# PoTaTo-Mika/fish-speech

Measured on AMD Instinct MI355X. Metric: audio-sec/wall-sec (RTF) + p50 first-sample latency, S2-Pro 4B @1/2/4/8 GPU, higher is better.
Workload: dtype bf16; 1 GPU; BASELINE config 2 per GPU: one utterance = 64-token prompt + 216 Dual-AR frames (top_k 30, top_p 0.8, temp 0.8) + codec decode [1,10,216] -> 442368 samples; global_batch=1, frames=216, prompt_len=64, first_chunk_frames=1, vocoder_chunks=first_chunk_frames, then growing 4x, vocoder=serial, parallelism=dp1

## Files before the change

### fish-speech_amd/csrc/fm_attn.hip

```cpp
#include "fm_kernels.h"
#include "fm_runtime.h"
#include "fm_attn_dev.h"
#include "fm_frag.h"

template <typename T>
__device__ __forceinline__ void head_prep(const T* src, int hd, bool norm, const T* nw, float eps,
                                          const float* tab, bool do_rope, float (&x0)[2],
                                          float (&x1)[2], int& np, int lane) {
    const int half = hd >> 1;
    np = 0;
    for (int p = lane; p < half; p += 64, ++np) {
        x0[np] = ld(src, 2 * p);
        x1[np] = ld(src, 2 * p + 1);
    }
    if (norm) {
        float ss = 0.f;
        for (int i = 0; i < np; ++i) ss += x0[i] * x0[i] + x1[i] * x1[i];
        ss = wave_sum(ss);
        const float rs = 1.0f / sqrtf(ss / (float)hd + eps);
        for (int i = 0; i < np; ++i) {
            const int p = lane + 64 * i;
            x0[i] = rnd<T>((x0[i] * rs) * ld(nw, 2 * p));
            x1[i] = rnd<T>((x1[i] * rs) * ld(nw, 2 * p + 1));
        }
    }
    if (do_rope) {
        for (int i = 0; i < np; ++i) {
            const int p = lane + 64 * i;
            const float c = tab[2 * p], s = tab[2 * p + 1];
            const float y0 = x0[i] * c - x1[i] * s;
            const float y1 = x1[i] * c + x0[i] * s;
            x0[i] = rnd<T>(y0);
            x1[i] = rnd<T>(y1);
        }
    }
}

template <typename T>
__global__ __launch_bounds__(512) void attn_decode2_kernel(AttnDecArgs<T> a) {
    extern __shared__ __attribute__((aligned(16))) unsigned char smem[];
    unsigned long long tz[7] = {0, 0, 0, 0, 0, 0, 0};
    DBG_TS(tz, 0)
    const int lane = threadIdx.x & 63, wave = threadIdx.x >> 6;
    const int r = blockIdx.x, kvh = blockIdx.y, sp = blockIdx.z;
    const int hd = a.hd, g = a.nh / a.nkv, ks = hd + 8, cap = a.cap;
    const int half = hd >> 1;
    const T* raw = a.qkv + (size_t)r * a.ldqkv;
    const int slot = a.row_slot[r];
    const int pos = a.row_pos[r];
    float q0[2][2], q1[2][2];
    for (int i = 0; i < 2; ++i) {
        const int hh = wave + 8 * i;
        for (int u = 0; u < 2; ++u) {
            const int p = lane + 64 * u;
            const bool ok = hh < g && p < half;
            const T* src = raw + (size_t)(kvh * g + (ok ? hh : 0)) * hd;
// ... 385 lines not shown
        for (int e = 0; e < 8; ++e) {
            o[e] += __shfl_xor(o[e], 16);
            o[e] += __shfl_xor(o[e], 32);
        }
        if (lane < 16 && vd < hd)
#pragma unroll
            for (int e = 0; e < 8; ++e) ored[wave][h][vd + e] = o[e];
    }
    __syncthreads();
    const bool single = nsp == 1;
    float* part = a.part + (((size_t)r * a.nh + (size_t)kvh * g) * a.maxsplit + sp) * (hd + 2);
    for (int idx = threadIdx.x; idx < g * hd; idx += 256) {
        const int h = idx / hd, e = idx - h * hd;
        const float o = (ored[0][h][e] + ored[1][h][e]) + (ored[2][h][e] + ored[3][h][e]);
        if (single) {
            st(a.out + (size_t)r * a.nh * hd + (size_t)(kvh * g + h) * hd, e, o / mls[h][1]);
        } else {
            float* pp = part + (size_t)h * a.maxsplit * (hd + 2);
            __hip_atomic_store(pp + 2 + e, o, __ATOMIC_RELAXED, __HIP_MEMORY_SCOPE_AGENT);
            if (e == 0) {
                __hip_atomic_store(pp, mls[h][0], __ATOMIC_RELAXED, __HIP_MEMORY_SCOPE_AGENT);
                __hip_atomic_store(pp + 1, mls[h][1], __ATOMIC_RELAXED, __HIP_MEMORY_SCOPE_AGENT);
            }
        }
    }
    if (single) return;
    asm volatile("s_waitcnt vmcnt(0)" ::: "memory");
    __syncthreads();
    if (threadIdx.x == 0) {
        const int t = __hip_atomic_fetch_add(a.cnt + (size_t)r * a.nkv + kvh, 1, __ATOMIC_RELAXED,
                                             __HIP_MEMORY_SCOPE_AGENT);
        flag = t == nsp - 1;
        if (t == nsp - 1) __hip_atomic_store(a.cnt + (size_t)r * a.nkv + kvh, 0, __ATOMIC_RELAXED, __HIP_MEMORY_SCOPE_AGENT);
    }
    __syncthreads();
    if (!flag) return;
    const float* p0 = a.part + (((size_t)r * a.nh + (size_t)kvh * g) * a.maxsplit) * (hd + 2);
    auto ldp = [](const float* q) { return __hip_atomic_load(q, __ATOMIC_RELAXED, __HIP_MEMORY_SCOPE_AGENT); };
    for (int idx = threadIdx.x; idx < g * hd; idx += 256) {
        const int h = idx / hd, e = idx - h * hd;
        const float* pp = p0 + (size_t)h * a.maxsplit * (hd + 2);
        float M = -INFINITY;
        for (int q = 0; q < nsp; ++q) M = fmaxf(M, ldp(pp + (size_t)q * (hd + 2)));
        float L = 0.f, O = 0.f;
        for (int q = 0; q < nsp; ++q) {
            const float w = expf(ldp(pp + (size_t)q * (hd + 2)) - M);
            L += w * ldp(pp + (size_t)q * (hd + 2) + 1);
            O += w * ldp(pp + (size_t)q * (hd + 2) + 2 + e);
        }
        st(a.out + (size_t)r * a.nh * hd + (size_t)(kvh * g + h) * hd, e, O / L);
    }
}

template <typename T> __device__ __forceinline__ void cvt16(const u32x4_t v, float (&o)[16 / sizeof(T)]) {
    if constexpr (sizeof(T) == 2) {
#pragma unroll
        for (int i = 0; i < 4; ++i) {
            o[2 * i] = __uint_as_float(v[i] << 16);
            o[2 * i + 1] = __uint_as_float(v[i] & 0xffff0000u);
        }
    } else {
#pragma unroll
        for (int i = 0; i < 4; ++i) o[i] = __uint_as_float(v[i]);
    }
}

constexpr int FD_GM = 4;
__device__ __forceinline__ float sum_rows4(float v, int lane) {
    const unsigned u = __float_as_uint(v);
    const auto r32 = __builtin_amdgcn_permlane32_swap(u, u, false, false);
    v += __uint_as_float(lane < 32 ? r32[1] : r32[0]);
    const unsigned w = __float_as_uint(v);
    const auto r16 = __builtin_amdgcn_permlane16_swap(w, w, false, false);
    return v + __uint_as_float(((lane >> 4) & 1) ? r16[0] : r16[1]);
}
template <typename T> __device__ __forceinline__ typename Frag<T>::f frag_f32(const float* v) {
    typename Frag<T>::f f;
    if constexpr (sizeof(T) == 2) {
#pragma unroll
        for (int i = 0; i < 4; ++i) f[i] = hi_pair(v[2 * i], v[2 * i + 1]);
    } else {
#pragma unroll
        for (int i = 0; i < 4; ++i) {
            f.lo[i] = v[i];
            f.hi[i] = v[4 + i];
        }
    }
    return f;
}
template <typename T, int HD, int NW, int GM>
__global__ __launch_bounds__(NW * 64) void attn_fd_kernel(AttnDecArgs<T> a) {
    static_assert(GM == 1 || GM == 2 || GM == FD_GM, "1, 2 or every q head of the kv head");
    static_assert(HD % 32 == 0 && HD <= 128, "head_dim a multiple of 32 up to 128");
    constexpr int NT = NW * 64, FD_TILE = 16 * NW;
    constexpr int VL = 8 * (int)sizeof(T) / 16;
    constexpr int half = HD / 2;
    __shared__ __attribute__((aligned(16))) float q_s[GM][HD];
    __shared__ __attribute__((aligned(16))) float kv_new[2][HD];
    __shared__ __attribute__((aligned(16))) float wml[NW][GM][2];
    constexpr int OG = NW > 4 ? 1 : 4;
    __shared__ __attribute__((aligned(16))) float ored[NW][OG][GM][HD];
    __shared__ int flag;
    unsigned long long tz[7] = {0, 0, 0, 0, 0, 0, 0};
    DBG_TS(tz, 0)
    const int lane = threadIdx.x & 63, wave = threadIdx.x >> 6;
    const int l16 = lane & 15, qq = lane >> 4;
    const int r = blockIdx.x, kvh = blockIdx.y;
    const int hg = GM == FD_GM ? 0 : (int)blockIdx.z / a.maxsplit, sp = (int)blockIdx.z - hg * a.maxsplit;
    const int g = min(GM, a.nh / a.nkv - hg * GM), h0 = kvh * (a.nh / a.nkv) + hg * GM, nitem = g + 2;
    const int slot = a.row_slot[r];
    const int pos = a.row_pos[r];
    constexpr int NI = (2 + GM + NW - 1) / NW;
    float x0[NI], x1[NI];
#pragma unroll
    for (int i = 0; i < NI; ++i) {
        const int it = wave + NW * i;
        const int row = it < g ? h0 + it : (it == g ? a.nh + kvh : a.nh + a.nkv + kvh);
        const bool ok = it < nitem && lane < half;
        float v0, v1;
        raw_pair<T>(a.qkv, a.ldqkv, a.qslab, a.qslab_kp, gridDim.x, a.qbias, r,
                    (size_t)(it < nitem ? row : 0) * HD + 2 * (lane < half ? lane : 0), v0, v1);
        x0[i] = ok ? v0 : 0.f;
        x1[i] = ok ? v1 : 0.f;
    }
    const int npos = pos + 1;
    int nsp = min(a.maxsplit, (npos + a.cap - 1) / a.cap);
    const int chunk = ((npos + nsp - 1) / nsp + 15) & ~15;
    nsp = (npos + chunk - 1) / chunk;
    if (sp >= nsp) return;
    const int j0 = sp * chunk, jend = min(j0 + chunk, npos);
    const bool owner = jend == npos;
    const size_t base = (size_t)slot * a.slot_stride + a.layer_off + (size_t)kvh * a.S * HD;
    T* kc = a.kc + base;
    T* vc = a.vc + base;
    const int vd = 8 * l16 < HD ? 8 * l16 : HD - 8;
    using F = Frag<T>;
    constexpr int NKS = HD / 32;
    typename F::f kb[NKS];
    u32x4_t vb[4][VL];
    auto issue = [&](int jb) {
        const int jk = min(jb + 16 * wave + l16, jend - 1);
#pragma unroll
        for (int ks = 0; ks < NKS; ++ks) kb[ks] = F::load(kc + (size_t)jk * HD + 32 * ks + 8 * qq);
#pragma unroll
        for (int it = 0; it < 4; ++it) {
            const int jv = min(jb + 16 * wave + 4 * it + qq, jend - 1);
            const u32x4_t* pv = reinterpret_cast<const u32x4_t*>(vc + (size_t)jv * HD + vd);
#pragma unroll
            for (int c = 0; c < VL; ++c) vb[it][c] = pv[c];
        }
    };
    const float* tab = a.rope + (size_t)pos * HD;
    const float2 rcs = *reinterpret_cast<const float2*>(tab + 2 * (lane < half ? lane : 0));
    issue(j0);
#pragma unroll
    for (int i = 0; i < NI; ++i) {
        const int it = wave + NW * i;
        if (it >= nitem || (it >= g && !owner)) continue;
        const bool isq = it < g, isk = it == g;
        if (a.qk_norm && (isq || isk)) {
            const float ss = wave_sum(x0[i] * x0[i] + x1[i] * x1[i]);
            const float rs = 1.0f / sqrtf(ss / (float)HD + a.eps);
            const T* nw = isq ? a.qn : a.kn;
            if (lane < half) {
                x0[i] = rnd<T>((x0[i] * rs) * ld(nw, 2 * lane));
                x1[i] = rnd<T>((x1[i] * rs) * ld(nw, 2 * lane + 1));
            }
        }
        if (lane < half) {
            float y0 = x0[i], y1 = x1[i];
            if (isq || isk) {
                const float c = rcs.x, sn = rcs.y;
                y0 = rnd<T>(x0[i] * c - x1[i] * sn);
                y1 = rnd<T>(x1[i] * c + x0[i] * sn);
            }
            if (isq) {
                q_s[it][2 * lane] = y0;
                q_s[it][2 * lane + 1] = y1;
                if (a.qdbg && sp == 0) {
                    float* qdp = a.qdbg + ((size_t)r * a.nh + h0 + it) * HD;
                    qdp[2 * lane] = y0;
                    qdp[2 * lane + 1] = y1;
                }
            } else {
                kv_new[isk ? 0 : 1][2 * lane] = y0;
                kv_new[isk ? 0 : 1][2 * lane + 1] = y1;
                if (hg == 0) {
                    T* dst = (isk ? kc : vc) + (size_t)pos * HD;
                    st(dst, 2 * lane, y0);
                    st(dst, 2 * lane + 1, y1);
                }
            }
        }
    }
    lds_barrier();
    DBG_TS(tz, 1)
    const int qh = l16 >> 2;
    const bool qrow = (l16 & 3) == 0 && qh < g;
    typename F::f qa[NKS];
#pragma unroll
    for (int ks = 0; ks < NKS; ++ks) {
        float qv[8];
#pragma unroll
        for (int e = 0; e < 8; ++e) qv[e] = qrow ? q_s[qh < GM ? qh : 0][32 * ks + 8 * qq + e] : 0.f;
        qa[ks] = frag_f32<T>(qv);
    }
    __shared__ __attribute__((aligned(16))) float p_s[NW][16][GM];
    float m_run = -INFINITY, l_run = 0.f, o[GM][8];
#pragma unroll
    for (int h = 0; h < GM; ++h)
#pragma unroll
        for (int e = 0; e < 8; ++e) o[h][e] = 0.f;
    const int npass = (jend - j0 + FD_TILE - 1) / FD_TILE;
    for (int pa = 0; pa < npass; ++pa) {
        const int jb = j0 + pa * FD_TILE;
        const int jk = jb + 16 * wave + l16;
        if (owner && jk == pos) {
#pragma unroll
            for (int ks = 0; ks < NKS; ++ks) kb[ks] = frag_f32<T>(&kv_new[0][32 * ks + 8 * qq]);
        }
        f32x4_t sc = {0.f, 0.f, 0.f, 0.f};
#pragma unroll
        for (int ks = 0; ks < NKS; ++ks) sc = F::mma(qa[ks], kb[ks], sc);
        float vf[4][8];
#pragma unroll
        for (int it = 0; it < 4; ++it)
#pragma unroll
            for (int c = 0; c < VL; ++c) {
                float t[16 / sizeof(T)];
                cvt16<T>(vb[it][c], t);
#pragma unroll
                for (int u = 0; u < (int)(16 / sizeof(T)); ++u) vf[it][c * (16 / sizeof(T)) + u] = t[u];
            }
        if (pa + 1 < npass) issue(jb + FD_TILE);
        if (owner) {
#pragma unroll
            for (int it = 0; it < 4; ++it)
                if (min(jb + 16 * wave + 4 * it + qq, jend - 1) == pos)
#pragma unroll
                    for (int e = 0; e < 8; ++e) vf[it][e] = kv_new[1][vd + e];
        }
        const bool kval = jk < jend && qq < g;
        {
            const float sv = kval ? sc[0] * a.scale : -INFINITY;
            const float mnew = fmaxf(m_run, row_max16(sv));
            const float alpha = mnew == -INFINITY ? 1.f : expf(m_run - mnew);
            const float p = kval ? expf(sv - mnew) : 0.f;
            m_run = mnew;
            l_run = l_run * alpha + p;
            if (GM == FD_GM || qq < GM) p_s[wave][l16][qq] = p;
#pragma unroll
            for (int h = 0; h < GM; ++h) {
                if (h >= g) break;
                const float ah = __int_as_float(__builtin_amdgcn_readlane(__float_as_int(alpha), 16 * h));
#pragma unroll
                for (int e = 0; e < 8; ++e) o[h][e] *= ah;
            }
        }
        __builtin_amdgcn_wave_barrier();
#pragma unroll
        for (int it = 0; it < 4; ++it) {
            float pv[GM];
            if constexpr (GM == 4) {
                const f32x4_t t = *reinterpret_cast<const f32x4_t*>(&p_s[wave][4 * it + qq][0]);
                pv[0] = t[0], pv[1] = t[1], pv[2] = t[2], pv[3] = t[3];
            } else if constexpr (GM == 2) {
                const float2 t = *reinterpret_cast<const float2*>(&p_s[wave][4 * it + qq][0]);
                pv[0] = t.x, pv[1] = t.y;
            } else {
                pv[0] = p_s[wave][4 * it + qq][0];
            }
#pragma unroll
            for (int h = 0; h < GM; ++h) {
                if (h >= g) break;
#pragma unroll
                for (int e = 0; e < 8; ++e) o[h][e] += pv[h] * vf[it][e];
            }
        }
        __builtin_amdgcn_wave_barrier();
    }
    DBG_TS(tz, 2)
    __shared__ unsigned long long wend[NW];
    if (a.dbg && lane == 0) wend[wave] = __builtin_amdgcn_s_memrealtime();
    const float lrow = row_sum16(l_run);
    if (l16 == 0 && qq < g) {
        wml[wave][qq][0] = m_run;
        wml[wave][qq][1] = lrow;
    }
#pragma unroll
    for (int h = 0; h < GM; ++h) {
        if (h >= g) break;
        if constexpr (OG == 1) {
#pragma unroll
            for (int e = 0; e < 8; ++e) o[h][e] = sum_rows4(o[h][e], lane);
        }
        if (8 * l16 < HD && (OG == 4 || qq == 0)) {
            f32x4_t* dst = reinterpret_cast<f32x4_t*>(&ored[wave][OG == 4 ? qq : 0][h][8 * l16]);
            dst[0] = (f32x4_t){o[h][0], o[h][1], o[h][2], o[h][3]};
            dst[1] = (f32x4_t){o[h][4], o[h][5], o[h][6], o[h][7]};
        }
    }
    DBG_TS(tz, 5)
    lds_barrier();
    DBG_TS(tz, 3)
    const bool single = nsp == 1;
    for (int idx = threadIdx.x; idx < g * HD; idx += NT) {
        const int h = idx / HD, e = idx - h * HD;
        float M = wml[0][h][0];
#pragma unroll
        for (int w = 1; w < NW; ++w) M = fmaxf(M, wml[w][h][0]);
        float L = 0.f, O = 0.f;
#pragma unroll
        for (int w = 0; w < NW; ++w) {
            const float sc = expf(wml[w][h][0] - M);
            L += sc * wml[w][h][1];
            if constexpr (OG == 4)
                O += sc * ((ored[w][0][h][e] + ored[w][1][h][e]) + (ored[w][2][h][e] + ored[w][3][h][e]));
            else
                O += sc * ored[w][0][h][e];
        }
        if (single) {
            st(a.out + (size_t)r * a.nh * HD + (size_t)(h0 + h) * HD, e, O / L);
        } else {
            float* pp = a.part + (((size_t)r * a.nh + h0 + h) * a.maxsplit + sp) * (HD + 2);
            __hip_atomic_store(pp + 2 + e, O, __ATOMIC_RELAXED, __HIP_MEMORY_SCOPE_AGENT);
            if (e == 0) {
                __hip_atomic_store(pp, M, __ATOMIC_RELAXED, __HIP_MEMORY_SCOPE_AGENT);
                __hip_atomic_store(pp + 1, L, __ATOMIC_RELAXED, __HIP_MEMORY_SCOPE_AGENT);
            }
        }
    }
    if (a.dbg && threadIdx.x == 0) {
        tz[4] = __builtin_amdgcn_s_memrealtime();
        for (int w = 0; w < NW; ++w) tz[6] = wend[w] > tz[6] ? wend[w] : tz[6];
        dbg_record(a.dbg, 0xFFFC, (unsigned)(nsp << 16 | (jend - j0)), tz);
    }
    if (single) return;
    asm volatile("s_waitcnt vmcnt(0)" ::: "memory");
    __syncthreads();
    if (threadIdx.x == 0) {
        int* tk = a.cnt + (size_t)r * a.nh + kvh * (a.nh / a.nkv) + hg;
        const int t = __hip_atomic_fetch_add(tk, 1, __ATOMIC_RELAXED, __HIP_MEMORY_SCOPE_AGENT);
        flag = t == nsp - 1;
        if (t == nsp - 1) __hip_atomic_store(tk, 0, __ATOMIC_RELAXED, __HIP_MEMORY_SCOPE_AGENT);
    }
    __syncthreads();
    if (!flag) return;
    DBG_TS(tz, 5)
    constexpr int PP = GM * HD * 8 / NT > 0 ? GM * HD * 8 / NT : 1;
    const int q = l16, grp = threadIdx.x >> 4;
    const int k0 = grp * PP, h = k0 / half, e0 = 2 * (k0 - h * half);
    if (h >= g) return;
    const int qc = q < nsp ? q : nsp - 1;
    const unsigned long long* pp = reinterpret_cast<const unsigned long long*>(
        a.part + (((size_t)r * a.nh + h0 + h) * a.maxsplit + qc) * (HD + 2));
    const unsigned long long ml = __hip_atomic_load(pp, __ATOMIC_RELAXED, __HIP_MEMORY_SCOPE_AGENT);
    unsigned long long ov[PP];
#pragma unroll
    for (int j = 0; j < PP; ++j) ov[j] = __hip_atomic_load(pp + 1 + e0 / 2 + j, __ATOMIC_RELAXED, __HIP_MEMORY_SCOPE_AGENT);
    const float mq = q < nsp ? __uint_as_float((unsigned)ml) : -INFINITY;
    const float lq = __uint_as_float((unsigned)(ml >> 32));
    float M = mq;
#pragma unroll
    for (int m = 1; m < 16; m <<= 1) M = fmaxf(M, __shfl_xor(M, m));
    const float w = q < nsp ? expf(mq - M) : 0.f;
    float L = w * lq;
#pragma unroll
    for (int m = 1; m < 16; m <<= 1) L += __shfl_xor(L, m);
    T* out = a.out + (size_t)r * a.nh * HD + (size_t)(h0 + h) * HD + e0;
#pragma unroll
    for (int j = 0; j < PP; ++j) {
        float o0 = w * __uint_as_float((unsigned)ov[j]), o1 = w * __uint_as_float((unsigned)(ov[j] >> 32));
#pragma unroll
        for (int m = 1; m < 16; m <<= 1) {
            o0 += __shfl_xor(o0, m);
            o1 += __shfl_xor(o1, m);
        }
        if (q == (j & 15)) {
            st(out, 2 * j, o0 / L);
            st(out, 2 * j + 1, o1 / L);
        }
    }
    if (a.dbg && threadIdx.x == 0) {
        tz[6] = __builtin_amdgcn_s_memrealtime();
        dbg_record(a.dbg, 0xFFFB, (unsigned)nsp, tz);
    }
}

template <typename T>
__global__ __launch_bounds__(64) void fast_attn2_kernel(FastFusedArgs<T> a) {
    unsigned long long tz[7] = {0, 0, 0, 0, 0, 0, 0};
    DBG_TS(tz, 0)
    fast_attn_head<T>(a, blockIdx.x, blockIdx.y, threadIdx.x, tz);
    if (a.dbg && threadIdx.x == 0) {
        tz[4] = __builtin_amdgcn_s_memrealtime();
        dbg_record(a.dbg, 0xFFFE, (unsigned)a.cpos, tz);
    }
}

template <typename T>
__global__ __launch_bounds__(256) void fast_attn_fused_kernel(FastFusedArgs<T> a) {
    extern __shared__ __attribute__((aligned(16))) unsigned char smem[];
    const int lane = threadIdx.x & 63, wave = threadIdx.x >> 6;
    const int r = blockIdx.x, kvh = blockIdx.y;
    const int slot = a.row_slot[r];
    const int hd = a.hd, g = a.nh / a.nkv, C = a.S, cpos = a.cpos;
    float* Kt = reinterpret_cast<float*>(smem);
    float* Vt = Kt + (size_t)C * hd;
    float* qs = Vt + (size_t)C * hd;
    float* ps = qs + 4 * hd;
    const size_t base = (size_t)slot * a.slot_stride + a.layer_off + (size_t)kvh * C * hd;
    T* kc = a.kc + base;
    T* vc = a.vc + base;
    const T* raw = a.qkv + (size_t)r * a.ldqkv;
    const float* tab = a.rope + (size_t)cpos * hd;
    if (wave < 2) {
        float x0[2], x1[2];
        int np;
        const int hk = wave == 0 ? a.nh + kvh : a.nh + a.nkv + kvh;
        head_prep<T>(raw + (size_t)hk * hd, hd, wave == 0 && a.qk_norm, a.kn, a.eps, tab, wave == 0, x0,
                     x1, np, lane);
        T* dst = (wave == 0 ? kc : vc) + (size_t)cpos * hd;
        float* tile = (wave == 0 ? Kt : Vt) + (size_t)cpos * hd;
        for (int i = 0; i < np; ++i) {
            const int p = lane + 64 * i;
            st(dst, 2 * p, x0[i]);
            st(dst, 2 * p + 1, x1[i]);
            tile[2 * p] = x0[i];
            tile[2 * p + 1] = x1[i];
        }
    }
    for (int idx = threadIdx.x; idx < cpos * hd; idx += 256) {
        Kt[idx] = ld(kc, idx);
        Vt[idx] = ld(vc, idx);
    }
    for (int hb = 0; hb < g; hb += 4) {
        const int ql = hb + wave;
        if (ql < g) {
            float x0[2], x1[2];
// ... 785 lines not shown
```

### fish-speech_amd/csrc/fm_kernels.h

```cpp
#pragma once
#include <algorithm>
#include "fm_common.h"
#include "fm_tune_table.h"

enum { EPI_STORE = 0, EPI_RESID = 1, EPI_SWIGLU = 2, EPI_F32 = 3 };

template <typename T> void launch_swiglu_i8(hipStream_t s, const T* t, int ldt, T* act, int lda, int inter, int R);
template <typename T> void launch_pack(hipStream_t s, const T* src, int N, int K, T* dst);
template <typename T> void launch_quant_rows(hipStream_t s, T* w, int N, int K, int8_t* q, T* scale);
template <typename T> void launch_i8_to(hipStream_t s, const int8_t* q, int64_t n, T* dst);
void launch_pack_q8(hipStream_t s, const int8_t* src, int N, int K, int8_t* dst);
void launch_pack_q8s(hipStream_t s, const int8_t* src, int N, int K, int8_t* dst);
void launch_quant4(hipStream_t s, bf16_t* w, int N, int K, int gs, uint8_t* q, uint32_t* sz);
void launch_pack_q4(hipStream_t s, const uint8_t* q, int N, int K, uint8_t* dst);
void launch_pack_q4_rows(hipStream_t s, const uint8_t* q, int N, int K, uint32_t* dst);
void launch_pack_sz4(hipStream_t s, const uint32_t* sz, int N, int K, int gs, uint32_t* dst);
void launch_pack_q4s(hipStream_t s, const uint8_t* q, int N, int K, uint32_t* dst);

template <typename T> struct LinearArgs {
    const T* W;
    const T* W2;
    const T* bias;
    const T* X;
    int ldx, R, N, K;
// ... 341 lines not shown
    float* slab;
    bf16_t* act = nullptr;
    int lda = 0;
    const bf16_t* wscale = nullptr;
    const unsigned char* q8s = nullptr;
    const uint32_t* q4s = nullptr;
    const uint32_t* sz = nullptr;
};
void launch_prompt_skinny(hipStream_t s, const PromptSkinnyArgs& a, int ks);
int prompt_skinny_ks(int N, int K, int target);

template <typename T> struct AttnDecArgs {
    const T* qkv;
    int ldqkv;
    const int* row_slot;
    const int* row_pos;
    int nh, nkv, hd, qk_norm;
    float eps;
    const T* qn;
    const T* kn;
    const float* rope;
    T* kc;
    T* vc;
    size_t slot_stride, layer_off;
    int S, maxsplit;
    float scale;
    float* part;
    int cap;
    int* cnt;
    T* out;
    unsigned long long* dbg;
    float* qdbg = nullptr;
    int nwb = 4;
    int hpb = 4;
    const float* qslab = nullptr;
    int qslab_kp = 1;
    const T* qbias = nullptr;
};
template <typename T> void launch_attn_decode2(hipStream_t s, const AttnDecArgs<T>& a, int R);
inline size_t attn2_lds_bytes(int hd, int g, int cap, size_t esz) {
    return (size_t)cap * (hd + 8) * esz + (size_t)cap * hd * esz + (size_t)g * hd * 4 + (size_t)g * cap * 4 +
           16 + 8 * (size_t)g * 4;
}
inline int attn2_cap(int hd, int g, size_t esz) {
    long budget = 150L * 1024 - 16 - 8L * g * 4 - (long)g * hd * 4;
    long per = (long)(2 * hd + 8) * (long)esz + 4L * g;
    long c = budget / per;
    c = c > 256 ? 256 : c;
    return (int)(c & ~15L);
}
constexpr int FD_NSP = 16;
inline bool attn_fd_ok(int hd, int g) { return (hd == 32 || hd == 64 || hd == 128) && g >= 1 && g <= 4; }
template <typename T> void launch_attn_fd(hipStream_t s, const AttnDecArgs<T>& a, int R);
template <typename T> void launch_attn_decode3(hipStream_t s, const AttnDecArgs<T>& a, int R);
template <typename T> void launch_fast_attn_fused(hipStream_t s, const FastFusedArgs<T>& a, int R);
template <typename T> void launch_fast_attn2(hipStream_t s, const FastFusedArgs<T>& a, int R);
template <typename T> void launch_sample_radix(hipStream_t s, const SampleArgs& a, int R);
int sample_fast_max_row();
void sample_init();
template <typename T>
void launch_attn_combine(hipStream_t s, const float* part, const int* row_pos, int R, int nh, int hd,
                         int split, int maxsplit, T* out);
```

### fish-speech_amd/csrc/fm_llm.cpp

```cpp
#include <math.h>

#include <memory>

#include "fm_llm_model.h"

static thread_local std::string g_err;
void fm_set_error(const std::string& s) { g_err = s; }
extern "C" const char* fm_last_error(void) { return g_err.c_str(); }
extern "C" int fm_device_count(void) {
    int n = 0;
    if (hipGetDeviceCount(&n) != hipSuccess) return 0;
    return n;
}

static void check_tokens(fm_llm* m, const int32_t* tok, int T) {
    const fm_model_config& c = m->c;
    for (int t = 0; t < T; ++t) {
        const int t0 = tok[t];
        FMCHECK(t0 >= 0 && t0 < c.vocab_size, "token id out of range: " + std::to_string(t0));
        for (int q = 0; q < m->C; ++q) {
            const int v = tok[(size_t)(q + 1) * T + t];
            FMCHECK(v >= 0 && v < m->cb, "codebook token out of range: " + std::to_string(v));
        }
    }
}

static void reset_slot(fm_llm* m, int slot, const fm_sampling* sp) {
    HIPCHK(hipMemsetAsync((char*)m->ras + (size_t)slot * m->C1 * 10 * 4, 0, (size_t)m->C1 * 10 * 4, m->stream));
    SlotParams p{};
    if (sp) {
        FMCHECK(sp->top_k >= 1, "top_k must be >= 1: got " + std::to_string(sp->top_k));
        p.temperature = sp->temperature;
        p.top_p = sp->top_p;
        p.top_k = sp->top_k;
        p.mask_im_end = sp->mask_im_end;
        p.seed = sp->seed;
    } else {
        p.temperature = 0.7f;
        p.top_p = 0.9f;
        p.top_k = 1;
    }
    p.step = 0;
    p.force = m->host_force[slot];
    HIPCHK(hipMemcpyAsync(m->sp + slot, &p, sizeof p, hipMemcpyHostToDevice, m->stream));
    HIPCHK(hipStreamSynchronize(m->stream));
    m->host_step[slot] = 0;
}

static void upload_frame_rows(fm_llm* m, const int32_t* slots, int n) {
    std::vector<int> s(slots, slots + n), p(n);
    if (s == m->uploaded_slots) return;
    for (int i = 0; i < n; ++i) p[i] = m->host_pos[s[i]];
    HIPCHK(hipMemcpyAsync(m->frame_slot, s.data(), (size_t)n * 4, hipMemcpyHostToDevice, m->stream));
    HIPCHK(hipMemcpyAsync(m->frame_pos, p.data(), (size_t)n * 4, hipMemcpyHostToDevice, m->stream));
    HIPCHK(hipStreamSynchronize(m->stream));
    m->uploaded_slots = s;
}

static void chain_err_async(fm_llm* m) {
    if (fm_tuning().gemv_chain || fm_tuning().fin_split > 1 ||
        (m->fxt && fm_tuning().fattn_wo))
        HIPCHK(hipMemcpyAsync(m->h_chain_err, m->chain_err, sizeof(int), hipMemcpyDeviceToHost, m->stream));
}
static void chain_err_check(fm_llm* m) {
    if (!m->h_chain_err || !m->h_chain_err[0]) return;
    m->h_chain_err[0] = 0;
    HIPCHK(hipMemset(m->chain_cnt, 0, GEMV_CHAIN_WORDS * sizeof(unsigned)));
    HIPCHK(hipMemset(m->chain_err, 0, 16 * sizeof(int)));
    if (m->fin_cnt) HIPCHK(hipMemset(m->fin_cnt, 0, (size_t)std::max(m->max_slots, 64) * 2 * sizeof(int)));
    throw FmError{FM_ERR_STATE,
                  "in-launch hand-off wait timed out (gemv chain / split finalize / fused fast "
                  "attention + wo; counters reset)"};
}

extern "C" {

int fm_llm_open(const fm_model_config* cfg, int device, int precision, int max_slots, fm_llm** out) {
    return fm_guard([&] {
        FMCHECK(cfg && out, "null argument");
        FMCHECK(precision == FM_PREC_BF16 || precision == FM_PREC_FP32, "bad precision");
        FMCHECK(max_slots >= 1 && max_slots <= 4096, "bad max_slots");
        const fm_model_config& c = *cfg;
        FMCHECK(c.dim % 32 == 0 && c.fast_dim % 32 == 0, "dims must be multiples of 32");
        FMCHECK(c.intermediate_size % 32 == 0 && c.fast_intermediate_size % 32 == 0,
                "intermediate sizes must be multiples of 32");
        FMCHECK((c.n_head * c.head_dim) % 32 == 0 && (c.fast_n_head * c.fast_head_dim) % 32 == 0,
                "n_head*head_dim must be a multiple of 32");
        FMCHECK(c.head_dim % 8 == 0 && c.head_dim <= 256 && c.fast_head_dim <= 256, "bad head_dim");
        FMCHECK(c.n_head % c.n_local_heads == 0 && c.fast_n_head % c.fast_n_local_heads == 0, "bad GQA");
        FMCHECK(c.num_codebooks >= 1 && c.num_codebooks <= 63, "bad num_codebooks");
        FMCHECK(c.codebook_size <= 8192, "codebook_size > 8192 unsupported");
        FMCHECK(c.im_end_id >= 0 && c.im_end_id < c.vocab_size, "im_end_id must be set");
        FMCHECK(c.semantic_begin_id >= 0 && c.semantic_end_id < c.vocab_size &&
                    c.semantic_begin_id <= c.semantic_end_id,
                "bad semantic id range");
        int ndev = fm_device_count();
        FMCHECK(ndev > 0, "no HIP device visible");
        FMCHECK(device >= 0 && device < ndev, "bad device index");
        HIPCHK(hipSetDevice(device));
        std::unique_ptr<fm_llm> m(new fm_llm());
        m->c = c;
        m->device = device;
        m->prec = precision;
        m->esz = precision == FM_PREC_BF16 ? 2 : 4;
        m->max_slots = max_slots;
        m->S = (c.max_seq_len + 7) / 8 * 8;
        m->C = c.num_codebooks;
        m->C1 = c.num_codebooks + 1;
        m->cb = c.codebook_size;
        HIPCHK(hipStreamCreateWithFlags(&m->stream, hipStreamNonBlocking));
        const char* g = getenv("FISHMI_GRAPH");
        m->use_graph = !(g && g[0] == '0');
        build_inventory(m.get());
        *out = m.release();
    });
}

int fm_llm_set_quant_int4(fm_llm* m, int groupsize) {
    return fm_guard([&] {
        FMCHECK(m && (groupsize == 32 || groupsize == 64 || groupsize == 128 || groupsize == 256),
                "int4: groupsize must be 32, 64, 128 or 256 (WeightOnlyInt4QuantHandler, quantize.py:366)");
        FMCHECK(!m->finalized, "weights are frozen after finalize");
        for (auto& kv : m->w) FMCHECK(!kv.second.set, "set the quantization mode before any tensor");
        FMCHECK(m->quant == FM_QUANT_NONE, "quantization mode already set");
// ... 513 lines not shown
```

### fish-speech_amd/csrc/fm_llm_frame.cpp

```cpp
#include <math.h>

#include <algorithm>
#include <array>

#include "fm_codec.h"
#include "fm_llm_model.h"

template <typename T> struct Run {
    typedef T type_t;
    fm_llm* m;
    hipStream_t s;
    int64_t E;
    bool rows_distinct_slots = false, bs_frame = false, x_ss = false;
    struct BsPending {
        bool on = false;
        const float* slab = nullptr;
        int kparts = 0, d = 0, R = 0;
        void* res = nullptr;
        void* out = nullptr;
        const void* sc = nullptr;
    } pend;
    std::vector<std::array<int, 2>> segs;
    void set_pending(const float* slab, int kparts, int d, int R, void* res, void* out, const void* sc) {
        pend = BsPending{true, slab, kparts, d, R, res, out, sc};
// ... 692 lines not shown
        a.ldx = ldx_in;
        a.xidx = xidx;
        a.xidx_ld = m->C1;
        a.xidx_col = xcol;
        a.xidx_rows = xidx ? m->cb : 0;
        gemv(L.wqkv, a, PRO_NORM, EPI_STORE, 1, "linear", kv_rows ? d.nq() / 16 : 0);
    }
    GemvArgs<T> qkv_args(const StackDims& d, const LayerW& L, int n) {
        GemvArgs<T> a = ga();
        a.bias = (const T*)L.bqkv;
        a.nw = (const T*)L.an;
        a.R = n;
        a.N = d.nqkv();
        a.K = d.dim;
        a.Y = (T*)m->qkv;
        a.ldy = d.nqkv();
        return a;
    }
    static int dead_q_bits(const fm_llm* m) { return m->quant && !m->fdm.o_bias ? fm_tuning().fast_dead_q : 0; }
    bool qkv0_live() const {
        return sizeof(T) == 2 && (m->quant ? (dead_q_bits(m) & 1) : (row_bits() & 32)) && m->qkv0 && m->qkv0_built &&
               m->qkv0_epoch == fm_tuning().epoch;
    }

    struct Small {
        const StackDims& d;
        const LayerW& L;
        int n;
        bool first;
        const void* x_in;
        int ldx_in;
        const int32_t* xidx;
        int xcol;
        void *xb, *hb;
        bool is_fast;
        int cpos, layer;
        KsbPlan kp;
        void* xo;
        int pair = 0;
        const void* x_in1 = nullptr;
    };
    static const void* row1(const Small& c, const void* p, int w) {
        return (const char*)p + (c.pair == 2 ? (size_t)w * sizeof(T) : 0);
    }
    static void* row1(const Small& c, void* p, int w) { return (char*)p + (c.pair == 2 ? (size_t)w * sizeof(T) : 0); }
    struct SmallPath {
        bool rf;
        bool fw;
        bool att_wo;
        bool row_here;
        bool tab;
        bool kv0;
        bool kv_only;
    };
    SmallPath small_path(const Small& c, bool kv_only) const {
        const StackDims& d = c.d;
        SmallPath p{};
        p.kv_only = kv_only;
        p.rf = row_fin(c.n);
        const int fq = m->qmode();
        const bool fw_any = c.is_fast && p.rf && fm_tuning().fattn_wo && m->fxt && m->fdm.n_layer * m->C >= 2 &&
                            m->fdm.n_layer * m->C <= 40 && fattn_wo_ok(d.nh, d.nkv, d.hd, c.cpos, d.dim, d.nq(), fq);
        p.fw = fw_any && !kv_only;
        p.att_wo = c.is_fast && !kv_only && fm_tuning().attn_wo && !m->quant && c.n == 1 && c.cpos < 16 && d.hd % 16 == 0 &&
                   d.hd <= 128 && d.nh % d.nkv == 0 && (d.nq() / c.kp.wo) % d.hd == 0 && d.nqkv() % 8 == 0;
        p.row_here = row_qkv(c.n) && (!c.first || (row_bits() & 16));
        const bool bits56 = sizeof(T) == 2 && !m->quant && c.is_fast && c.n == 1;
        const int dq = sizeof(T) == 2 && c.is_fast && c.n == 1 && fw_any && fattn_wo_dead_ok(d.nq(), fq) ? dead_q_bits(m) : 0;
        p.tab = (bits56 || (dq & 1)) && c.first && c.xidx && p.fw && qkv0_live();
        p.kv0 = bits56 && c.cpos == 0 && (row_bits() & 64) && p.row_here && !p.att_wo && d.hd <= 256 &&
                (d.nqkv() - d.nq()) % fm_tuning().row_qkv_rp == 0;
        if ((dq & 2) && c.cpos == 0 && !p.att_wo && d.hd <= 256)
            p.kv0 = m->quant == FM_QUANT_INT4
                        ? p.row_here && (d.nqkv() - d.nq()) % fm_tuning().row_qkv_rp == 0 && (d.nqkv() - d.nq()) % 8 == 0
                        : !p.row_here && d.nq() % 16 == 0 && d.nqkv() % 16 == 0;
        return p;
    }
    FastFusedArgs<T> small_fast_args(const Small& c, const SmallPath& p) const {
        const StackDims& d = c.d;
        FastFusedArgs<T> fa{(const T*)m->qkv, d.nqkv(), m->frame_slot, d.nh, d.nkv, d.hd, d.qk_norm,
                            m->c.norm_eps, (const T*)c.L.qn, (const T*)c.L.kn, m->frope, (T*)m->fkc,
                            (T*)m->fvc, m->fslot_stride, (size_t)c.layer * m->flayer_stride, m->C, c.cpos,
                            1.0f / sqrtf((float)d.hd), (T*)m->att};
        fa.dbg = fm_tuning().dbg;
        fa.noq = p.kv0;
        return fa;
    }
    void small_qkv(const Small& c, const SmallPath& p) {
        if (p.tab && !c.pair) return;
        const StackDims& d = c.d;
        GemvArgs<T> a = qkv_args(d, c.L, c.n);
        if (!c.is_fast && c.n == 1 && fm_tuning().kv_prefetch)
            kv_prefetch(a, (const T*)m->kc, (const T*)m->vc, m->frame_slot, m->frame_pos, m->slot_stride,
                        (size_t)c.layer * m->layer_stride, m->S, d.nkv, d.hd);
        else if (c.is_fast && c.n == 1 && fm_tuning().fkv_prefetch && m->fiota && c.cpos < 16)
            kv_prefetch(a, (const T*)m->fkc, (const T*)m->fvc, m->frame_slot, m->fiota + c.cpos, m->fslot_stride,
                        (size_t)c.layer * m->flayer_stride, m->C, d.nkv, d.hd);
        if (c.first) {
            qkv_first(d, c.L, a, c.n, c.x_in, c.ldx_in, c.pair ? nullptr : c.xidx, c.pair ? 0 : c.xcol, m->qkv,
                      p.kv0 || c.pair);
        } else if (p.row_here) {
            qkv_row(d, c.L, a, false, c.xb, 0, nullptr, 0, m->qkv, p.kv0, c.pair != 0);
        } else {
            a.X = (const T*)c.xb;
            a.ldx = d.dim;
            a.ss_in = m->ssX;
            a.ss_gran = p.rf ? 1 : 0;
            gemv(c.L.wqkv, a, PRO_PRENORM, EPI_STORE, 1, "linear", p.kv0 ? d.nq() / 16 : 0);
        }
    }
    void small_attn(const Small& c, const SmallPath& p) {
        const StackDims& d = c.d;
        const int n = c.n;
        hipStream_t st = s;
        if (!c.is_fast) {
            AttnDecArgs<T> aa{(const T*)m->qkv, d.nqkv(), m->frame_slot, m->frame_pos, d.nh, d.nkv, d.hd,
                              d.qk_norm, m->c.norm_eps, (const T*)c.L.qn, (const T*)c.L.kn, m->rope, (T*)m->kc,
                              (T*)m->vc, m->slot_stride, (size_t)c.layer * m->layer_stride, m->S,
                              m->maxsplit, 1.0f / sqrtf((float)d.hd), m->part};
            aa.cap = attn2_frame_cap(d.hd, d.nh / d.nkv, E, false);
            aa.maxsplit = FM_CEIL(m->S, aa.cap);
            aa.cnt = m->attn_cnt;
            aa.dbg = fm_tuning().dbg;
            aa.out = (T*)m->att;
            auto go = [st, aa, n] { attn_slow_on(st, aa, n); };
            m->prof.record("attn_slow", 0, go);
            launch("attn", 0, 0, go);
        } else if (!p.att_wo && !p.fw) {
            const FastFusedArgs<T> fa = small_fast_args(c, p);
            const bool f2 = c.cpos < 16 && d.hd <= 256;
            launch("attn", 0, 0, [st, fa, n, f2] {
                if (f2)
                    launch_fast_attn2<T>(st, fa, n);
                else
                    launch_fast_attn_fused<T>(st, fa, n);
            });
        }
    }
    void small_wo(const Small& c, const SmallPath& p) {
        const StackDims& d = c.d;
        const LayerW& L = c.L;
        if (p.fw || p.rf) {
            FattnWoArgs A{};
            RowGemvArgs& r = A.wo;
            row_weight(r, L.wo);
            r.X = (const bf16_t*)m->att;
            r.bias = (const bf16_t*)L.bo;
            if (!c.pair) {
                row_residual(r, c.first, c.x_in, c.ldx_in, c.xidx, c.xcol, c.xb, d.dim);
                r.res_out = (bf16_t*)c.hb;
            } else {
                RowGemvArgs r1{};
                row_residual(r1, c.first, c.x_in1, c.ldx_in, c.xidx, c.xcol, (const bf16_t*)c.xb + d.dim, d.dim);
                r.ldr = r1.ldr;
                r.residx = r1.residx;
                r.res_col = r1.res_col;
                r.res_rows = r1.res_rows;
                if (c.pair == 2) {
                    r.res = r1.res;
                    r.res_out = (bf16_t*)c.hb + d.dim;
                } else {
                    r.xr = 2;
                    r.res = (const bf16_t*)(c.first ? c.x_in : c.xb);
                    r.res1 = r1.res;
                    r.res_out = (bf16_t*)c.hb;
                    r.res_out1 = (bf16_t*)c.hb + d.dim;
                }
            }
            r.N = d.dim;
            r.K = d.nq();
            if (!p.fw) {
                rowgemv(r, ROWGEMV_FIN);
                return;
            }
            const FastFusedArgs<T> fa = small_fast_args(c, p);
            A.at = *reinterpret_cast<const FastFusedArgs<bf16_t>*>(&fa);
            A.at.dbg = nullptr;
            A.at.row_pos = m->frame_pos;
            A.xt = m->fxt;
            A.gen = 1 + c.layer + m->fdm.n_layer * c.cpos;
            A.err = m->chain_err;
            A.delay = fm_tuning().fw_delay;
            A.cheap = fm_tuning().fw_cheap;
            A.prio = fm_tuning().fw_prio;
            A.ilp = fm_tuning().fattn_ilp;
            if (p.tab) {
                A.qtab = (const bf16_t*)m->qkv0;
                A.qidx = c.xidx;
                A.qcol = c.xcol;
                A.qrows = m->cb;
            }
            A.kv0 = p.kv0;
            A.pair = c.pair;
            hipStream_t st = s;
            auto go = [st, A] { launch_fattn_wo(st, A); };
            launch("attn", rowgemv_wbytes(r), 2.0 * r.N * r.K, go, "attn_wo");
            return;
        }
        GemvArgs<T> a = ga();
        a.bias = (const T*)L.bo;
        a.X = (const T*)m->att;
        a.ldx = d.nq();
        a.R = c.n;
        a.N = d.dim;
        a.K = d.nq();
        a.Yf = m->slabA;
        a.ldy = d.dim;
        if (c.first) {
            a.res = (const T*)c.x_in;
            a.ldr = c.ldx_in;
            a.residx = c.xidx;
            a.xidx_ld = m->C1;
            a.xidx_col = c.xcol;
            a.xidx_rows = c.xidx ? m->cb : 0;
        } else {
            a.res = (const T*)c.xb;
            a.ldr = d.dim;
        }
        a.res_out = (T*)c.hb;
        a.ldro = d.dim;
        a.ss_out = m->ssH;
        a.tickets = m->tickets;
        if (p.att_wo) a.att = small_fast_args(c, p);
// ... 556 lines not shown
```

### fish-speech_amd/csrc/fm_llm_model.h

```cpp
#pragma once
#include <hip/hip_runtime.h>

#include <algorithm>

#include "fm_kernels.h"
#include "fm_runtime.h"

static constexpr int PREFILL_CHUNK = 1024;
static constexpr int ATTN_PIECE = 256;
static constexpr int ATTN_SPLIT = 64;
static constexpr int GEMV_MAX_ROWS = 8;
static constexpr int KSB_MAX = 8;

inline int attn2_frame_cap(int hd, int g, size_t esz, bool batched) {
    const int cap = attn2_cap(hd, g, esz), knob = batched ? fm_tuning().attn_cap_batched : fm_tuning().attn_cap;
    return knob ? std::min(cap, knob) : cap;
}
struct AttnSlowPlan {
    int kernel, nwb, cap;
    int hpb = 4;
};
inline int fd_hpb_rows(int R) { return R <= GEMV_MAX_ROWS ? fm_tuning().fd_hpb : 4; }
inline AttnSlowPlan attn_slow_plan(int R, int hd, int g, int cap0) {
    const FmTuning& tu = fm_tuning();
// ... 82 lines not shown
    int S = 0, C = 0, C1 = 0, cb = 0, nsem = 0, Nhead = 0, maxsplit = 0, Rmax = 0;
    std::vector<LayerW> slow, fast;
    void *emb = nullptr, *cbemb = nullptr, *norm = nullptr, *fproj_b = nullptr, *femb = nullptr, *fnorm = nullptr;
    Linear head_c, fproj_w, fout;
    void *kc = nullptr, *vc = nullptr, *fkc = nullptr, *fvc = nullptr;
    size_t slot_stride = 0, layer_stride = 0, fslot_stride = 0, flayer_stride = 0;
    float *rope = nullptr, *frope = nullptr;
    void *x = nullptr, *h = nullptr, *xn = nullptr, *qkv = nullptr, *q = nullptr, *att = nullptr,
         *act = nullptr;
    void *xl = nullptr, *xnl = nullptr, *fx = nullptr, *fh = nullptr, *fxn = nullptr;
    void *x2 = nullptr, *fx2 = nullptr;
    unsigned* chain_cnt = nullptr;
    int* chain_err = nullptr;
    int* h_chain_err = nullptr;
    void* plast = nullptr;
    float *part = nullptr, *logits = nullptr, *flogits = nullptr;
    void* act2 = nullptr;
    int* attn_cnt = nullptr;
    float *ssX = nullptr, *ssH = nullptr;
    int* tickets = nullptr;
    float* skpart = nullptr;
    long long skpart_cap = 0;
    float *slabA = nullptr, *slabB = nullptr;
    float *bsA = nullptr, *bsB = nullptr;
    float* bsQ = nullptr;
    int *frame_slot = nullptr, *frame_pos = nullptr, *prow_slot = nullptr, *prow_pos = nullptr;
    int32_t *tok_in = nullptr, *cols = nullptr, *ptok = nullptr, *ras = nullptr;
    SlotParams* sp = nullptr;
    int32_t* force_cols = nullptr;
    float *tap_slow = nullptr, *tap_fast = nullptr;
    std::vector<int> host_force;
    int32_t* h_cols = nullptr;
    int32_t* h_hist = nullptr;
    size_t h_hist_n = 0;
    std::vector<int> host_pos, host_step;
    std::vector<int> uploaded_slots;
    bool use_graph = true;
    std::map<int, hipGraphExec_t> graphs;
    Profiler prof;
    std::vector<void*> allocs;
    int quant = FM_QUANT_NONE;
    int q4_gs = 0;
    int qmode() const { return quant == FM_QUANT_INT8 ? 1 : (quant == FM_QUANT_INT4 ? 2 : 0); }
    int* fin_cnt = nullptr;
    float* fin_ss = nullptr;
    bool compact = false;
    bool streams_codes() const { return quant != FM_QUANT_INT4 || fm_tuning().int4_stream || compact; }
    int64_t mem[7] = {0, 0, 0, 0, 0, 0, 0};
    int mem_cat = 6;
    bool row_ok = false;
    bool row_qkv_ok = false;
    bool row_w13_ok = false;
    uint32_t* fxt = nullptr;
    int32_t* fiota = nullptr;
    void* qkv0 = nullptr;
    int32_t* qkv0_iota = nullptr;
    unsigned qkv0_epoch = 0;
    bool qkv0_built = false;
    struct Prefix {
        void* buf = nullptr;
        int npos = 0;
        size_t bytes = 0;
    };
    std::map<int, Prefix> prefixes;
    int next_prefix_id = 1;
    int* pfx_slots = nullptr;

    ~fm_llm() {
        if (device >= 0) (void)hipSetDevice(device);
        for (auto& g : graphs) (void)hipGraphExecDestroy(g.second);
        for (auto& kv : w) {
            if (kv.second.p) (void)hipFree(kv.second.p);
            if (kv.second.q) (void)hipFree(kv.second.q);
        }
        for (void* p : allocs) (void)hipFree(p);
        for (auto& kv : prefixes) (void)hipFree(kv.second.buf);
        if (h_cols) (void)hipHostFree(h_cols);
        if (h_hist) (void)hipHostFree(h_hist);
        if (h_chain_err) (void)hipHostFree(h_chain_err);
        if (stream) (void)hipStreamDestroy(stream);
    }
    void* dalloc(size_t bytes, bool zero = true) {
        void* p = nullptr;
        if (bytes == 0) bytes = 16;
        hipError_t e = hipMalloc(&p, bytes);
        if (e != hipSuccess)
            throw FmError{FM_ERR_OOM, "hipMalloc(" + std::to_string(bytes) + ") failed: " + hipGetErrorString(e)};
        if (zero) HIPCHK(hipMemsetAsync(p, 0, bytes, stream));
        allocs.push_back(p);
        mem[mem_cat] += (int64_t)bytes;
        return p;
    }
};

void add_t(fm_llm* m, const std::string& n, int64_t rows, int64_t cols);
void build_inventory(fm_llm* m);
DTensor& tensor_for(fm_llm* m, const char* name, int64_t numel);
bool is_quant_linear(const std::string& n);
std::string base_of(const std::string& n);
void finalize(fm_llm* m);
void ensure_qkv0(fm_llm* m);
void launch_frame(fm_llm* m, int n);
void decode_frame_eager(fm_llm* m, int n);
void prefill_frame(fm_llm* m, int slot, const int32_t* tokens, int T, int pos0);
void prefill_batch_frame(fm_llm* m, int n, const int32_t* slots, const int32_t* const* toks, const int32_t* T,
                         const int32_t* pos0);
// ... 3 lines not shown
```

### fish-speech_amd/csrc/fm_llm_weights.cpp

```cpp
#include "fm_llm_model.h"

void add_t(fm_llm* m, const std::string& n, int64_t rows, int64_t cols) {
    DTensor t;
    t.rows = rows;
    t.cols = cols;
    t.numel = rows * cols;
    m->w[n] = t;
}
static void add_stack(fm_llm* m, const std::string& pre, const StackDims& s) {
    for (int i = 0; i < s.n_layer; ++i) {
        std::string p = pre + std::to_string(i) + ".";
        add_t(m, p + "attention.wqkv.weight", s.nqkv(), s.dim);
        if (s.qkv_bias) add_t(m, p + "attention.wqkv.bias", 1, s.nqkv());
        add_t(m, p + "attention.wo.weight", s.dim, s.nq());
        if (s.o_bias) add_t(m, p + "attention.wo.bias", 1, s.dim);
        if (s.qk_norm) {
            add_t(m, p + "attention.q_norm.weight", 1, s.hd);
            add_t(m, p + "attention.k_norm.weight", 1, s.hd);
        }
        add_t(m, p + "feed_forward.w1.weight", s.inter, s.dim);
        add_t(m, p + "feed_forward.w3.weight", s.inter, s.dim);
        add_t(m, p + "feed_forward.w2.weight", s.dim, s.inter);
        add_t(m, p + "ffn_norm.weight", 1, s.dim);
        add_t(m, p + "attention_norm.weight", 1, s.dim);
// ... 330 lines not shown
    if (m->finalized) return;
    const fm_model_config& c = m->c;
    bsacc_init();
    sample_init();
    for (auto& kv : m->w) FMCHECK(kv.second.set || kv.second.optional, "tensor not set: " + kv.first);
    if (m->compact) {
        FMCHECK(m->quant && m->prec == FM_PREC_BF16, "compact: a weight-only bf16 handle only");
        for (auto& kv : m->w) {
            if (!is_quant_linear(kv.first)) continue;
            const int64_t K = kv.second.cols;
            if (m->quant == FM_QUANT_INT4)
                FMCHECK(m->q4_gs % 128 == 0 && K % 128 == 0 && K % m->q4_gs == 0,
                        "compact int4 needs a group size and in_features that are multiples of 128: " + kv.first +
                            " (group size " + std::to_string(m->q4_gs) + ", in_features " + std::to_string(K) + ")");
            else
                FMCHECK(K % 64 == 0, "compact int8 needs in_features % 64 == 0: " + kv.first);
        }
    }
    if (m->quant) quantize_linears(m);
    std::map<std::string, Linear> plain;
    for (auto& kv : m->w)
        if (is_linear_weight(kv.first) && !is_ffn_w13(kv.first)) plain[kv.first] = plain_linear(m, kv.first);
    m->row_ok = m->row_qkv_ok = m->row_w13_ok = true;
    auto stack = [&](const std::string& pre, const StackDims& d, std::vector<LayerW>& out) {
        out.resize(d.n_layer);
        for (int i = 0; i < d.n_layer; ++i) {
            std::string p = pre + std::to_string(i) + ".";
            LayerW& L = out[i];
            L.wqkv = plain.at(p + "attention.wqkv.weight");
            L.wo = plain.at(p + "attention.wo.weight");
            L.w13 = w13_linear(m, p, d.inter, d.dim);
            L.w2 = plain.at(p + "feed_forward.w2.weight");
            L.bqkv = m->quant ? nullptr : Wopt(m, p + "attention.wqkv.bias");
            L.bo = m->quant ? nullptr : Wopt(m, p + "attention.wo.bias");
            L.qn = Wopt(m, p + "attention.q_norm.weight");
            L.kn = Wopt(m, p + "attention.k_norm.weight");
            L.an = W(m, p + "attention_norm.weight");
            L.fn = W(m, p + "ffn_norm.weight");
            m->row_ok = m->row_ok && L.wo.rm && L.w2.rm;
            m->row_qkv_ok = m->row_qkv_ok && L.wqkv.rm;
            m->row_w13_ok = m->row_w13_ok && L.w13.rm;
        }
    };
    stack("layers.", m->sd, m->slow);
    stack("fast_layers.", m->fdm, m->fast);
    {
        int32_t io[16];
        for (int c = 0; c < 16; ++c) io[c] = c - 1;
        m->fiota = (int32_t*)m->dalloc(sizeof(io), false);
        HIPCHK(hipMemcpy(m->fiota, io, sizeof(io), hipMemcpyHostToDevice));
    }
    if (m->prec == FM_PREC_BF16)
        m->fxt = (uint32_t*)m->dalloc(2 * (size_t)m->fdm.nh * m->fdm.hd * sizeof(uint32_t));
    m->emb = W(m, "embeddings.weight");
    m->cbemb = W(m, "codebook_embeddings.weight");
    m->norm = W(m, "norm.weight");
    if (plain.count("fast_project_in.weight")) m->fproj_w = plain.at("fast_project_in.weight");
    m->fproj_b = m->quant ? nullptr : Wopt(m, "fast_project_in.bias");
    m->femb = W(m, "fast_embeddings.weight");
    m->fnorm = W(m, "fast_norm.weight");
    m->fout = plain.at("fast_output.weight");
    m->head_c = head_linear(m);
    for (auto& kv : m->w) {
        const DTensor& t = kv.second;
        if (!t.p || is_linear_weight(kv.first)) continue;
        const int64_t rows = t.rows > 1 ? (t.rows + 15) / 16 * 16 : 1;
        const std::string& n = kv.first;
        const bool scales = n.size() > 7 && n.compare(n.size() - 7, 7, ".scales") == 0;
        m->mem[scales ? 1 : 4] += rows * t.cols * (int64_t)m->esz;
    }
    const StackDims& d = m->sd;
    m->layer_stride = (size_t)d.nkv * m->S * d.hd;
    m->slot_stride = m->layer_stride * d.n_layer;
    m->mem_cat = 5;
    m->kc = m->dalloc(m->slot_stride * m->max_slots * m->esz);
    m->vc = m->dalloc(m->slot_stride * m->max_slots * m->esz);
    const StackDims& f = m->fdm;
    m->flayer_stride = (size_t)f.nkv * m->C * f.hd;
    m->fslot_stride = m->flayer_stride * f.n_layer;
    m->fkc = m->dalloc(m->fslot_stride * m->max_slots * m->esz);
    m->fvc = m->dalloc(m->fslot_stride * m->max_slots * m->esz);
    m->mem_cat = 6;
    auto rt = rope_table_host(m->S, d.hd, c.rope_base);
    m->rope = (float*)m->dalloc(rt.size() * 4, false);
    HIPCHK(hipMemcpy(m->rope, rt.data(), rt.size() * 4, hipMemcpyHostToDevice));
    auto frt = rope_table_host(m->C, f.hd, c.rope_base);
    m->frope = (float*)m->dalloc(frt.size() * 4, false);
    HIPCHK(hipMemcpy(m->frope, frt.data(), frt.size() * 4, hipMemcpyHostToDevice));
    const int R = m->Rmax = std::max(m->max_slots, PREFILL_CHUNK);
    const int dmax = std::max(c.dim, c.fast_dim);
    const int qkvmax = std::max(d.nqkv(), f.nqkv()), qmax = std::max(d.nq(), f.nq());
    const int imax = std::max(d.inter, f.inter);
    const size_t E = m->esz;
    m->x = m->dalloc((size_t)R * dmax * E);
    m->h = m->dalloc((size_t)R * dmax * E);
    m->xn = m->dalloc((size_t)R * dmax * E);
    m->qkv = m->dalloc((size_t)R * qkvmax * E);
    m->q = m->dalloc((size_t)R * qmax * E);
    m->att = m->dalloc((size_t)R * qmax * E);
    m->act = m->dalloc((size_t)R * imax * E);
    m->act2 = m->dalloc((size_t)R * 2 * imax * E);
    const int n = m->max_slots;
    m->xl = m->dalloc((size_t)n * dmax * E);
    m->plast = m->dalloc((size_t)n * dmax * E);
    m->xnl = m->dalloc((size_t)n * dmax * E);
    m->fx = m->dalloc((size_t)std::max(n, 2) * dmax * E);
// ... 54 lines not shown
```

### fish-speech_amd/csrc/fm_ops.cpp

```cpp
#include <hip/hip_runtime.h>
#include <math.h>
#include <string.h>

#include <algorithm>
#include <vector>

#include "fm_codec.h"
#include "fm_kernels.h"
#include "fm_llm_model.h"
#include "fm_ops_util.h"
#include "fm_runtime.h"

using namespace fm_ops_util;

namespace {

struct TuneScope {
    int& knob;
    const int keep;
    TuneScope(int& k, int v) : knob(k), keep(k) { knob = v; }
    ~TuneScope() { knob = keep; }
};

template <typename T>
// ... 468 lines not shown
    r.K = K;
    InOut<bf16_t> y(b, o.y, (size_t)(o.pair == 1 ? 2 : 1) * N);
    r.res = res;
    r.res_out = y.d;
    if (o.pair == 1) {
        r.xr = 2;
        r.res = b.upload<bf16_t>(o.res0, (size_t)N);
        r.res1 = res;
        r.res_out1 = y.d + N;
    }
    int* err = (int*)b.alloc(16);
    if (o.fused) {
        FattnWoArgs A{};
        A.at = at;
        A.wo = r;
        A.wo.X = att;
        A.xt = (uint32_t*)b.alloc((size_t)2 * K * 4);
        if (o.xt_init) b.put(A.xt, o.xt_init, (size_t)2 * K * 4);
        A.gen = o.gen;
        A.err = err;
        A.delay = fm_tuning().fw_delay;
        A.cheap = fm_tuning().fw_cheap;
        A.prio = fm_tuning().fw_prio;
        A.ilp = o.ilp;
        if (qtab) {
            A.qtab = qtab;
            A.qidx = idx;
            A.qcol = o.idx_col;
            A.qrows = o.qrows;
        }
        A.kv0 = o.kv0;
        A.pair = o.pair;
        launch_fattn_wo(s, A);
    } else {
        FMCHECK(!o.pair, "the unfused composition runs one row");
        if (qtab) {
            const int iv = o.idx[o.idx_col], xi = iv < 0 ? 0 : (iv >= o.qrows ? o.qrows - 1 : iv);
            at.qkv = qtab + (size_t)xi * ld;
        }
        at.noq = o.kv0;
        launch_fast_attn2<bf16_t>(s, at, 1);
        HIPCHK(hipGetLastError());
        r.X = att;
        launch_rowgemv(s, r, ROWGEMV_FIN);
    }
    HIPCHK(hipGetLastError());
    y.get(s);
    kc.get(s);
    vc.get(s);
    HIPCHK(hipMemcpyAsync(&o.status[1], err, 4, hipMemcpyDeviceToHost, s));
    HIPCHK(hipStreamSynchronize(s));
}

template <typename T>
void embed_t(hipStream_t s, const int32_t* tok, int R, const float* emb, int V, const float* cbemb, int d, int C,
             int cb, int sb, int se, int scale, float* x) {
    DevBufs b(s);
    T* e = b.upload<T>(emb, (size_t)V * d);
    T* ce = b.upload<T>(cbemb, (size_t)C * cb * d);
    int32_t* td = (int32_t*)b.alloc((size_t)R * (C + 1) * 4);
    b.put(td, tok, (size_t)R * (C + 1) * 4);
    T* xd = (T*)b.alloc((size_t)R * d * sizeof(T));
    launch_embed<T>(s, td, R, e, ce, d, C, cb, sb, se, scale, xd, nullptr);
    HIPCHK(hipGetLastError());
    download<T>(xd, (size_t)R * d, x, s);
}

int count_nonzero(const int* d, size_t n, hipStream_t s) {
    std::vector<int> h(n);
    HIPCHK(hipMemcpyAsync(h.data(), d, n * 4, hipMemcpyDeviceToHost, s));
    HIPCHK(hipStreamSynchronize(s));
    return (int)std::count_if(h.begin(), h.end(), [](int v) { return v != 0; });
}

template <typename T> T* upload_packed(DevBufs& b, const float* w, int N, int K) {
    T* t = b.upload<T>(w, (size_t)N * K);
    T* pk = (T*)b.alloc((size_t)((N + 15) / 16 * 16) * K * sizeof(T));
    launch_pack<T>(b.s, t, N, K, pk);
    HIPCHK(hipGetLastError());
    return pk;
}

template <typename T>
void linear_op_t(hipStream_t s, int epi, const float* w, const float* w2, const float* bias, const float* x, int ldx,
                 const float* res, int ldr, int R, int N, int K, int split, float* y, int ldy, int y_rows, int reps,
                 int* ksb_out, int* dirty) {
    DevBufs b(s);
    const bool f32 = epi == EPI_F32;
    LinearArgs<T> a{};
    a.W = upload_packed<T>(b, w, N, K);
    if (epi == EPI_SWIGLU) a.W2 = upload_packed<T>(b, w2, N, K);
    if (bias) a.bias = b.upload<T>(bias, (size_t)N);
    a.X = b.upload<T>(x, (size_t)R * ldx);
    a.ldx = ldx;
    a.R = R;
    a.N = N;
    a.K = K;
    a.ldy = ldy;
    if (epi == EPI_RESID) {
        a.res = b.upload<T>(res, (size_t)R * ldr);
        a.ldr = ldr;
    }
    InOut<T> yt(b, y, f32 ? 1 : (size_t)y_rows * ldy);
    InOut<float> yf(b, y, f32 ? (size_t)y_rows * ldy : 1);
    a.Y = f32 ? nullptr : yt.d;
    a.Yf = f32 ? yf.d : nullptr;
// ... 563 lines not shown
        FMCHECK(qkv && kcache && vcache && out, "null argument");
        FMCHECK(!qk_norm || (qn && kn), "qk_norm needs both norm weights");
        FMCHECK(kernel >= 0 && kernel <= 3,
                "kernel must be 0 (fast_attn2), 1 (fast_attn2, noq), 2 (fast_attn_fused) or 3 (qk_rope_cache + fast_attn)");
        FMCHECK(R >= 1 && R <= 64 && nh >= 1 && nkv >= 1 && nh % nkv == 0, "bad rows / head counts");
        FMCHECK(hd >= 8 && hd <= 256 && hd % 8 == 0, "head_dim a multiple of 8 up to 256");
        FMCHECK(S >= 1 && S <= 63 && cpos >= 0 && cpos < S, "1 to 63 codebooks, cpos among them");
        FMCHECK(kernel > 1 || cpos < 16, "fast_attn2 positions are < 16");
        FMCHECK(kernel != 1 || cpos == 0, "noq is the codebook-0 form");
        FMCHECK(kernel != 2 || (size_t)2 * S * hd * 4 + (size_t)4 * hd * 4 + 1024 <= 64 * 1024, "fast_attn_fused: LDS tile too large");
        check_slot_rows(R, row_slot, nullptr, nslots, layers, layer, S);
        for (int r = 0; r < R; ++r)
            for (int q = 0; q < r; ++q) FMCHECK(row_slot[q] != row_slot[r], "two rows in one slot");
        StreamGuard g(device);
        const SlotRows sr{row_slot, nullptr, nslots, layers, layer};
        if (precision == FM_PREC_BF16)
            fast_attn_t<bf16_t>(g.s, kernel, qkv, R, nh, nkv, hd, qn, kn, qk_norm, eps, rope_base, sr, cpos, kcache, vcache, S, out);
        else
            fast_attn_t<float>(g.s, kernel, qkv, R, nh, nkv, hd, qn, kn, qk_norm, eps, rope_base, sr, cpos, kcache, vcache, S, out);
    });
}

int fm_op_fattn_wo(int device, int quant, int gs, int fused, const float* qkv, const float* qtab, int qrows,
                   const int32_t* idx, int idx_n, int idx_col, int nh, int nkv, int hd, const float* qn, const float* kn,
                   int qk_norm, float eps, float rope_base, int slot, int cpos, int nslots, int layers, int layer,
                   float* kcache, float* vcache, int S, const float* w, const float* bias, const float* res,
                   int res_rows, int ldr, const float* res0, int N, int kv0, int pair, int ilp, int gen, int pos0,
                   const uint32_t* xt_init, float* y, int* status) {
    return fm_guard([&] {
        FMCHECK(qkv && kcache && vcache && w && res && y && status, "null argument");
        FMCHECK(quant == FM_QUANT_NONE || quant == FM_QUANT_INT8 || quant == FM_QUANT_INT4, "bad quant");
        FMCHECK(!qk_norm || (qn && kn), "qk_norm needs both norm weights");
        FMCHECK(nh >= 1 && nkv >= 1 && nh % nkv == 0 && hd >= 8 && hd <= 128 && hd % 8 == 0, "bad heads / head_dim");
        FMCHECK(S >= 1 && S <= 63 && cpos >= 0 && cpos < S && N >= 16 && N % 16 == 0, "bad S / cpos / N");
        FMCHECK(quant == FM_QUANT_NONE || !bias, "the int8 / int4 row forms take no bias");
        FMCHECK(quant != FM_QUANT_INT4 || (gs >= 8 && gs % 8 == 0 && (nh * hd) % gs == 0), "bad int4 group size");
        FMCHECK(!idx || (idx_n >= 1 && idx_col >= 0 && idx_col < idx_n), "bad index column");
        FMCHECK(res_rows >= 1 && ldr >= N && gen >= 1 && gen <= 40 && pos0 >= 0, "bad residual table / gen / position");
        FMCHECK(!qtab || (idx && !kv0 && qrows >= 1 && qrows == res_rows), "the table form is gathered by the residual's index");
        FMCHECK(!kv0 || (!idx && cpos == 0), "the K / V-only form runs at codebook 0, no gather");
        FMCHECK(pair >= 0 && pair <= 2, "pair must be 0, 1 or 2");
        FMCHECK(!pair || (fused && quant == FM_QUANT_NONE && !kv0 && cpos == 1 && (qtab != nullptr) == (idx != nullptr) &&
                          (pair == 1 ? res0 != nullptr : !qtab)),
                "pair form: fused, bf16, positions 0 and 1, row 0's residual (pair 1), no table in the last layer (pair 2)");
        check_slot_rows(1, &slot, nullptr, nslots, layers, layer, S);
        StreamGuard g(device);
        const FattnWoOp o{quant, gs, fused, qkv, qtab, qrows, idx, idx_n, idx_col, nh, nkv, hd, qn, kn, qk_norm, eps,
                          rope_base, slot, cpos, nslots, layers, layer, kcache, vcache, S, w, bias, res, res_rows, ldr,
                          res0, N, kv0, pair, ilp, gen, pos0, xt_init, y, status};
        fattn_wo_op(g.s, o);
    });
}

int fm_op_qk_rope(int device, int precision, int kernel, const float* qkv, int nh, int nkv, int hd, const float* qn,
                  const float* kn, int qk_norm, float eps, float rope_base, int pos, float* q_out, float* k_out) {
    return fm_guard([&] {
        FMCHECK(qkv && q_out && k_out, "null argument");
        FMCHECK(!qk_norm || (qn && kn), "qk_norm needs both norm weights");
        FMCHECK(kernel >= 0 && kernel <= 3,
                "kernel must be 0 (slow attn_decode2), 1 (fast attn2), 2 (slow attn_dec3) or 3 (slow attn_fd)");
        FMCHECK(nh >= 1 && nkv >= 1 && nh % nkv == 0 && nh / nkv <= 16, "bad head counts");
        FMCHECK(hd >= 8 && hd <= 256 && hd % 8 == 0, "bad head_dim");
        FMCHECK(pos >= 0 && pos < 65536, "bad position");
        StreamGuard g(device);
        if (precision == FM_PREC_BF16)
            qk_rope_t<bf16_t>(g.s, kernel, qkv, nh, nkv, hd, qn, kn, qk_norm, eps, rope_base, pos, q_out, k_out);
        else
            qk_rope_t<float>(g.s, kernel, qkv, nh, nkv, hd, qn, kn, qk_norm, eps, rope_base, pos, q_out, k_out);
    });
}

int fm_op_embed(int device, int precision, const int32_t* tok, int R, const float* emb, int vocab,
                const float* cbemb, int dim, int num_codebooks, int codebook_size, int semantic_begin_id,
                int semantic_end_id, int scale_codebook_embeddings, float* x) {
    return fm_guard([&] {
        FMCHECK(tok && emb && cbemb && x && R >= 1 && dim % 8 == 0, "bad arguments");
        for (int r = 0; r < R; ++r) {
            FMCHECK(tok[(size_t)r * (num_codebooks + 1)] >= 0 && tok[(size_t)r * (num_codebooks + 1)] < vocab,
                    "token id out of range");
            for (int q = 1; q <= num_codebooks; ++q) {
                const int v = tok[(size_t)r * (num_codebooks + 1) + q];
                FMCHECK(v >= 0 && v < codebook_size, "codebook token out of range");
            }
        }
        StreamGuard g(device);
        if (precision == FM_PREC_BF16)
            embed_t<bf16_t>(g.s, tok, R, emb, vocab, cbemb, dim, num_codebooks, codebook_size, semantic_begin_id,
                            semantic_end_id, scale_codebook_embeddings, x);
        else
            embed_t<float>(g.s, tok, R, emb, vocab, cbemb, dim, num_codebooks, codebook_size, semantic_begin_id,
                           semantic_end_id, scale_codebook_embeddings, x);
    });
}

int fm_op_quant4(int device, const float* w, int N, int K, int gs, uint8_t* q, float* scale, float* zero,
                 float* w_deq, const float* x, int R, float* y_q4, float* y_bf16) {
    return fm_guard([&] {
        FMCHECK(w && q && scale && zero && w_deq && N >= 1 && gs >= 2 && K % gs == 0, "bad arguments");
        FMCHECK(!x || (R >= 1 && R <= 8 && K % 32 == 0 && y_bf16), "bad GEMV arguments");
        StreamGuard g(device);
        DevBufs b(g.s);
        const int Np = (N + 15) / 16 * 16;
        bf16_t* dw = (bf16_t*)b.alloc((size_t)Np * K * 2);
        {
            bf16_t* t = b.upload<bf16_t>(w, (size_t)N * K);
            HIPCHK(hipMemcpyAsync(dw, t, (size_t)N * K * 2, hipMemcpyDeviceToDevice, g.s));
// ... 703 lines not shown
```

### fish-speech_amd/csrc/fm_rowgemv.hip

```cpp
#include "fm_common.h"
#include "fm_kernels.h"
#include "fm_runtime.h"
#include <type_traits>

typedef __attribute__((ext_vector_type(2))) uint32_t u32x2_t;
typedef __attribute__((ext_vector_type(4))) __bf16 bf16x4_t;

__device__ __forceinline__ float dot4(u32x2_t w, u32x2_t x, float acc) {
    const bf16x4_t wb = __builtin_bit_cast(bf16x4_t, w), xb = __builtin_bit_cast(bf16x4_t, x);
    acc = __builtin_amdgcn_fdot2_f32_bf16(__builtin_shufflevector(wb, wb, 0, 1), __builtin_shufflevector(xb, xb, 0, 1),
                                          acc, false);
    acc = __builtin_amdgcn_fdot2_f32_bf16(__builtin_shufflevector(wb, wb, 2, 3), __builtin_shufflevector(xb, xb, 2, 3),
                                          acc, false);
    return acc;
}
__device__ __forceinline__ float lo16(uint32_t w) { return __uint_as_float(w << 16); }
__device__ __forceinline__ float hi16(uint32_t w) { return __uint_as_float(w & 0xffff0000u); }
__device__ __forceinline__ float dot8r(u32x4_t w, u32x4_t x, float acc) {
    const bf16x8_t wb = __builtin_bit_cast(bf16x8_t, w), xb = __builtin_bit_cast(bf16x8_t, x);
    acc = __builtin_amdgcn_fdot2_f32_bf16(__builtin_shufflevector(wb, wb, 0, 1), __builtin_shufflevector(xb, xb, 0, 1),
                                          acc, false);
    acc = __builtin_amdgcn_fdot2_f32_bf16(__builtin_shufflevector(wb, wb, 2, 3), __builtin_shufflevector(xb, xb, 2, 3),
                                          acc, false);
    acc = __builtin_amdgcn_fdot2_f32_bf16(__builtin_shufflevector(wb, wb, 4, 5), __builtin_shufflevector(xb, xb, 4, 5),
                                          acc, false);
    acc = __builtin_amdgcn_fdot2_f32_bf16(__builtin_shufflevector(wb, wb, 6, 7), __builtin_shufflevector(xb, xb, 6, 7),
                                          acc, false);
    return acc;
}
__device__ __forceinline__ void ld_pair_bf(const bf16_t* p, float& x0, float& x1) {
    const uint32_t w = *reinterpret_cast<const uint32_t*>(p);
    x0 = lo16(w);
    x1 = hi16(w);
}

template <int QM> struct RowT {
    static constexpr int EPL = QM ? 8 : 4;
    static constexpr int CE = 64 * EPL;
    using XV = typename std::conditional<QM != 0, u32x4_t, u32x2_t>::type;
    static constexpr int WPL = QM == 2 ? 1 : 2;
};

template <int U, int RP, bool PRENORM, int EPI, bool G, int QM, bool TX, int XR = 1>
__device__ __forceinline__ void rowgemv_body(const RowGemvArgs& a, const int blk, const uint32_t* xt, const uint32_t gen,
                                             int* err) {
    static_assert(!TX || (!PRENORM && EPI == 1), "tagged x: the residual form only");
    static_assert(XR == 1 || (XR == 2 && QM == 0 && EPI <= 1 && (!G || EPI == 1)), "two x rows: bf16 STORE / FIN");
    constexpr bool FIN = EPI == 1;
    using R = RowT<QM>;
    using XV = typename R::XV;
    constexpr int EPL = R::EPL, NW = EPL / 2;
    constexpr int SB = XR * 4 * RP;
    constexpr bool LATE = XR == 2 && !TX && !PRENORM && U >= 10;
    __shared__ float red[XR * (4 * RP + 8)];
    const int lane = threadIdx.x & 63, wave = threadIdx.x >> 6;
    const int n0 = blk * RP;
    const int nch = a.K / R::CE;
    const int wa = (wave * nch) >> 2, nmy = (((wave + 1) * nch) >> 2) - wa;
    const int last = nmy > 0 ? nmy - 1 : 0;
    const unsigned long long ts0 = a.dbg ? __builtin_amdgcn_s_memrealtime() : 0;
    const int er = n0 + (int)(threadIdx.x % RP);
    const int ex = XR == 2 ? (int)((threadIdx.x / RP) & 1) : 0;
    int ri = 0, xi = 0;
    if constexpr (G && FIN) {
        const int32_t iv = a.residx[a.res_col];
        ri = iv < 0 ? 0 : (iv >= a.res_rows ? a.res_rows - 1 : iv);
    } else if constexpr (G) {
        const int32_t iv = a.xidx[a.xcol];
        xi = iv < 0 ? 0 : (iv >= a.xrows ? a.xrows - 1 : iv);
    }
    bf16_t rv = 0;
    if constexpr (FIN && XR == 2) rv = ex ? a.res1[(size_t)ri * a.ldr + er] : a.res[er];
    else if constexpr (FIN) rv = a.res[(size_t)ri * a.ldr + er];
    const bf16_t bv = *(a.bias ? a.bias + er : a.X);
    bf16_t sv = 0;
    if constexpr (QM == 1) sv = a.wscale[er];
    const XV* xp = reinterpret_cast<const XV*>(a.X + (size_t)xi * a.ldx) + (size_t)wa * 64 + lane;
    const XV* gp = reinterpret_cast<const XV*>(PRENORM ? a.nw : a.X) + (size_t)wa * 64 + lane;
    XV xv[XR][U], gv[PRENORM ? U : 1];
    if constexpr (!TX) {
#pragma unroll
        for (int u = 0; u < U; ++u) {
            const int j = (u < last ? u : last) * 64;
            xv[0][u] = xp[j];
            if constexpr (XR == 2 && !LATE) xv[1][u] = (reinterpret_cast<const XV*>(a.X1) + (size_t)wa * 64 + lane)[j];
            if constexpr (PRENORM) gv[u] = gp[j];
        }
    }
    constexpr int PF = 2;
    const bool pf_on = EPI == 0 && a.pf_kc != nullptr;
    int pf_s = 0, pf_p = 0;
    if constexpr (EPI == 0) {
        pf_s = *(pf_on ? a.pf_slot : reinterpret_cast<const int32_t*>(a.X));
        pf_p = *(pf_on ? a.pf_pos : reinterpret_cast<const int32_t*>(a.X));
    }
    asm volatile("" ::: "memory");
    constexpr int WU = QM == 2 ? 1 : U, WR = QM == 2 ? 1 : RP;
    constexpr int QU = QM == 2 ? U : 1, QR = QM == 2 ? RP : 1;
    u32x2_t wv[WU][WR];
    uint32_t w4[QU][QR], szv[QU][QR];
    if constexpr (QM == 2) {
        const size_t rw = (size_t)(a.K >> 3);
        const int ng = a.K / a.gs;
        const uint32_t* wp = a.Wq4 + (size_t)n0 * rw + (size_t)wa * 64 + lane;
#pragma unroll
        for (int u = 0; u < U; ++u) {
            const int jc = u < last ? u : last;
#pragma unroll
            for (int r = 0; r < RP; ++r) {
                w4[u][r] = __builtin_nontemporal_load(wp + r * rw + jc * 64);
                szv[u][r] = a.wsz[(size_t)(n0 + r) * ng + ((wa + jc) * 512 + lane * 8) / a.gs];
            }
        }
    } else {
        const unsigned char* wb = QM ? reinterpret_cast<const unsigned char*>(a.Wq) : reinterpret_cast<const unsigned char*>(a.W);
        const size_t rowb = (size_t)a.K * (QM ? 1 : 2);
        const u32x2_t* wp = reinterpret_cast<const u32x2_t*>(wb + (size_t)n0 * rowb) + (size_t)wa * 64 + lane;
        const size_t rs8 = rowb / 8;
#pragma unroll
        for (int u = 0; u < U; ++u) {
            const int j = (u < last ? u : last) * 64;
#pragma unroll
            for (int r = 0; r < RP; ++r) wv[u][r] = __builtin_nontemporal_load(wp + r * rs8 + j);
        }
    }
    asm volatile("" ::: "memory");
    unsigned long long tsw = 0, tsx = 0;
    unsigned polls = 0;
    if constexpr (TX) {
        if (a.dbg) tsw = __builtin_amdgcn_s_memrealtime();
        const __amdgpu_buffer_rsrc_t xr = __builtin_amdgcn_make_buffer_rsrc((void*)xt, (short)0, XR * a.K * 4, 0x00020000);
        u32x4_t xw[XR][U][EPL / 4];
        for (unsigned it = 0;; ++it) {
            polls = it + 1;
#pragma unroll
            for (int x = 0; x < XR; ++x)
#pragma unroll
                for (int u = 0; u < U; ++u) {
                    const int jc = u < last ? u : last;
#pragma unroll
                    for (int q = 0; q < EPL / 4; ++q)
                        xw[x][u][q] = __builtin_amdgcn_raw_buffer_load_b128(
                            xr, (x * a.K + (wa + jc) * R::CE + EPL * lane + 4 * q) * 4, 0, 16);
                }
            bool ok = true;
#pragma unroll
            for (int x = 0; x < XR; ++x)
#pragma unroll
                for (int u = 0; u < U; ++u)
#pragma unroll
                    for (int q = 0; q < EPL / 4; ++q)
#pragma unroll
                        for (int e = 0; e < 4; ++e) ok = ok && ((xw[x][u][q][e] & 0xffffu) == gen);
            if (__all(ok)) break;
            if (it >= (1u << 14)) {
                if (lane == 0) __hip_atomic_store(err, 1, __ATOMIC_RELAXED, __HIP_MEMORY_SCOPE_AGENT);
                break;
            }
            __builtin_amdgcn_s_sleep(1);
        }
        if (a.dbg) tsx = __builtin_amdgcn_s_memrealtime();
#pragma unroll
        for (int x = 0; x < XR; ++x)
#pragma unroll
            for (int u = 0; u < U; ++u)
#pragma unroll
                for (int h = 0; h < NW; ++h) {
                    const uint32_t w0 = xw[x][u][(2 * h) >> 2][(2 * h) & 3], w1 = xw[x][u][(2 * h + 1) >> 2][(2 * h + 1) & 3];
                    xv[x][u][h] = (w0 >> 16) | (w1 & 0xffff0000u);
                }
    }
    float pfw[PF];
    if constexpr (EPI == 0) {
        const char* kcb = reinterpret_cast<const char*>(pf_on ? a.pf_kc : a.X);
        const long long dv = pf_on ? reinterpret_cast<const char*>(a.pf_vc) - kcb : 0;
        const int nkv = pf_on ? a.pf_nkv : 1;
        const int b = blockIdx.x, h = b % nkv, jb = b / nkv, nb = ((int)gridDim.x - 1 - h) / nkv + 1;
        const int spr = pf_on ? a.pf_hd * 2 / 64 : 1;
        const int np = pf_on ? pf_p + 1 : 0, total = 2 * np * spr;
        const long long base = pf_on ? (long long)pf_s * (long long)a.pf_slot_stride + (long long)a.pf_layer_off +
                                           (long long)h * a.pf_S * a.pf_hd
                                     : 0;
#pragma unroll
        for (int q = 0; q < PF; ++q) {
            const int i = (jb + nb * q) * 256 + (int)threadIdx.x;
            const bool ok = i < total;
            const int ii = ok ? i : 0, row = ii / spr, sec = ii - row * spr;
            const bool isv = row >= np;
            const long long off = (isv ? dv : 0) + 2 * (base + (long long)(isv ? row - np : row) * a.pf_hd) + sec * 64;
            pfw[q] = *reinterpret_cast<const float*>(kcb + (ok ? off : 0));
        }
    }
    if constexpr (PRENORM && XR == 1) {
        float sl = 0.f;
#pragma unroll
        for (int u = 0; u < U; ++u) {
            if (u < nmy) {
#pragma unroll
                for (int h = 0; h < NW; ++h) {
                    const float e0 = lo16(xv[0][u][h]), e1 = hi16(xv[0][u][h]);
                    sl += e0 * e0 + e1 * e1;
                }
            }
        }
        sl = wave_sum(sl);
        if (lane == 0) red[4 * RP + wave] = sl;
        lds_barrier();
        const float tot = ((red[4 * RP] + red[4 * RP + 1]) + red[4 * RP + 2]) + red[4 * RP + 3];
        const float rs = 1.0f / sqrtf(tot / (float)a.K + a.eps);
#pragma unroll
        for (int u = 0; u < U; ++u) {
            XV o;
// ... 71 lines not shown
                }
            } else {
                float xf[8];
#pragma unroll
                for (int h = 0; h < 4; ++h) {
                    xf[2 * h] = lo16(xv[0][u][h]);
                    xf[2 * h + 1] = hi16(xv[0][u][h]);
                }
                xs += ((xf[0] + xf[1]) + (xf[2] + xf[3])) + ((xf[4] + xf[5]) + (xf[6] + xf[7]));
#pragma unroll
                for (int r = 0; r < RP; ++r) {
                    const uint32_t c0 = wv[u][r][0] ^ 0x80808080u, c1 = wv[u][r][1] ^ 0x80808080u;
                    float t = acc[0][r];
#pragma unroll
                    for (int e = 0; e < 4; ++e) t = fmaf((float)((c0 >> (8 * e)) & 0xffu), xf[e], t);
#pragma unroll
                    for (int e = 0; e < 4; ++e) t = fmaf((float)((c1 >> (8 * e)) & 0xffu), xf[4 + e], t);
                    acc[0][r] = t;
                }
            }
        }
    }
    if constexpr (LATE) {
#pragma unroll
        for (int r = 0; r < RP; ++r) asm volatile("" : "+v"(acc[0][r])::"memory");
        const XV* xp1 = reinterpret_cast<const XV*>(a.X1) + (size_t)wa * 64 + lane;
#pragma unroll
        for (int u = 0; u < U; ++u) xv[1][u] = xp1[(u < last ? u : last) * 64];
#pragma unroll
        for (int u = 0; u < U; ++u) {
            if (u < nmy) {
#pragma unroll
                for (int r = 0; r < RP; ++r) acc[1][r] = dot4(wv[u][r], xv[1][u], acc[1][r]);
            }
        }
    }
    if constexpr (EPI == 0) {
#pragma unroll
        for (int q = 0; q < PF; ++q) asm volatile("" ::"v"(pfw[q]));
    }
    const unsigned long long ts1 = a.dbg ? __builtin_amdgcn_s_memrealtime() : 0;
#pragma unroll
    for (int x = 0; x < XR; ++x)
#pragma unroll
        for (int r = 0; r < RP; ++r) {
            const float v = wave_sum(acc[x][r]);
            if (lane == 0) red[(4 * x + wave) * RP + r] = v;
        }
    if constexpr (QM == 1) {
        const float v = wave_sum(xs);
        if (lane == 0) red[4 * RP + 4 + wave] = v;
    }
    __syncthreads();
    if ((int)threadIdx.x < XR * RP) {
        const int t = XR == 2 ? (int)(threadIdx.x % RP) : (int)threadIdx.x;
        const float* rd = red + 4 * RP * ex;
        float v = ((rd[t] + rd[RP + t]) + rd[2 * RP + t]) + rd[3 * RP + t];
        if constexpr (QM == 1) {
            const float xt = ((red[4 * RP + 4] + red[4 * RP + 5]) + red[4 * RP + 6]) + red[4 * RP + 7];
            v = bfround(bfround(v - 128.f * xt) * bf2f(sv));
        }
        if (a.bias) v += bf2f(bv);
        if constexpr (FIN) {
            (ex ? a.res_out1 : a.res_out)[er] = f2bf(bfround(bf2f(rv) + bfround(v)));
        } else if constexpr (EPI == 3) {
            a.Yf[er] = bfround(v);
        } else if constexpr (EPI == 2) {
            const float up = __shfl_down(v, RP / 2, 64);
            if (t < RP / 2) {
                const float g = bfround(v);
                a.Y[blockIdx.x * (RP / 2) + t] = f2bf(bfround(g / (1.0f + expf(-g))) * bfround(up));
            }
        } else if constexpr (XR == 2) {
            if (ex || er >= a.skip0) (ex ? a.Y1 : a.Y)[er] = f2bf(v);
        } else {
            a.Y[er] = f2bf(v);
        }
    }
    if (a.dbg && threadIdx.x == 0) {
#pragma unroll
        for (int x = 0; x < XR; ++x) {
            if constexpr (TX) {
                const unsigned long long t[7] = {ts0, tsw, tsx, ts1, __builtin_amdgcn_s_memrealtime(), 0, 0};
                dbg_record(a.dbg, 0xFFF8u, polls, t);
            } else {
                const unsigned long long t[7] = {ts0, ts1, __builtin_amdgcn_s_memrealtime(), 0, 0, 0, 0};
                dbg_record(a.dbg, 0xFFFAu, (unsigned)blk, t);
            }
        }
    }
}

template <int U, int RP, bool PRENORM, int EPI, bool G, int QM>
__global__ __launch_bounds__(256) __attribute__((amdgpu_waves_per_eu(RP == 2 ? 5 : 3)))
void rowgemv_kernel(RowGemvArgs a) {
    rowgemv_body<U, RP, PRENORM, EPI, G, QM, false>(a, blockIdx.x, nullptr, 0u, nullptr);
}

template <int U, int RP, bool PRENORM, int EPI, bool G>
__global__ __launch_bounds__(256) __attribute__((amdgpu_waves_per_eu(RP == 2 ? 5 : 3)))
void rowgemv2_kernel(RowGemvArgs a) {
    if constexpr (EPI == 0) {
        if (((int)blockIdx.x + 1) * RP <= a.skip0) {
            RowGemvArgs b = a;
            b.X = a.X1;
            b.Y = a.Y1;
            rowgemv_body<U, RP, PRENORM, EPI, false, 0, false>(b, blockIdx.x, nullptr, 0u, nullptr);
            return;
        }
    }
    rowgemv_body<U, RP, PRENORM, EPI, G, 0, false, 2>(a, blockIdx.x, nullptr, 0u, nullptr);
}

int rowgemv_u(int K, int qm) {
    const int ce = qm ? 512 : 256;
    if (K <= 0 || K % ce) return 0;
    const int need = (K / ce + 3) / 4;
    for (int u : {2, 3, 4, 5, 6, 8, 10, 12})
        if (need <= u) return u;
    return 0;
}

template <int RP, bool PRENORM, int EPI, int QM>
static void rowgemv_go(hipStream_t s, const RowGemvArgs& a, int U) {
    const dim3 grid(a.N / RP), block(256);
    auto go = [&](void (*plain)(RowGemvArgs), void (*gathered)(RowGemvArgs)) {
        ((EPI == 1 ? a.residx != nullptr : a.xidx != nullptr) ? gathered : plain)<<<grid, block, 0, s>>>(a);
    };
#define RG(u) go(rowgemv_kernel<u, RP, PRENORM, EPI, false, QM>, rowgemv_kernel<u, RP, PRENORM, EPI, true, QM>)
    switch (U) {
        case 2: RG(2); break;
        case 3: RG(3); break;
        case 4: RG(4); break;
        case 5: RG(5); break;
        case 6: RG(6); break;
        case 8: RG(8); break;
        case 10: RG(10); break;
// ... 497 lines not shown
        const bool two = A.pair != 2;
        FMCHECK(two || !A.qtab, "fused fast attention + wo, pair form: the first layer is not the last");
        switch (rowgemv_u(A.wo.K, 0)) {
#define FW(u)                                                                                                            \
    case u:                                                                                                              \
        (A.qtab ? fattn_wo_pair_kernel<u, true, 2>                                                                       \
                : (two ? fattn_wo_pair_kernel<u, false, 2> : fattn_wo_pair_kernel<u, false, 1>))<<<grid, block, 0, s>>>(A); \
        break;
            FW(2) FW(3) FW(4)
            default: FW(5)
#undef FW
        }
        return;
    }
    if ((A.qtab || A.kv0) && qm) {
        auto dead = [&](auto q) {
            constexpr int Q = decltype(q)::value;
            switch (rowgemv_u(A.wo.K, Q)) {
#define FW(u) \
    case u: (A.qtab ? fattn_wo_kernel<u, true, Q, 1> : fattn_wo_kernel<u, false, Q, 2>)<<<grid, block, 0, s>>>(A); break;
                FW(2) FW(3) FW(4)
                default: FW(5)
#undef FW
            }
        };
        if (qm == 2) dead(std::integral_constant<int, 2>{});
        else dead(std::integral_constant<int, 1>{});
        return;
    }
    if (A.qtab || A.kv0) {
        switch (rowgemv_u(A.wo.K, 0)) {
#define FW(u) \
    case u: (A.qtab ? fattn_wo_kernel<u, true, 0, 1> : fattn_wo_kernel<u, false, 0, 2>)<<<grid, block, 0, s>>>(A); break;
            FW(2) FW(3) FW(4) FW(5) FW(6)
            default: (A.qtab ? fattn_wo_kernel<8, true, 0, 1> : fattn_wo_kernel<8, false, 0, 2>)<<<grid, block, 0, s>>>(A); break;
#undef FW
        }
        return;
    }
    auto go = [&](auto q) {
        constexpr int Q = decltype(q)::value;
        switch (rowgemv_u(A.wo.K, Q)) {
#define FW(u) \
    case u: (G ? fattn_wo_kernel<u, true, Q, 0> : fattn_wo_kernel<u, false, Q, 0>)<<<grid, block, 0, s>>>(A); break;
            FW(2) FW(3) FW(4) FW(5) FW(6)
            default: (G ? fattn_wo_kernel<8, true, Q, 0> : fattn_wo_kernel<8, false, Q, 0>)<<<grid, block, 0, s>>>(A); break;
#undef FW
        }
    };
    if (qm == 2) go(std::integral_constant<int, 2>{});
    else if (qm == 1) go(std::integral_constant<int, 1>{});
    else go(std::integral_constant<int, 0>{});
}
```

### fish-speech_amd/csrc/fm_tune_table.h

```cpp
#ifndef FM_TUNE_RULES
#define FM_TUNE_RULES
enum { FM_RULE_BOOL, FM_RULE_ANY, FM_RULE_SET, FM_RULE_RANGE, FM_RULE_MULT16 };
template <typename... V> constexpr int fm_knob_set(V... v) { return (0 | ... | (1 << v)); }
#define FM_BOOL FM_RULE_BOOL, 0, 0
#define FM_ANY FM_RULE_ANY, 0, 0
#define FM_SET(...) FM_RULE_SET, fm_knob_set(__VA_ARGS__), 0
#define FM_RANGE(lo, hi) FM_RULE_RANGE, lo, hi
#define FM_MIN(lo) FM_RULE_RANGE, lo, 0x7fffffff
#define FM_MULT16 FM_RULE_MULT16, 0, 0
#define FM_ZERO_OR_MULT16 FM_RULE_MULT16, 1, 0
#endif

#ifdef FM_KNOB
FM_KNOB(gemv_nt, 1, FM_BOOL)
FM_KNOB(gemv_u, 8, FM_SET(2, 4, 8))
FM_KNOB(gemv_wpb, 4, FM_SET(4, 8))
FM_KNOB(sampler_kth, 1, FM_BOOL)
FM_KNOB(sampler_fast, 1, FM_BOOL)
FM_KNOB(attn_cap, 32, FM_ZERO_OR_MULT16)
FM_KNOB(attn_wo, 0, FM_BOOL)
FM_KNOB(ksb_blocks, 512, FM_MIN(1))
FM_KNOB(batched_fused_attn, 1, FM_BOOL)
FM_KNOB(attn_cap_batched, 128, FM_ZERO_OR_MULT16)
FM_KNOB(linear_u32, 4, FM_SET(4, 8))
// ... 15 lines not shown
FM_KNOB(prompt_qkv_slab, 1, FM_BOOL)
FM_KNOB(prompt_fin, 1, FM_BOOL)
FM_KNOB(prompt_swiglu, 1, FM_BOOL)
FM_KNOB(prompt_skinny_q, 1, FM_RANGE(0, 2))
FM_KNOB(prompt_gemm_q, 1, FM_RANGE(0, 2))
FM_KNOB(prompt_ks_tiles, 384, FM_MIN(1))
FM_KNOB(prompt_ks_max, 8, FM_SET(1, 2, 4, 8))
FM_KNOB(conv2, 1, FM_BOOL)
FM_KNOB(conv_splitk, 1, FM_BOOL)
FM_KNOB(resunit_cfg, 1, FM_RANGE(0, 2))
FM_KNOB(resunit_enc, 1, FM_BOOL)
FM_KNOB(resunit_384, 1, FM_BOOL)
FM_KNOB(codec_norm, 1, FM_BOOL)
FM_KNOB(codec_rope, 1, FM_BOOL)
FM_KNOB(codec_swiglu, 1, FM_BOOL)
FM_KNOB(codec_fuse, 1, FM_BOOL)
FM_KNOB(bstream, 1, FM_BOOL)
FM_KNOB(bstream_kparts, 0, FM_SET(0, 1, 2, 4, 8))
FM_KNOB(bstream_nw, 0, FM_RANGE(0, 16))
FM_KNOB(bs_dummy, 2, FM_RANGE(0, 2))
FM_KNOB(gemv_dummy, 2, FM_RANGE(0, 2))
FM_KNOB(bs_qkv_slab, 1, FM_BOOL)
FM_KNOB(fast_tail, 1, FM_BOOL)
FM_KNOB(fkv_prefetch, 0, FM_BOOL)
FM_KNOB(kv_prefetch, 1, FM_BOOL)
FM_KNOB(bstream_chain, 0, FM_ANY)
FM_KNOB(bstream_acc, 1, FM_ANY)
FM_KNOB(rmsnorm_block, 0, FM_BOOL)
FM_KNOB(ksb_balance, 0, FM_BOOL)
FM_KNOB(chain_max, 4, FM_RANGE(2, 4))
FM_KNOB(chain_sleep, 4, FM_SET(1, 4, 16))
FM_KNOB(gemv_chain, 0, FM_BOOL)
FM_KNOB(bs_xfirst, 1, FM_BOOL)
FM_KNOB(bs_vec_epi, 1, FM_BOOL)
FM_KNOB(bsacc_kparts, 0, FM_SET(0, 1, 2, 4, 8))
FM_KNOB(q_u, 4, FM_SET(2, 4, 8, 16))
FM_KNOB(fin8, 1, FM_BOOL)
FM_KNOB(fin_split, 0, FM_RANGE(0, 16))
FM_KNOB(bstream_q8, 1, FM_BOOL)
FM_KNOB(bstream_q4, 1, FM_BOOL)
FM_KNOB(int4_stream, 1, FM_BOOL)
FM_KNOB(fw_delay, 0, FM_RANGE(0, 1000))
FM_KNOB(fw_cheap, 0, FM_BOOL)
FM_KNOB(fw_prio, 0, FM_BOOL)
FM_KNOB(fattn_wo, 1, FM_BOOL)
FM_KNOB(fattn_ilp, 1, FM_BOOL)
FM_KNOB(row_qkv_rp, 8, FM_SET(4, 8, 16))
FM_KNOB(rowgemv_q4, 31, FM_RANGE(0, 31))
FM_KNOB(rowgemv, 123, FM_RANGE(0, 127))
FM_KNOB(row_copies, 1, FM_BOOL)
FM_KNOB(prefix_vec, 1, FM_BOOL)
FM_KNOB(fast_pair, 1, FM_BOOL)
FM_KNOB(fast_dead_q, 1, FM_RANGE(0, 3))
#endif
```

### fish-speech_amd/fishmi/native.py

```python
from __future__ import annotations

import ctypes
import os

import numpy as np

HERE = os.path.dirname(os.path.abspath(__file__))
LIB_PATH = os.path.join(HERE, "libfishmi.so")

FM_PREC_BF16, FM_PREC_FP32 = 0, 1
FM_DT_F32, FM_DT_BF16, FM_DT_I8 = 0, 1, 2
FM_QUANT_NONE, FM_QUANT_INT8, FM_QUANT_INT4 = 0, 1, 2

_lib = None

ABI_SYMBOLS = [
    "fm_device_count", "fm_last_error", "fm_stream_peak", "fm_llm_open", "fm_llm_set_quant", "fm_llm_set_quant_int4", "fm_llm_set_tensor", "fm_llm_synth_tensor",
    "fm_llm_finalize", "fm_llm_prefill", "fm_llm_prefill_batch", "fm_llm_decode", "fm_llm_decode_frames", "fm_llm_generate", "fm_llm_generate_at", "fm_llm_prefill_at", "fm_llm_slot_pos", "fm_llm_teacher_step",
    "fm_llm_frame_bytes", "fm_llm_profile", "fm_llm_profile_read", "fm_llm_kernel_bench", "fm_llm_use_graph", "fm_llm_debug_vec", "fm_tune", "fm_tune_get", "fm_debug_ts_read",
    "fm_llm_close", "fm_source_hash", "fm_codec_open", "fm_codec_set_tensor", "fm_codec_synth_tensor",
    "fm_codec_finalize", "fm_codec_decode", "fm_codec_stream_reset", "fm_codec_decode_chunk",
    "fm_codec_stream_open", "fm_codec_stream_decode", "fm_codec_stream_rewind", "fm_codec_stream_close",
    "fm_codec_profile_read", "fm_codec_debug_read", "fm_codec_enable_encoder", "fm_codec_encode",
    "fm_codec_close", "fm_llm_force", "fm_llm_read_logits", "fm_op_rmsnorm", "fm_op_qk_rope", "fm_op_decode_attn", "fm_op_prompt_attn",
    "fm_op_embed", "fm_op_quant4", "fm_op_batched_linear_q8", "fm_op_batched_linear_q4", "fm_rope_table",
    "fm_op_linear", "fm_op_gemv", "fm_op_rowgemv", "fm_op_rowgemv_pair", "fm_op_bstream", "fm_op_finalize_norm", "fm_op_prompt_skinny", "fm_op_sample",
    "fm_llm_prefix_save", "fm_llm_prefix_load", "fm_llm_prefix_drop", "fm_llm_prefix_info", "fm_llm_prefill_batch_at",
    "fm_llm_set_quant_compact", "fm_llm_memory_info", "fm_op_linear_q", "fm_op_prompt_skinny_q", "fm_op_prompt_gemm_q",
    "fm_op_codec_conv", "fm_op_codec_resunit", "fm_op_codec_window_attn", "fm_op_codec_rope_qk", "fm_op_codec_dwconv_ln",
    "fm_op_codec_rvq_decode", "fm_op_codec_snake", "fm_op_codec_silu_mul", "fm_op_codec_wn_fold", "fm_op_codec_vq_encode",
    "fm_op_decode_attn_ex", "fm_op_prompt_attn_ex", "fm_op_qk_rope_cache", "fm_op_fast_attn", "fm_op_fattn_wo",
]


FM_ERR_OOM = -4


class FishMIError(RuntimeError):
    code = None


def tree_source_hash() -> str:
    import hashlib
    import re

    pkg = os.path.dirname(HERE)
    mk = open(os.path.join(pkg, "Makefile")).read()
    srcs = re.search(r"^SRCS\s*=\s*(.+)$", mk, re.M).group(1).split()
    heads = sorted(f for f in os.listdir(os.path.join(pkg, "csrc")) if f.endswith(".h"))
    files = srcs + [os.path.join("csrc", h) for h in heads] + [os.path.join("..", "include", "fishmi.h")]
    h = hashlib.sha256()
    for f in files:
        with open(os.path.join(pkg, f), "rb") as fh:
            h.update(fh.read())
    return h.hexdigest()[:16]


class SamplingC(ctypes.Structure):
    _fields_ = [("temperature", ctypes.c_float), ("top_p", ctypes.c_float),
                ("top_k", ctypes.c_int), ("seed", ctypes.c_uint64), ("mask_im_end", ctypes.c_int)]


class CodecConvDesc(ctypes.Structure):
    _fields_ = [(n, ctypes.c_int) for n in
                "precision kind Ci Co k stride dil strided npre Lx ldx Lq flags ksplit slab_rows rope_pos0 rope_nqk "
                "rope_hd".split()] + \
               [("rope_base", ctypes.c_float), ("norm_eps", ctypes.c_float)] + \
               [(n, ctypes.c_int) for n in "ldo out_rows ldr res_rows ldo2 out2_rows reps".split()]


def lib():
    global _lib
    if _lib is not None:
        return _lib
    if not os.path.exists(LIB_PATH):
        raise FishMIError(f"{LIB_PATH} is missing: build it with `make -C fish-speech_amd` "
                          "(or __graft_entry__.build()); there is no CPU fallback")
    if not os.environ.get("FISHMI_NO_TORCH_FIRST"):
        try:
            import torch
        except ImportError:
            pass
    L = ctypes.CDLL(LIB_PATH)
    L.fm_source_hash.restype = ctypes.c_char_p
# ... 24 lines not shown
    L.fm_llm_set_quant_int4.argtypes = [vp, i32]
    L.fm_llm_set_quant_compact.argtypes = [vp, i32]
    L.fm_llm_memory_info.argtypes = [vp, ctypes.POINTER(ctypes.c_int64)]
    L.fm_llm_set_tensor.argtypes = [vp, ctypes.c_char_p, vp, i32, i64]
    L.fm_llm_synth_tensor.argtypes = [vp, ctypes.c_char_p, i64, u64, f32, i32]
    L.fm_llm_finalize.argtypes = [vp]
    L.fm_llm_prefill.argtypes = [vp, i32, pi32, i32, ctypes.POINTER(SamplingC), pi32]
    L.fm_llm_prefill_batch.argtypes = [vp, i32, pi32, pi32, pi32, ctypes.POINTER(SamplingC), pi32]
    L.fm_llm_decode.argtypes = [vp, pi32, i32, pi32]
    L.fm_llm_decode_frames.argtypes = [vp, pi32, i32, i32, pi32]
    L.fm_llm_generate.argtypes = [vp, i32, pi32, i32, i32, ctypes.POINTER(SamplingC), pi32,
                                  ctypes.POINTER(ctypes.c_int)]
    L.fm_llm_generate_at.argtypes = [vp, i32, pi32, i32, i32, i32, ctypes.POINTER(SamplingC), pi32,
                                     ctypes.POINTER(ctypes.c_int)]
    L.fm_llm_prefill_at.argtypes = [vp, i32, pi32, i32, i32, ctypes.POINTER(SamplingC), pi32]
    L.fm_llm_slot_pos.argtypes = [vp, i32, ctypes.POINTER(ctypes.c_int)]
    L.fm_llm_prefix_save.argtypes = [vp, i32, i32, ctypes.POINTER(ctypes.c_int)]
    L.fm_llm_prefix_load.argtypes = [vp, i32, pi32, i32]
    L.fm_llm_prefix_drop.argtypes = [vp, i32]
    L.fm_llm_prefix_info.argtypes = [vp, i32, ctypes.POINTER(ctypes.c_int), ctypes.POINTER(ctypes.c_int64)]
    L.fm_llm_prefill_batch_at.argtypes = [vp, i32, pi32, pi32, pi32, pi32, ctypes.POINTER(SamplingC), pi32]
    L.fm_llm_teacher_step.argtypes = [vp, i32, pi32, i32, i32, pi32, pf32, pf32, pf32]
    L.fm_llm_frame_bytes.argtypes = [vp, i32, i32]
    L.fm_llm_frame_bytes.restype = i64
    L.fm_llm_profile.argtypes = [vp, i32]
    L.fm_llm_profile_read.argtypes = [vp, ctypes.c_char_p, ctypes.POINTER(ctypes.c_double),
                                      ctypes.POINTER(ctypes.c_int64), ctypes.POINTER(ctypes.c_int64)]
    L.fm_llm_kernel_bench.argtypes = [vp, ctypes.c_char_p, i32, ctypes.POINTER(ctypes.c_double),
                                      ctypes.POINTER(ctypes.c_int64), ctypes.POINTER(ctypes.c_int64)]
    L.fm_llm_use_graph.argtypes = [vp, i32]
    L.fm_llm_debug_vec.argtypes = [vp, ctypes.c_char_p, i32, pf32, i64]
    L.fm_tune.argtypes = [ctypes.c_char_p, i32]
    L.fm_tune_get.argtypes = [ctypes.c_char_p, ctypes.POINTER(ctypes.c_int)]
    L.fm_debug_ts_read.argtypes = [ctypes.POINTER(ctypes.c_uint64), i64, ctypes.POINTER(ctypes.c_int64)]
    L.fm_llm_close.argtypes = [vp]
    L.fm_llm_force.argtypes = [vp, i32, pi32]
    L.fm_llm_read_logits.argtypes = [vp, i32, pf32, pf32]
    L.fm_op_rmsnorm.argtypes = [i32, i32, i32, pf32, pf32, i32, i32, f32, pf32]
    L.fm_op_qk_rope.argtypes = [i32, i32, i32, pf32, i32, i32, i32, pf32, pf32, i32, f32, f32, i32, pf32, pf32]
    L.fm_op_prompt_attn.argtypes = [i32, i32, i32, pf32, i32, i32, i32, i32, i32, pf32, pf32, i32, pf32]
    L.fm_op_decode_attn.argtypes = [i32, i32, i32, pf32, i32, i32, i32, i32, pf32, pf32, i32, f32, f32, pi32, pf32,
                                    pf32, i32, i32, pf32, pf32, pf32]
    L.fm_op_decode_attn_ex.argtypes = [i32, i32, i32, pf32, pf32, i32, pf32, i32, i32, i32, i32, pf32, pf32, i32, f32, f32,
                                       pi32, pi32, i32, i32, i32, pf32, pf32, i32, i32, i32, i32, i32, pf32, pi32]
    L.fm_op_prompt_attn_ex.argtypes = [i32, i32, i32, pf32, i32, i32, i32, i32, pi32, pi32, i32, i32, i32, i32, pf32, pf32,
                                       i32, pf32]
    L.fm_op_qk_rope_cache.argtypes = [i32, i32, pf32, pf32, i32, pf32, i32, i32, i32, i32, pf32, pf32, i32, f32, f32, pi32,
                                      pi32, i32, i32, i32, i32, pf32, pf32, i32, pf32]
    L.fm_op_fast_attn.argtypes = [i32, i32, i32, pf32, i32, i32, i32, i32, pf32, pf32, i32, f32, f32, pi32, i32, i32, i32,
                                  i32, pf32, pf32, i32, pf32]
    L.fm_op_fattn_wo.argtypes = [i32, i32, i32, i32, pf32, pf32, i32, pi32, i32, i32, i32, i32, i32, pf32, pf32, i32, f32, f32,
                                 i32, i32, i32, i32, i32, pf32, pf32, i32, pf32, pf32, pf32, i32, i32, pf32, i32, i32, i32,
                                 i32, i32, i32, ctypes.POINTER(ctypes.c_uint32), pf32, pi32]
    L.fm_op_embed.argtypes = [i32, i32, pi32, i32, pf32, i32, pf32, i32, i32, i32, i32, i32, i32, pf32]
    L.fm_op_quant4.argtypes = [i32, pf32, i32, i32, i32, ctypes.POINTER(ctypes.c_uint8), pf32, pf32, pf32, pf32, i32,
                               pf32, pf32]
    L.fm_op_batched_linear_q8.argtypes = [i32, pf32, i32, i32, pf32, i32, i32, pf32, pf32, pi32,
                                          ctypes.POINTER(ctypes.c_int8), pf32]
    L.fm_op_batched_linear_q4.argtypes = [i32, pf32, i32, i32, i32, pf32, i32, i32, pf32, pf32, pi32,
                                          ctypes.POINTER(ctypes.c_uint8), pf32, pf32, pf32]
    L.fm_rope_table.argtypes = [i32, i32, f32, pf32]
    L.fm_op_linear.argtypes = [i32, i32, i32, pf32, pf32, pf32, pf32, i32, pf32, i32, i32, i32, i32, i32, pf32, i32,
                               i32, i32, pi32, pi32]
    L.fm_op_linear_q.argtypes = [i32, i32, i32, pf32, i32, i32, pf32, pf32, i32, pf32, i32, i32, i32, i32, pf32, pf32, i32,
                                 i32, i32, pi32, pi32, ctypes.POINTER(ctypes.c_int8), pf32, pf32]
    L.fm_op_gemv.argtypes = [i32, i32, i32, i32, i32, pf32, pf32, pf32, pf32, f32, pf32, i32, pi32, i32, i32, i32,
                             pf32, i32, i32, i32, i32, i32, pf32, i32, i32, pf32, i32, pi32]
    L.fm_op_rowgemv.argtypes = [i32, i32, i32, pf32, pf32, pf32, f32, pf32, i32, i32, pf32, i32, i32, pi32, i32, i32,
                                i32, i32, pf32, i32, i32, ctypes.POINTER(ctypes.c_int8), pf32]
    L.fm_op_rowgemv_pair.argtypes = [i32, i32, pf32, pf32, pf32, f32, pf32, pf32, pf32, i32, i32, pi32, i32, i32, i32, i32,
                                     i32, pf32, i32]
    L.fm_op_bstream.argtypes = [i32, i32, i32, i32, pf32, pf32, pf32, f32, pf32, i32, pf32, i32, i32, i32, i32, pf32,
                                i32, i32, pf32, i32, pi32, pi32]
    L.fm_op_finalize_norm.argtypes = [i32, i32, pf32, i32, i32, pf32, pf32, i32, pf32, pf32, f32, i32, i32, pf32, i32,
                                      i32, pf32, i32, i32, i32, pi32, pi32, pi32]
    L.fm_op_prompt_skinny.argtypes = [i32, pf32, pf32, i32, i32, i32, i32, i32, i32, pf32, i32, i32, i32, pi32]
    L.fm_op_prompt_skinny_q.argtypes = [i32, i32, i32, pf32, pf32, i32, i32, i32, i32, i32, i32, pf32, pf32, i32, i32, i32,
                                        pi32, ctypes.POINTER(ctypes.c_int8), pf32, pf32]
    L.fm_op_prompt_gemm_q.argtypes = [i32, i32, i32, pf32, pf32, pf32, i32, i32, i32, i32, pf32, i32, i32, pf32, pf32, i32,
                                      i32, i32, pi32, ctypes.POINTER(ctypes.c_int8), pf32, pf32]
    L.fm_op_sample.argtypes = [i32, i32, i32, pf32, i32, i32, i32, pi32, i32, pf32, pf32, pi32, pi32,
                               ctypes.POINTER(ctypes.c_uint64), pi32, pi32, i32, i32, i32, i32, i32, i32, pi32, i32,
                               pi32, pi32, i32, pf32, i32, pi32]
    L.fm_op_codec_conv.argtypes = [i32, ctypes.POINTER(CodecConvDesc), pf32, pf32, pf32, pf32, pf32, pf32, pf32, pf32, pf32,
                                   pi32, pi32]
    L.fm_op_codec_resunit.argtypes = [i32, i32, i32, i32, i32, pf32, pf32, pf32, pf32, pf32, pf32, pf32, pf32, i32, i32,
                                      pf32, i32, i32, pi32, pi32]
    L.fm_op_codec_window_attn.argtypes = [i32, i32, pf32, i32, i32, i32, i32, i32, pf32, i32, i32, pi32]
    L.fm_op_codec_rope_qk.argtypes = [i32, i32, pf32, i32, i32, i32, i32, f32, i32, i32, pi32]
    L.fm_op_codec_dwconv_ln.argtypes = [i32, i32, pf32, i32, i32, i32, pf32, pf32, pf32, pf32, pf32, i32, i32, pi32]
    L.fm_op_codec_rvq_decode.argtypes = [i32, i32, pi32, i32, i32, i32, i32, i32, pf32, pf32, pf32, pf32, i32, pf32, i32,
                                         i32, pi32]
    L.fm_op_codec_snake.argtypes = [i32, i32, pf32, i32, i64, pf32, pf32, i64, pf32, i32, pi32]
    L.fm_op_codec_silu_mul.argtypes = [i32, i32, pf32, pf32, i64, i64, i32, pi32]
    L.fm_op_codec_wn_fold.argtypes = [i32, pf32, pf32, i32, i32, pf32, i64, i32, pi32]
    L.fm_op_codec_vq_encode.argtypes = [i32, pf32, i32, i32, i32, i32, pf32, pf32, pf32, pi32, pf32, pf32, pi32, i32, pi32]
    if hasattr(L, "fm_codec_open"):
        L.fm_codec_open.argtypes = [vp, i32, i32, i32, ctypes.POINTER(vp)]
        L.fm_codec_set_tensor.argtypes = [vp, ctypes.c_char_p, vp, i32, i64]
        L.fm_codec_synth_tensor.argtypes = [vp, ctypes.c_char_p, i64, u64, f32, i32]
        L.fm_codec_finalize.argtypes = [vp]
        L.fm_codec_decode.argtypes = [vp, pi32, i32, pf32]
        L.fm_codec_stream_reset.argtypes = [vp]
        L.fm_codec_decode_chunk.argtypes = [vp, pi32, i32, pf32]
        L.fm_codec_stream_open.argtypes = [vp, ctypes.POINTER(ctypes.c_int)]
        L.fm_codec_stream_decode.argtypes = [vp, i32, pi32, i32, pf32]
# ... 56 lines not shown
```

### fish-speech_amd/fishmi/ops.py

```python
from __future__ import annotations

import ctypes

import numpy as np

from . import native

MODES = {"prologue_norm": 0, "prologue_prenorm": 1, "row_kernel": 2}


def _prec(precision: str) -> int:
    return native.FM_PREC_BF16 if precision == "bf16" else native.FM_PREC_FP32


def rmsnorm(x, w, eps, precision="bf16", mode="prologue_prenorm", device=0):
    x = np.ascontiguousarray(x, np.float32)
    R, d = x.reshape(-1, x.shape[-1]).shape
    w = np.ascontiguousarray(w, np.float32)
    y = np.zeros((R, d), np.float32)
    native.check(native.lib().fm_op_rmsnorm(device, _prec(precision), MODES[mode], native.f32p(x),
                                            native.f32p(w), R, d, float(eps), native.f32p(y)))
    return y.reshape(x.shape)


# ... 143 lines not shown


FAST_ATTN_KERNELS = {"attn2": 0, "attn2_noq": 1, "fused": 2, "unfused": 3}


def fast_attn(qkv, nh, nkv, hd, row_slot, cpos, kcache, vcache, rope_base, qn=None, kn=None, eps=1e-6, layer=0,
              precision="bf16", kernel="attn2", device=0):
    raw = np.ascontiguousarray(qkv, np.float32)
    R = raw.shape[0]
    assert raw.shape == (R, (nh + 2 * nkv) * hd)
    kc, vc = _caches(kcache, vcache, nkv, hd)
    nslots, layers, _, S, _ = kc.shape
    rs = np.ascontiguousarray(row_slot, np.int32)
    assert rs.shape == (R,)
    qk, qn_, kn_ = _norm_w(qn, kn, hd)
    out = np.zeros((R, nh, hd), np.float32)
    native.check(native.lib().fm_op_fast_attn(
        device, _prec(precision), FAST_ATTN_KERNELS[kernel], native.f32p(raw), R, nh, nkv, hd, native.f32p(qn_),
        native.f32p(kn_), qk, float(eps), float(rope_base), native.i32p(rs), int(cpos), nslots, layers, int(layer),
        native.f32p(kc), native.f32p(vc), S, native.f32p(out)))
    return out, kc, vc


def fattn_wo(qkv, nh, nkv, hd, slot, cpos, kcache, vcache, rope_base, w, res, bias=None, qn=None, kn=None, eps=1e-6,
             layer=0, quant=0, gs=128, fused=True, qtab=None, idx=None, idx_col=0, res0=None, kv0=False, pair=0, ilp=1,
             gen=1, pos0=0, xt_init=None, device=0):
    raw = np.ascontiguousarray(qkv, np.float32).reshape(-1, (nh + 2 * nkv) * hd)
    assert raw.shape[0] == (2 if pair else 1)
    kc, vc = _caches(kcache, vcache, nkv, hd)
    nslots, layers, _, S, _ = kc.shape
    ww = np.ascontiguousarray(w, np.float32)
    N = ww.shape[0]
    assert ww.shape == (N, nh * hd)
    rr = np.ascontiguousarray(res, np.float32).reshape(-1, np.shape(res)[-1])
    qt = None if qtab is None else np.ascontiguousarray(qtab, np.float32)
    ix = None if idx is None else np.ascontiguousarray(idx, np.int32)
    bi = None if bias is None else np.ascontiguousarray(bias, np.float32)
    r0 = None if res0 is None else np.ascontiguousarray(res0, np.float32)
    xt = None if xt_init is None else np.ascontiguousarray(xt_init, np.uint32)
    assert xt is None or xt.shape == (2 * nh * hd,)
    qk, qn_, kn_ = _norm_w(qn, kn, hd)
    y = np.zeros((2, N) if pair == 1 else (N,), np.float32)
    status = np.zeros(2, np.int32)
    native.check(native.lib().fm_op_fattn_wo(
        device, int(quant), int(gs), int(fused), native.f32p(raw), _opt(qt), 0 if qt is None else qt.shape[0],
        None if ix is None else native.i32p(ix), 0 if ix is None else ix.size, int(idx_col), nh, nkv, hd,
        native.f32p(qn_), native.f32p(kn_), qk, float(eps), float(rope_base), int(slot), int(cpos), nslots, layers,
        int(layer), native.f32p(kc), native.f32p(vc), S, native.f32p(ww), _opt(bi), native.f32p(rr), rr.shape[0],
        rr.shape[1], _opt(r0), N, int(kv0), int(pair), int(ilp), int(gen), int(pos0),
        None if xt is None else xt.ctypes.data_as(ctypes.POINTER(ctypes.c_uint32)), native.f32p(y), native.i32p(status)))
    return y, kc, vc, bool(status[0]), int(status[1])


def embed(tok, emb, cbemb, num_codebooks, codebook_size, semantic_begin_id, semantic_end_id, scale,
          precision="bf16", device=0):
    t = np.ascontiguousarray(tok, np.int32)
    emb = np.ascontiguousarray(emb, np.float32)
    cbemb = np.ascontiguousarray(cbemb, np.float32)
    R, d = t.shape[0], emb.shape[1]
    x = np.zeros((R, d), np.float32)
    native.check(native.lib().fm_op_embed(device, _prec(precision), native.i32p(t), R, native.f32p(emb),
                                          emb.shape[0], native.f32p(cbemb), d, num_codebooks, codebook_size,
                                          semantic_begin_id, semantic_end_id, int(scale), native.f32p(x)))
    return x


def rope_table(seq_len, head_dim, base):
    out = np.zeros((seq_len, head_dim // 2, 2), np.float32)
    native.check(native.lib().fm_rope_table(seq_len, head_dim, float(base), native.f32p(out)))
    return out


def quant4(w, gs, x=None, device=0):
    w = np.ascontiguousarray(w, np.float32)
    N, K = w.shape
    q = np.zeros((N, K), np.uint8)
    sc = np.zeros((N, K // gs), np.float32)
    zr = np.zeros((N, K // gs), np.float32)
    wd = np.zeros((N, K), np.float32)
    if x is None:
        native.check(native.lib().fm_op_quant4(device, native.f32p(w), N, K, gs,
                                               q.ctypes.data_as(ctypes.POINTER(ctypes.c_uint8)),
                                               native.f32p(sc), native.f32p(zr), native.f32p(wd), None, 0, None, None))
        return q, sc, zr, wd
    x = np.ascontiguousarray(x, np.float32).reshape(-1, K)
    R = x.shape[0]
    yb = np.zeros((R, N), np.float32)
    y4 = np.zeros((R, N), np.float32) if (gs % 128 == 0 and K % 128 == 0) else None
    native.check(native.lib().fm_op_quant4(device, native.f32p(w), N, K, gs,
                                           q.ctypes.data_as(ctypes.POINTER(ctypes.c_uint8)), native.f32p(sc),
                                           native.f32p(zr), native.f32p(wd), native.f32p(x), R,
                                           native.f32p(y4) if y4 is not None else None, native.f32p(yb)))
    return q, sc, zr, wd, yb, y4


EPI_STORE, EPI_F32, EPI_SLAB, EPI_SWIGLU8 = 0, 3, 4, 7


def batched_linear_q8(w, x, epi, device=0):
    w = np.ascontiguousarray(w, np.float32)
    N, K = w.shape
    x = np.ascontiguousarray(x, np.float32).reshape(-1, K)
    R = x.shape[0]
    No = N // 2 if epi == EPI_SWIGLU8 else N
    cap = 8 if epi == EPI_SLAB else 1
    yq = np.zeros((cap, R, No), np.float32)
# ... 392 lines not shown
```

### include/fishmi.h

```cpp
#ifndef FISHMI_H
#define FISHMI_H

#include <stdint.h>

#ifdef __cplusplus
extern "C" {
#endif

#define FM_OK 0
#define FM_ERR_ARG -1
#define FM_ERR_HIP -2
#define FM_ERR_STATE -3
#define FM_ERR_OOM -4

#define FM_PREC_BF16 0
#define FM_PREC_FP32 1

#define FM_DT_F32 0
#define FM_DT_BF16 1
#define FM_DT_I8 2

#define FM_QUANT_NONE 0
#define FM_QUANT_INT8 1
#define FM_QUANT_INT4 2
// ... 56 lines not shown
int fm_llm_prefill_batch_at(fm_llm* h, int n, const int32_t* slots, const int32_t* tokens,
                            const int32_t* T, const int32_t* pos0, const fm_sampling* sp,
                            int32_t* first_cols);
int fm_llm_teacher_step(fm_llm* h, int slot, const int32_t* x, int S, int pos0,
                        const int32_t* next_col, float* slow_logits, float* hidden,
                        float* fast_logits);
int64_t fm_llm_frame_bytes(fm_llm* h, int n, int pos);
int fm_llm_profile(fm_llm* h, int enable);
int fm_llm_profile_read(fm_llm* h, const char* kernel_class, double* total_ms, int64_t* launches,
                        int64_t* bytes);
int fm_llm_kernel_bench(fm_llm* h, const char* kernel_class, int reps, double* avg_us,
                        int64_t* launches, int64_t* bytes);
int fm_llm_use_graph(fm_llm* h, int enable);
int fm_llm_debug_vec(fm_llm* h, const char* name, int index, float* out, int64_t n);
int fm_llm_force(fm_llm* h, int slot, const int32_t* col);
int fm_llm_read_logits(fm_llm* h, int slot, float* slow_logits, float* fast_logits);
int fm_tune(const char* key, int value);
int fm_tune_get(const char* key, int* value);
int fm_debug_ts_read(unsigned long long* out, int64_t max_records, int64_t* n_records);
int fm_llm_close(fm_llm* h);

int fm_op_rmsnorm(int device, int precision, int mode, const float* x, const float* w, int R, int d,
                  float eps, float* y);
int fm_op_qk_rope(int device, int precision, int kernel, const float* qkv, int nh, int nkv, int hd,
                  const float* qn, const float* kn, int qk_norm, float eps, float rope_base, int pos,
                  float* q_out, float* k_out);
int fm_op_decode_attn(int device, int precision, int kernel, const float* qkv, int R, int nh, int nkv, int hd,
                      const float* qn, const float* kn, int qk_norm, float eps, float rope_base, const int* pos,
                      const float* kcache, const float* vcache, int S, int min_split, float* out, float* kc_out,
                      float* vc_out);
int fm_op_prompt_attn(int device, int precision, int kernel, const float* q, int R, int nh, int nkv, int hd, int pos0,
                      const float* kcache, const float* vcache, int S, float* out);
int fm_op_decode_attn_ex(int device, int precision, int kernel, const float* qkv, const float* slab, int kp,
                         const float* bias, int R, int nh, int nkv, int hd, const float* qn, const float* kn,
                         int qk_norm, float eps, float rope_base, const int* row_slot, const int* pos, int nslots,
                         int layers, int layer, float* kcache, float* vcache, int S, int cap, int nwb, int frame,
                         int reps, float* out, int* info);
int fm_op_prompt_attn_ex(int device, int precision, int kernel, const float* q, int R, int nh, int nkv, int hd,
                         const int* row_slot, const int* row_pos, int one_slot, int nslots, int layers, int layer,
                         const float* kcache, const float* vcache, int S, float* out);
int fm_op_qk_rope_cache(int device, int precision, const float* qkv, const float* slab, int kp, const float* bias, int R,
                        int nh, int nkv, int hd, const float* qn, const float* kn, int qk_norm, float eps,
                        float rope_base, const int* row_slot, const int* row_pos, int fixed_pos, int nslots, int layers,
                        int layer, float* kcache, float* vcache, int S, float* q_out);
int fm_op_fast_attn(int device, int precision, int kernel, const float* qkv, int R, int nh, int nkv, int hd,
                    const float* qn, const float* kn, int qk_norm, float eps, float rope_base, const int* row_slot,
                    int cpos, int nslots, int layers, int layer, float* kcache, float* vcache, int S, float* out);
int fm_op_fattn_wo(int device, int quant, int gs, int fused, const float* qkv, const float* qtab, int qrows,
                   const int32_t* idx, int idx_n, int idx_col, int nh, int nkv, int hd, const float* qn, const float* kn,
                   int qk_norm, float eps, float rope_base, int slot, int cpos, int nslots, int layers, int layer,
                   float* kcache, float* vcache, int S, const float* w, const float* bias, const float* res,
                   int res_rows, int ldr, const float* res0, int N, int kv0, int pair, int ilp, int gen, int pos0,
                   const uint32_t* xt_init, float* y, int* status);
int fm_op_embed(int device, int precision, const int32_t* tok, int R, const float* emb, int vocab,
                const float* cbemb, int dim, int num_codebooks, int codebook_size, int semantic_begin_id,
                int semantic_end_id, int scale_codebook_embeddings, float* x);
int fm_op_quant4(int device, const float* w, int N, int K, int gs, uint8_t* q, float* scale, float* zero,
                 float* w_deq, const float* x, int R, float* y_q4, float* y_bf16);
int fm_op_batched_linear_q8(int device, const float* w, int N, int K, const float* x, int R, int epi,
                            float* y_q8, float* y_bf16, int* kparts, int8_t* q_out, float* scale_out);
int fm_op_linear(int device, int precision, int epi, const float* w, const float* w2, const float* bias,
                 const float* x, int ldx, const float* res, int ldr, int R, int N, int K, int split, float* y, int ldy,
                 int y_rows, int reps, int* ksb, int* dirty);
int fm_op_linear_q(int device, int quant, int gs, const float* w, int N, int K, const float* bias, const float* x,
                   int ldx, const float* res, int ldr, int R, int epi, int split, float* y_q, float* y_bf16, int ldy,
                   int y_rows, int reps, int* ksb, int* dirty, int8_t* q_out, float* scale_out, float* zero_out);
int fm_op_gemv(int device, int precision, int pro, int epi, int ksb, const float* w, const float* w2, const float* bias,
               const float* nw, float eps, const float* x, int ldx, const int32_t* idx, int idx_ld, int idx_col,
               int idx_rows, const float* res, int ldr, int ss_gran, int R, int N, int K, float* y, int ldy, int y_rows,
               float* ss_out, int reps, int* dirty);
int fm_op_rowgemv(int device, int kind, int q8, const float* w, const float* bias, const float* nw, float eps,
                  const float* x, int x_rows, int ldx, const float* res, int res_rows, int ldr, const int32_t* idx,
                  int idx_n, int idx_col, int N, int K, float* y, int y_len, int reps, int8_t* q_out, float* scale_out);
int fm_op_rowgemv_pair(int device, int kind, const float* w, const float* bias, const float* nw, float eps, const float* x,
                       const float* res0, const float* res1, int res_rows, int ldr, const int32_t* idx, int idx_n,
                       int idx_col, int skip0, int N, int K, float* y, int y_ld);
int fm_op_bstream(int device, int precision, int pro, int epi, const float* w, const float* bias, const float* nw,
                  float eps, const float* x, int ldx, const float* res, int ldr, int R, int N, int K, float* y, int ldy,
                  int y_rows, float* ss_out, int reps, int* plan, int* dirty);
int fm_op_finalize_norm(int device, int precision, const float* slab, int kparts, int lds, const float* bias,
                        const float* res, int ldr, const float* nw, const float* wscale, float eps, int d, int R,
                        float* x_out, int ldx, int x_rows, float* xn_out, int ldxn, int xn_rows, int reps, int* split,
                        int* err, int* dirty);
int fm_op_prompt_skinny(int device, const float* w, const float* x, int ldx, int R, int N, int K, int target, int act,
                        float* out, int out_rows, int ldo, int reps, int* ks);
int fm_op_prompt_skinny_q(int device, int quant, int gs, const float* w, const float* x, int ldx, int R, int N, int K,
                          int target, int act, float* y_q, float* y_bf16, int out_rows, int ldo, int reps, int* ks,
                          int8_t* q_out, float* scale_out, float* zero_out);
int fm_op_prompt_gemm_q(int device, int quant, int gs, const float* w, const float* bias, const float* x, int ldx, int R,
                        int N, int K, const float* res, int ldr, int ksplit, float* y_q, float* y_bf16, int out_rows,
                        int ldo, int reps, int* plan, int8_t* q_out, float* scale_out, float* zero_out);
int fm_op_sample(int device, int precision, int slow, const float* logits, int R, int ldl, int Nl,
                 const int32_t* row_slot, int slots, const float* temperature, const float* top_p, const int32_t* top_k,
                 const int32_t* mask_im_end, const uint64_t* seed, const int32_t* step, const int32_t* force, int sb,
                 int se, int im_end, int cb, int draw, int col_idx, const int32_t* ras, int ras_enable,
                 const int32_t* force_cols, int32_t* cols, int ldc, float* tap, int tap_ld, int* kernel);
int fm_op_batched_linear_q4(int device, const float* w, int N, int K, int gs, const float* x, int R, int epi,
                            float* y_q4, float* y_bf16, int* kparts, uint8_t* q_out, float* scale_out,
                            float* zero_out, float* w_deq);
int fm_rope_table(int seq_len, int head_dim, float base, float* out);

#define FM_CE_GELU 2
#define FM_CE_RES 4
#define FM_CE_GAMMA 8
#define FM_CE_STORE 16
#define FM_CE_TANH 64
// ... 74 lines not shown
```

Before: 12.47 audio-sec/wall-sec.

## Fuse slow-transformer decode attention with the output projection in one kernel

```diff
diff --git a/fish-speech_amd/csrc/fm_attn.hip b/fish-speech_amd/csrc/fm_attn.hip
--- a/fish-speech_amd/csrc/fm_attn.hip
+++ b/fish-speech_amd/csrc/fm_attn.hip
@@ -2,6 +2,7 @@
 #include "fm_runtime.h"
 #include "fm_attn_dev.h"
 #include "fm_frag.h"
+#include "fm_attn_fd_dev.h"
 
 template <typename T>
 __device__ __forceinline__ void head_prep(const T* src, int hd, bool norm, const T* nw, float eps,
@@ -493,339 +494,9 @@
     }
 }
 
-template <typename T> __device__ __forceinline__ void cvt16(const u32x4_t v, float (&o)[16 / sizeof(T)]) {
-    if constexpr (sizeof(T) == 2) {
-#pragma unroll
-        for (int i = 0; i < 4; ++i) {
-            o[2 * i] = __uint_as_float(v[i] << 16);
-            o[2 * i + 1] = __uint_as_float(v[i] & 0xffff0000u);
-        }
-    } else {
-#pragma unroll
-        for (int i = 0; i < 4; ++i) o[i] = __uint_as_float(v[i]);
-    }
-}
-
-constexpr int FD_GM = 4;
-__device__ __forceinline__ float sum_rows4(float v, int lane) {
-    const unsigned u = __float_as_uint(v);
-    const auto r32 = __builtin_amdgcn_permlane32_swap(u, u, false, false);
-    v += __uint_as_float(lane < 32 ? r32[1] : r32[0]);
-    const unsigned w = __float_as_uint(v);
-    const auto r16 = __builtin_amdgcn_permlane16_swap(w, w, false, false);
-    return v + __uint_as_float(((lane >> 4) & 1) ? r16[0] : r16[1]);
-}
-template <typename T> __device__ __forceinline__ typename Frag<T>::f frag_f32(const float* v) {
-    typename Frag<T>::f f;
-    if constexpr (sizeof(T) == 2) {
-#pragma unroll
-        for (int i = 0; i < 4; ++i) f[i] = hi_pair(v[2 * i], v[2 * i + 1]);
-    } else {
-#pragma unroll
-        for (int i = 0; i < 4; ++i) {
-            f.lo[i] = v[i];
-            f.hi[i] = v[4 + i];
-        }
-    }
-    return f;
-}
 template <typename T, int HD, int NW, int GM>
 __global__ __launch_bounds__(NW * 64) void attn_fd_kernel(AttnDecArgs<T> a) {
-    static_assert(GM == 1 || GM == 2 || GM == FD_GM, "1, 2 or every q head of the kv head");
-    static_assert(HD % 32 == 0 && HD <= 128, "head_dim a multiple of 32 up to 128");
-    constexpr int NT = NW * 64, FD_TILE = 16 * NW;
-    constexpr int VL = 8 * (int)sizeof(T) / 16;
-    constexpr int half = HD / 2;
-    __shared__ __attribute__((aligned(16))) float q_s[GM][HD];
-    __shared__ __attribute__((aligned(16))) float kv_new[2][HD];
-    __shared__ __attribute__((aligned(16))) float wml[NW][GM][2];
-    constexpr int OG = NW > 4 ? 1 : 4;
-    __shared__ __attribute__((aligned(16))) float ored[NW][OG][GM][HD];
-    __shared__ int flag;
-    unsigned long long tz[7] = {0, 0, 0, 0, 0, 0, 0};
-    DBG_TS(tz, 0)
-    const int lane = threadIdx.x & 63, wave = threadIdx.x >> 6;
-    const int l16 = lane & 15, qq = lane >> 4;
-    const int r = blockIdx.x, kvh = blockIdx.y;
-    const int hg = GM == FD_GM ? 0 : (int)blockIdx.z / a.maxsplit, sp = (int)blockIdx.z - hg * a.maxsplit;
-    const int g = min(GM, a.nh / a.nkv - hg * GM), h0 = kvh * (a.nh / a.nkv) + hg * GM, nitem = g + 2;
-    const int slot = a.row_slot[r];
-    const int pos = a.row_pos[r];
-    constexpr int NI = (2 + GM + NW - 1) / NW;
-    float x0[NI], x1[NI];
-#pragma unroll
-    for (int i = 0; i < NI; ++i) {
-        const int it = wave + NW * i;
-        const int row = it < g ? h0 + it : (it == g ? a.nh + kvh : a.nh + a.nkv + kvh);
-        const bool ok = it < nitem && lane < half;
-        float v0, v1;
-        raw_pair<T>(a.qkv, a.ldqkv, a.qslab, a.qslab_kp, gridDim.x, a.qbias, r,
-                    (size_t)(it < nitem ? row : 0) * HD + 2 * (lane < half ? lane : 0), v0, v1);
-        x0[i] = ok ? v0 : 0.f;
-        x1[i] = ok ? v1 : 0.f;
-    }
-    const int npos = pos + 1;
-    int nsp = min(a.maxsplit, (npos + a.cap - 1) / a.cap);
-    const int chunk = ((npos + nsp - 1) / nsp + 15) & ~15;
-    nsp = (npos + chunk - 1) / chunk;
-    if (sp >= nsp) return;
-    const int j0 = sp * chunk, jend = min(j0 + chunk, npos);
-    const bool owner = jend == npos;
-    const size_t base = (size_t)slot * a.slot_stride + a.layer_off + (size_t)kvh * a.S * HD;
-    T* kc = a.kc + base;
-    T* vc = a.vc + base;
-    const int vd = 8 * l16 < HD ? 8 * l16 : HD - 8;
-    using F = Frag<T>;
-    constexpr int NKS = HD / 32;
-    typename F::f kb[NKS];
-    u32x4_t vb[4][VL];
-    auto issue = [&](int jb) {
-        const int jk = min(jb + 16 * wave + l16, jend - 1);
-#pragma unroll
-        for (int ks = 0; ks < NKS; ++ks) kb[ks] = F::load(kc + (size_t)jk * HD + 32 * ks + 8 * qq);
-#pragma unroll
-        for (int it = 0; it < 4; ++it) {
-            const int jv = min(jb + 16 * wave + 4 * it + qq, jend - 1);
-            const u32x4_t* pv = reinterpret_cast<const u32x4_t*>(vc + (size_t)jv * HD + vd);
-#pragma unroll
-            for (int c = 0; c < VL; ++c) vb[it][c] = pv[c];
-        }
-    };
-    const float* tab = a.rope + (size_t)pos * HD;
-    const float2 rcs = *reinterpret_cast<const float2*>(tab + 2 * (lane < half ? lane : 0));
-    issue(j0);
-#pragma unroll
-    for (int i = 0; i < NI; ++i) {
-        const int it = wave + NW * i;
-        if (it >= nitem || (it >= g && !owner)) continue;
-        const bool isq = it < g, isk = it == g;
-        if (a.qk_norm && (isq || isk)) {
-            const float ss = wave_sum(x0[i] * x0[i] + x1[i] * x1[i]);
-            const float rs = 1.0f / sqrtf(ss / (float)HD + a.eps);
-            const T* nw = isq ? a.qn : a.kn;
-            if (lane < half) {
-                x0[i] = rnd<T>((x0[i] * rs) * ld(nw, 2 * lane));
-                x1[i] = rnd<T>((x1[i] * rs) * ld(nw, 2 * lane + 1));
-            }
-        }
-        if (lane < half) {
-            float y0 = x0[i], y1 = x1[i];
-            if (isq || isk) {
-                const float c = rcs.x, sn = rcs.y;
-                y0 = rnd<T>(x0[i] * c - x1[i] * sn);
-                y1 = rnd<T>(x1[i] * c + x0[i] * sn);
-            }
-            if (isq) {
-                q_s[it][2 * lane] = y0;
-                q_s[it][2 * lane + 1] = y1;
-                if (a.qdbg && sp == 0) {
-                    float* qdp = a.qdbg + ((size_t)r * a.nh + h0 + it) * HD;
-                    qdp[2 * lane] = y0;
-                    qdp[2 * lane + 1] = y1;
-                }
-            } else {
-                kv_new[isk ? 0 : 1][2 * lane] = y0;
-                kv_new[isk ? 0 : 1][2 * lane + 1] = y1;
-                if (hg == 0) {
-                    T* dst = (isk ? kc : vc) + (size_t)pos * HD;
-                    st(dst, 2 * lane, y0);
-                    st(dst, 2 * lane + 1, y1);
-                }
-            }
-        }
-    }
-    lds_barrier();
-    DBG_TS(tz, 1)
-    const int qh = l16 >> 2;
-    const bool qrow = (l16 & 3) == 0 && qh < g;
-    typename F::f qa[NKS];
-#pragma unroll
-    for (int ks = 0; ks < NKS; ++ks) {
-        float qv[8];
-#pragma unroll
-        for (int e = 0; e < 8; ++e) qv[e] = qrow ? q_s[qh < GM ? qh : 0][32 * ks + 8 * qq + e] : 0.f;
-        qa[ks] = frag_f32<T>(qv);
-    }
-    __shared__ __attribute__((aligned(16))) float p_s[NW][16][GM];
-    float m_run = -INFINITY, l_run = 0.f, o[GM][8];
-#pragma unroll
-    for (int h = 0; h < GM; ++h)
-#pragma unroll
-        for (int e = 0; e < 8; ++e) o[h][e] = 0.f;
-    const int npass = (jend - j0 + FD_TILE - 1) / FD_TILE;
-    for (int pa = 0; pa < npass; ++pa) {
-        const int jb = j0 + pa * FD_TILE;
-        const int jk = jb + 16 * wave + l16;
-        if (owner && jk == pos) {
-#pragma unroll
-            for (int ks = 0; ks < NKS; ++ks) kb[ks] = frag_f32<T>(&kv_new[0][32 * ks + 8 * qq]);
-        }
-        f32x4_t sc = {0.f, 0.f, 0.f, 0.f};
-#pragma unroll
-        for (int ks = 0; ks < NKS; ++ks) sc = F::mma(qa[ks], kb[ks], sc);
-        float vf[4][8];
-#pragma unroll
-        for (int it = 0; it < 4; ++it)
-#pragma unroll
-            for (int c = 0; c < VL; ++c) {
-                float t[16 / sizeof(T)];
-                cvt16<T>(vb[it][c], t);
-#pragma unroll
-                for (int u = 0; u < (int)(16 / sizeof(T)); ++u) vf[it][c * (16 / sizeof(T)) + u] = t[u];
-            }
-        if (pa + 1 < npass) issue(jb + FD_TILE);
-        if (owner) {
-#pragma unroll
-            for (int it = 0; it < 4; ++it)
-                if (min(jb + 16 * wave + 4 * it + qq, jend - 1) == pos)
-#pragma unroll
-                    for (int e = 0; e < 8; ++e) vf[it][e] = kv_new[1][vd + e];
-        }
-        const bool kval = jk < jend && qq < g;
-        {
-            const float sv = kval ? sc[0] * a.scale : -INFINITY;
-            const float mnew = fmaxf(m_run, row_max16(sv));
-            const float alpha = mnew == -INFINITY ? 1.f : expf(m_run - mnew);
-            const float p = kval ? expf(sv - mnew) : 0.f;
-            m_run = mnew;
-            l_run = l_run * alpha + p;
-            if (GM == FD_GM || qq < GM) p_s[wave][l16][qq] = p;
-#pragma unroll
-            for (int h = 0; h < GM; ++h) {
-                if (h >= g) break;
-                const float ah = __int_as_float(__builtin_amdgcn_readlane(__float_as_int(alpha), 16 * h));
-#pragma unroll
-                for (int e = 0; e < 8; ++e) o[h][e] *= ah;
-            }
-        }
-        __builtin_amdgcn_wave_barrier();
-#pragma unroll
-        for (int it = 0; it < 4; ++it) {
-            float pv[GM];
-            if constexpr (GM == 4) {
-                const f32x4_t t = *reinterpret_cast<const f32x4_t*>(&p_s[wave][4 * it + qq][0]);
-                pv[0] = t[0], pv[1] = t[1], pv[2] = t[2], pv[3] = t[3];
-            } else if constexpr (GM == 2) {
-                const float2 t = *reinterpret_cast<const float2*>(&p_s[wave][4 * it + qq][0]);
-                pv[0] = t.x, pv[1] = t.y;
-            } else {
-                pv[0] = p_s[wave][4 * it + qq][0];
-            }
-#pragma unroll
-            for (int h = 0; h < GM; ++h) {
-                if (h >= g) break;
-#pragma unroll
-                for (int e = 0; e < 8; ++e) o[h][e] += pv[h] * vf[it][e];
-            }
-        }
-        __builtin_amdgcn_wave_barrier();
-    }
-    DBG_TS(tz, 2)
-    __shared__ unsigned long long wend[NW];
-    if (a.dbg && lane == 0) wend[wave] = __builtin_amdgcn_s_memrealtime();
-    const float lrow = row_sum16(l_run);
-    if (l16 == 0 && qq < g) {
-        wml[wave][qq][0] = m_run;
-        wml[wave][qq][1] = lrow;
-    }
-#pragma unroll
-    for (int h = 0; h < GM; ++h) {
-        if (h >= g) break;
-        if constexpr (OG == 1) {
-#pragma unroll
-            for (int e = 0; e < 8; ++e) o[h][e] = sum_rows4(o[h][e], lane);
-        }
-        if (8 * l16 < HD && (OG == 4 || qq == 0)) {
-            f32x4_t* dst = reinterpret_cast<f32x4_t*>(&ored[wave][OG == 4 ? qq : 0][h][8 * l16]);
-            dst[0] = (f32x4_t){o[h][0], o[h][1], o[h][2], o[h][3]};
-            dst[1] = (f32x4_t){o[h][4], o[h][5], o[h][6], o[h][7]};
-        }
-    }
-    DBG_TS(tz, 5)
-    lds_barrier();
-    DBG_TS(tz, 3)
-    const bool single = nsp == 1;
-    for (int idx = threadIdx.x; idx < g * HD; idx += NT) {
-        const int h = idx / HD, e = idx - h * HD;
-        float M = wml[0][h][0];
-#pragma unroll
-        for (int w = 1; w < NW; ++w) M = fmaxf(M, wml[w][h][0]);
-        float L = 0.f, O = 0.f;
-#pragma unroll
-        for (int w = 0; w < NW; ++w) {
-            const float sc = expf(wml[w][h][0] - M);
-            L += sc * wml[w][h][1];
-            if constexpr (OG == 4)
-                O += sc * ((ored[w][0][h][e] + ored[w][1][h][e]) + (ored[w][2][h][e] + ored[w][3][h][e]));
-            else
-                O += sc * ored[w][0][h][e];
-        }
-        if (single) {
-            st(a.out + (size_t)r * a.nh * HD + (size_t)(h0 + h) * HD, e, O / L);
-        } else {
-            float* pp = a.part + (((size_t)r * a.nh + h0 + h) * a.maxsplit + sp) * (HD + 2);
-            __hip_atomic_store(pp + 2 + e, O, __ATOMIC_RELAXED, __HIP_MEMORY_SCOPE_AGENT);
-            if (e == 0) {
-                __hip_atomic_store(pp, M, __ATOMIC_RELAXED, __HIP_MEMORY_SCOPE_AGENT);
-                __hip_atomic_store(pp + 1, L, __ATOMIC_RELAXED, __HIP_MEMORY_SCOPE_AGENT);
-            }
-        }
-    }
-    if (a.dbg && threadIdx.x == 0) {
-        tz[4] = __builtin_amdgcn_s_memrealtime();
-        for (int w = 0; w < NW; ++w) tz[6] = wend[w] > tz[6] ? wend[w] : tz[6];
-        dbg_record(a.dbg, 0xFFFC, (unsigned)(nsp << 16 | (jend - j0)), tz);
-    }
-    if (single) return;
-    asm volatile("s_waitcnt vmcnt(0)" ::: "memory");
-    __syncthreads();
-    if (threadIdx.x == 0) {
-        int* tk = a.cnt + (size_t)r * a.nh + kvh * (a.nh / a.nkv) + hg;
-        const int t = __hip_atomic_fetch_add(tk, 1, __ATOMIC_RELAXED, __HIP_MEMORY_SCOPE_AGENT);
-        flag = t == nsp - 1;
-        if (t == nsp - 1) __hip_atomic_store(tk, 0, __ATOMIC_RELAXED, __HIP_MEMORY_SCOPE_AGENT);
-    }
-    __syncthreads();
-    if (!flag) return;
-    DBG_TS(tz, 5)
-    constexpr int PP = GM * HD * 8 / NT > 0 ? GM * HD * 8 / NT : 1;
-    const int q = l16, grp = threadIdx.x >> 4;
-    const int k0 = grp * PP, h = k0 / half, e0 = 2 * (k0 - h * half);
-    if (h >= g) return;
-    const int qc = q < nsp ? q : nsp - 1;
-    const unsigned long long* pp = reinterpret_cast<const unsigned long long*>(
-        a.part + (((size_t)r * a.nh + h0 + h) * a.maxsplit + qc) * (HD + 2));
-    const unsigned long long ml = __hip_atomic_load(pp, __ATOMIC_RELAXED, __HIP_MEMORY_SCOPE_AGENT);
-    unsigned long long ov[PP];
-#pragma unroll
-    for (int j = 0; j < PP; ++j) ov[j] = __hip_atomic_load(pp + 1 + e0 / 2 + j, __ATOMIC_RELAXED, __HIP_MEMORY_SCOPE_AGENT);
-    const float mq = q < nsp ? __uint_as_float((unsigned)ml) : -INFINITY;
-    const float lq = __uint_as_float((unsigned)(ml >> 32));
-    float M = mq;
-#pragma unroll
-    for (int m = 1; m < 16; m <<= 1) M = fmaxf(M, __shfl_xor(M, m));
-    const float w = q < nsp ? expf(mq - M) : 0.f;
-    float L = w * lq;
-#pragma unroll
-    for (int m = 1; m < 16; m <<= 1) L += __shfl_xor(L, m);
-    T* out = a.out + (size_t)r * a.nh * HD + (size_t)(h0 + h) * HD + e0;
-#pragma unroll
-    for (int j = 0; j < PP; ++j) {
-        float o0 = w * __uint_as_float((unsigned)ov[j]), o1 = w * __uint_as_float((unsigned)(ov[j] >> 32));
-#pragma unroll
-        for (int m = 1; m < 16; m <<= 1) {
-            o0 += __shfl_xor(o0, m);
-            o1 += __shfl_xor(o1, m);
-        }
-        if (q == (j & 15)) {
-            st(out, 2 * j, o0 / L);
-            st(out, 2 * j + 1, o1 / L);
-        }
-    }
-    if (a.dbg && threadIdx.x == 0) {
-        tz[6] = __builtin_amdgcn_s_memrealtime();
-        dbg_record(a.dbg, 0xFFFB, (unsigned)nsp, tz);
-    }
+    attn_fd_body<T, HD, NW, GM, false>(a, blockIdx.x, blockIdx.y, blockIdx.z, gridDim.x, nullptr, 0u);
 }
 
 template <typename T>
diff --git a/fish-speech_amd/csrc/fm_attn_fd_dev.h b/fish-speech_amd/csrc/fm_attn_fd_dev.h
--- /dev/null
+++ b/fish-speech_amd/csrc/fm_attn_fd_dev.h
@@ -0,0 +1,352 @@
+#pragma once
+#include "fm_kernels.h"
+#include "fm_attn_dev.h"
+#include "fm_frag.h"
+
+template <typename T> __device__ __forceinline__ void cvt16(const u32x4_t v, float (&o)[16 / sizeof(T)]) {
+    if constexpr (sizeof(T) == 2) {
+#pragma unroll
+        for (int i = 0; i < 4; ++i) {
+            o[2 * i] = __uint_as_float(v[i] << 16);
+            o[2 * i + 1] = __uint_as_float(v[i] & 0xffff0000u);
+        }
+    } else {
+#pragma unroll
+        for (int i = 0; i < 4; ++i) o[i] = __uint_as_float(v[i]);
+    }
+}
+
+constexpr int FD_GM = 4;
+__device__ __forceinline__ float sum_rows4(float v, int lane) {
+    const unsigned u = __float_as_uint(v);
+    const auto r32 = __builtin_amdgcn_permlane32_swap(u, u, false, false);
+    v += __uint_as_float(lane < 32 ? r32[1] : r32[0]);
+    const unsigned w = __float_as_uint(v);
+    const auto r16 = __builtin_amdgcn_permlane16_swap(w, w, false, false);
+    return v + __uint_as_float(((lane >> 4) & 1) ? r16[0] : r16[1]);
+}
+template <typename T> __device__ __forceinline__ typename Frag<T>::f frag_f32(const float* v) {
+    typename Frag<T>::f f;
+    if constexpr (sizeof(T) == 2) {
+#pragma unroll
+        for (int i = 0; i < 4; ++i) f[i] = hi_pair(v[2 * i], v[2 * i + 1]);
+    } else {
+#pragma unroll
+        for (int i = 0; i < 4; ++i) {
+            f.lo[i] = v[i];
+            f.hi[i] = v[4 + i];
+        }
+    }
+    return f;
+}
+template <typename T, int HD, int NW, int GM, bool TAG>
+__device__ __forceinline__ void attn_fd_body(const AttnDecArgs<T>& a, const int bx, const int by, const int bz, const int R,
+                                             uint32_t* xt, const uint32_t gen) {
+    static_assert(!TAG || sizeof(T) == 2, "tagged output words: bf16");
+    static_assert(GM == 1 || GM == 2 || GM == FD_GM, "1, 2 or every q head of the kv head");
+    static_assert(HD % 32 == 0 && HD <= 128, "head_dim a multiple of 32 up to 128");
+    constexpr int NT = NW * 64, FD_TILE = 16 * NW;
+    constexpr int VL = 8 * (int)sizeof(T) / 16;
+    constexpr int half = HD / 2;
+    __shared__ __attribute__((aligned(16))) float q_s[GM][HD];
+    __shared__ __attribute__((aligned(16))) float kv_new[2][HD];
+    __shared__ __attribute__((aligned(16))) float wml[NW][GM][2];
+    constexpr int OG = NW > 4 ? 1 : 4;
+    __shared__ __attribute__((aligned(16))) float ored[NW][OG][GM][HD];
+    __shared__ int flag;
+    unsigned long long tz[7] = {0, 0, 0, 0, 0, 0, 0};
+    DBG_TS(tz, 0)
+    const int lane = threadIdx.x & 63, wave = threadIdx.x >> 6;
+    const int l16 = lane & 15, qq = lane >> 4;
+    const int r = bx, kvh = by;
+    const int hg = GM == FD_GM ? 0 : bz / a.maxsplit, sp = bz - hg * a.maxsplit;
+    const int g = min(GM, a.nh / a.nkv - hg * GM), h0 = kvh * (a.nh / a.nkv) + hg * GM, nitem = g + 2;
+    const int slot = a.row_slot[r];
+    const int pos = a.row_pos[r];
+    constexpr int NI = (2 + GM + NW - 1) / NW;
+    float x0[NI], x1[NI];
+#pragma unroll
+    for (int i = 0; i < NI; ++i) {
+        const int it = wave + NW * i;
+        const int row = it < g ? h0 + it : (it == g ? a.nh + kvh : a.nh + a.nkv + kvh);
+        const bool ok = it < nitem && lane < half;
+        float v0, v1;
+        raw_pair<T>(a.qkv, a.ldqkv, a.qslab, a.qslab_kp, R, a.qbias, r,
+                    (size_t)(it < nitem ? row : 0) * HD + 2 * (lane < half ? lane : 0), v0, v1);
+        x0[i] = ok ? v0 : 0.f;
+        x1[i] = ok ? v1 : 0.f;
+    }
+    const int npos = pos + 1;
+    int nsp = min(a.maxsplit, (npos + a.cap - 1) / a.cap);
+    const int chunk = ((npos + nsp - 1) / nsp + 15) & ~15;
+    nsp = (npos + chunk - 1) / chunk;
+    if (sp >= nsp) return;
+    const int j0 = sp * chunk, jend = min(j0 + chunk, npos);
+    const bool owner = jend == npos;
+    const size_t base = (size_t)slot * a.slot_stride + a.layer_off + (size_t)kvh * a.S * HD;
+    T* kc = a.kc + base;
+    T* vc = a.vc + base;
+    const int vd = 8 * l16 < HD ? 8 * l16 : HD - 8;
+    using F = Frag<T>;
+    constexpr int NKS = HD / 32;
+    typename F::f kb[NKS];
+    u32x4_t vb[4][VL];
+    auto issue = [&](int jb) {
+        const int jk = min(jb + 16 * wave + l16, jend - 1);
+#pragma unroll
+        for (int ks = 0; ks < NKS; ++ks) kb[ks] = F::load(kc + (size_t)jk * HD + 32 * ks + 8 * qq);
+#pragma unroll
+        for (int it = 0; it < 4; ++it) {
+            const int jv = min(jb + 16 * wave + 4 * it + qq, jend - 1);
+            const u32x4_t* pv = reinterpret_cast<const u32x4_t*>(vc + (size_t)jv * HD + vd);
+#pragma unroll
+            for (int c = 0; c < VL; ++c) vb[it][c] = pv[c];
+        }
+    };
+    const float* tab = a.rope + (size_t)pos * HD;
+    const float2 rcs = *reinterpret_cast<const float2*>(tab + 2 * (lane < half ? lane : 0));
+    issue(j0);
+#pragma unroll
+    for (int i = 0; i < NI; ++i) {
+        const int it = wave + NW * i;
+        if (it >= nitem || (it >= g && !owner)) continue;
+        const bool isq = it < g, isk = it == g;
+        if (a.qk_norm && (isq || isk)) {
+            const float ss = wave_sum(x0[i] * x0[i] + x1[i] * x1[i]);
+            const float rs = 1.0f / sqrtf(ss / (float)HD + a.eps);
+            const T* nw = isq ? a.qn : a.kn;
+            if (lane < half) {
+                x0[i] = rnd<T>((x0[i] * rs) * ld(nw, 2 * lane));
+                x1[i] = rnd<T>((x1[i] * rs) * ld(nw, 2 * lane + 1));
+            }
+        }
+        if (lane < half) {
+            float y0 = x0[i], y1 = x1[i];
+            if (isq || isk) {
+                const float c = rcs.x, sn = rcs.y;
+                y0 = rnd<T>(x0[i] * c - x1[i] * sn);
+                y1 = rnd<T>(x1[i] * c + x0[i] * sn);
+            }
+            if (isq) {
+                q_s[it][2 * lane] = y0;
+                q_s[it][2 * lane + 1] = y1;
+                if (a.qdbg && sp == 0) {
+                    float* qdp = a.qdbg + ((size_t)r * a.nh + h0 + it) * HD;
+                    qdp[2 * lane] = y0;
+                    qdp[2 * lane + 1] = y1;
+                }
+            } else {
+                kv_new[isk ? 0 : 1][2 * lane] = y0;
+                kv_new[isk ? 0 : 1][2 * lane + 1] = y1;
+                if (hg == 0) {
+                    T* dst = (isk ? kc : vc) + (size_t)pos * HD;
+                    st(dst, 2 * lane, y0);
+                    st(dst, 2 * lane + 1, y1);
+                }
+            }
+        }
+    }
+    lds_barrier();
+    DBG_TS(tz, 1)
+    const int qh = l16 >> 2;
+    const bool qrow = (l16 & 3) == 0 && qh < g;
+    typename F::f qa[NKS];
+#pragma unroll
+    for (int ks = 0; ks < NKS; ++ks) {
+        float qv[8];
+#pragma unroll
+        for (int e = 0; e < 8; ++e) qv[e] = qrow ? q_s[qh < GM ? qh : 0][32 * ks + 8 * qq + e] : 0.f;
+        qa[ks] = frag_f32<T>(qv);
+    }
+    __shared__ __attribute__((aligned(16))) float p_s[NW][16][GM];
+    float m_run = -INFINITY, l_run = 0.f, o[GM][8];
+#pragma unroll
+    for (int h = 0; h < GM; ++h)
+#pragma unroll
+        for (int e = 0; e < 8; ++e) o[h][e] = 0.f;
+    const int npass = (jend - j0 + FD_TILE - 1) / FD_TILE;
+    for (int pa = 0; pa < npass; ++pa) {
+        const int jb = j0 + pa * FD_TILE;
+        const int jk = jb + 16 * wave + l16;
+        if (owner && jk == pos) {
+#pragma unroll
+            for (int ks = 0; ks < NKS; ++ks) kb[ks] = frag_f32<T>(&kv_new[0][32 * ks + 8 * qq]);
+        }
+        f32x4_t sc = {0.f, 0.f, 0.f, 0.f};
+#pragma unroll
+        for (int ks = 0; ks < NKS; ++ks) sc = F::mma(qa[ks], kb[ks], sc);
+        float vf[4][8];
+#pragma unroll
+        for (int it = 0; it < 4; ++it)
+#pragma unroll
+            for (int c = 0; c < VL; ++c) {
+                float t[16 / sizeof(T)];
+                cvt16<T>(vb[it][c], t);
+#pragma unroll
+                for (int u = 0; u < (int)(16 / sizeof(T)); ++u) vf[it][c * (16 / sizeof(T)) + u] = t[u];
+            }
+        if (pa + 1 < npass) issue(jb + FD_TILE);
+        if (owner) {
+#pragma unroll
+            for (int it = 0; it < 4; ++it)
+                if (min(jb + 16 * wave + 4 * it + qq, jend - 1) == pos)
+#pragma unroll
+                    for (int e = 0; e < 8; ++e) vf[it][e] = kv_new[1][vd + e];
+        }
+        const bool kval = jk < jend && qq < g;
+        {
+            const float sv = kval ? sc[0] * a.scale : -INFINITY;
+            const float mnew = fmaxf(m_run, row_max16(sv));
+            const float alpha = mnew == -INFINITY ? 1.f : expf(m_run - mnew);
+            const float p = kval ? expf(sv - mnew) : 0.f;
+            m_run = mnew;
+            l_run = l_run * alpha + p;
+            if (GM == FD_GM || qq < GM) p_s[wave][l16][qq] = p;
+#pragma unroll
+            for (int h = 0; h < GM; ++h) {
+                if (h >= g) break;
+                const float ah = __int_as_float(__builtin_amdgcn_readlane(__float_as_int(alpha), 16 * h));
+#pragma unroll
+                for (int e = 0; e < 8; ++e) o[h][e] *= ah;
+            }
+        }
+        __builtin_amdgcn_wave_barrier();
+#pragma unroll
+        for (int it = 0; it < 4; ++it) {
+            float pv[GM];
+            if constexpr (GM == 4) {
+                const f32x4_t t = *reinterpret_cast<const f32x4_t*>(&p_s[wave][4 * it + qq][0]);
+                pv[0] = t[0], pv[1] = t[1], pv[2] = t[2], pv[3] = t[3];
+            } else if constexpr (GM == 2) {
+                const float2 t = *reinterpret_cast<const float2*>(&p_s[wave][4 * it + qq][0]);
+                pv[0] = t.x, pv[1] = t.y;
+            } else {
+                pv[0] = p_s[wave][4 * it + qq][0];
+            }
+#pragma unroll
+            for (int h = 0; h < GM; ++h) {
+                if (h >= g) break;
+#pragma unroll
+                for (int e = 0; e < 8; ++e) o[h][e] += pv[h] * vf[it][e];
+            }
+        }
+        __builtin_amdgcn_wave_barrier();
+    }
+    DBG_TS(tz, 2)
+    __shared__ unsigned long long wend[NW];
+    if (a.dbg && lane == 0) wend[wave] = __builtin_amdgcn_s_memrealtime();
+    const float lrow = row_sum16(l_run);
+    if (l16 == 0 && qq < g) {
+        wml[wave][qq][0] = m_run;
+        wml[wave][qq][1] = lrow;
+    }
+#pragma unroll
+    for (int h = 0; h < GM; ++h) {
+        if (h >= g) break;
+        if constexpr (OG == 1) {
+#pragma unroll
+            for (int e = 0; e < 8; ++e) o[h][e] = sum_rows4(o[h][e], lane);
+        }
+        if (8 * l16 < HD && (OG == 4 || qq == 0)) {
+            f32x4_t* dst = reinterpret_cast<f32x4_t*>(&ored[wave][OG == 4 ? qq : 0][h][8 * l16]);
+            dst[0] = (f32x4_t){o[h][0], o[h][1], o[h][2], o[h][3]};
+            dst[1] = (f32x4_t){o[h][4], o[h][5], o[h][6], o[h][7]};
+        }
+    }
+    DBG_TS(tz, 5)
+    lds_barrier();
+    DBG_TS(tz, 3)
+    const bool single = nsp == 1;
+    for (int idx = threadIdx.x; idx < g * HD; idx += NT) {
+        const int h = idx / HD, e = idx - h * HD;
+        float M = wml[0][h][0];
+#pragma unroll
+        for (int w = 1; w < NW; ++w) M = fmaxf(M, wml[w][h][0]);
+        float L = 0.f, O = 0.f;
+#pragma unroll
+        for (int w = 0; w < NW; ++w) {
+            const float sc = expf(wml[w][h][0] - M);
+            L += sc * wml[w][h][1];
+            if constexpr (OG == 4)
+                O += sc * ((ored[w][0][h][e] + ored[w][1][h][e]) + (ored[w][2][h][e] + ored[w][3][h][e]));
+            else
+                O += sc * ored[w][0][h][e];
+        }
+        if (single) {
+            if constexpr (TAG)
+                __hip_atomic_store(xt + (size_t)(h0 + h) * HD + e, ((uint32_t)f2bf(O / L) << 16) | gen, __ATOMIC_RELAXED,
+                                   __HIP_MEMORY_SCOPE_AGENT);
+            else
+                st(a.out + (size_t)r * a.nh * HD + (size_t)(h0 + h) * HD, e, O / L);
+        } else {
+            float* pp = a.part + (((size_t)r * a.nh + h0 + h) * a.maxsplit + sp) * (HD + 2);
+            __hip_atomic_store(pp + 2 + e, O, __ATOMIC_RELAXED, __HIP_MEMORY_SCOPE_AGENT);
+            if (e == 0) {
+                __hip_atomic_store(pp, M, __ATOMIC_RELAXED, __HIP_MEMORY_SCOPE_AGENT);
+                __hip_atomic_store(pp + 1, L, __ATOMIC_RELAXED, __HIP_MEMORY_SCOPE_AGENT);
+            }
+        }
+    }
+    if (a.dbg && threadIdx.x == 0) {
+        tz[4] = __builtin_amdgcn_s_memrealtime();
+        for (int w = 0; w < NW; ++w) tz[6] = wend[w] > tz[6] ? wend[w] : tz[6];
+        dbg_record(a.dbg, 0xFFFC, (unsigned)(nsp << 16 | (jend - j0)), tz);
+    }
+    if (single) return;
+    asm volatile("s_waitcnt vmcnt(0)" ::: "memory");
+    __syncthreads();
+    if (threadIdx.x == 0) {
+        int* tk = a.cnt + (size_t)r * a.nh + kvh * (a.nh / a.nkv) + hg;
+        const int t = __hip_atomic_fetch_add(tk, 1, __ATOMIC_RELAXED, __HIP_MEMORY_SCOPE_AGENT);
+        flag = t == nsp - 1;
+        if (t == nsp - 1) __hip_atomic_store(tk, 0, __ATOMIC_RELAXED, __HIP_MEMORY_SCOPE_AGENT);
+    }
+    __syncthreads();
+    if (!flag) return;
+    DBG_TS(tz, 5)
+    constexpr int PP = GM * HD * 8 / NT > 0 ? GM * HD * 8 / NT : 1;
+    const int q = l16, grp = threadIdx.x >> 4;
+    const int k0 = grp * PP, h = k0 / half, e0 = 2 * (k0 - h * half);
+    if (h >= g) return;
+    const int qc = q < nsp ? q : nsp - 1;
+    const unsigned long long* pp = reinterpret_cast<const unsigned long long*>(
+        a.part + (((size_t)r * a.nh + h0 + h) * a.maxsplit + qc) * (HD + 2));
+    const unsigned long long ml = __hip_atomic_load(pp, __ATOMIC_RELAXED, __HIP_MEMORY_SCOPE_AGENT);
+    unsigned long long ov[PP];
+#pragma unroll
+    for (int j = 0; j < PP; ++j) ov[j] = __hip_atomic_load(pp + 1 + e0 / 2 + j, __ATOMIC_RELAXED, __HIP_MEMORY_SCOPE_AGENT);
+    const float mq = q < nsp ? __uint_as_float((unsigned)ml) : -INFINITY;
+    const float lq = __uint_as_float((unsigned)(ml >> 32));
+    float M = mq;
+#pragma unroll
+    for (int m = 1; m < 16; m <<= 1) M = fmaxf(M, __shfl_xor(M, m));
+    const float w = q < nsp ? expf(mq - M) : 0.f;
+    float L = w * lq;
+#pragma unroll
+    for (int m = 1; m < 16; m <<= 1) L += __shfl_xor(L, m);
+    T* out = a.out + (size_t)r * a.nh * HD + (size_t)(h0 + h) * HD + e0;
+#pragma unroll
+    for (int j = 0; j < PP; ++j) {
+        float o0 = w * __uint_as_float((unsigned)ov[j]), o1 = w * __uint_as_float((unsigned)(ov[j] >> 32));
+#pragma unroll
+        for (int m = 1; m < 16; m <<= 1) {
+            o0 += __shfl_xor(o0, m);
+            o1 += __shfl_xor(o1, m);
+        }
+        if (q == (j & 15)) {
+            if constexpr (TAG) {
+                const uint64_t w = (uint64_t)(((uint32_t)f2bf(o0 / L) << 16) | gen) |
+                                   ((uint64_t)(((uint32_t)f2bf(o1 / L) << 16) | gen) << 32);
+                __hip_atomic_store(reinterpret_cast<uint64_t*>(xt + (size_t)(h0 + h) * HD + e0 + 2 * j), w, __ATOMIC_RELAXED,
+                                   __HIP_MEMORY_SCOPE_AGENT);
+            } else {
+                st(out, 2 * j, o0 / L);
+                st(out, 2 * j + 1, o1 / L);
+            }
+        }
+    }
+    if (a.dbg && threadIdx.x == 0) {
+        tz[6] = __builtin_amdgcn_s_memrealtime();
+        dbg_record(a.dbg, 0xFFFB, (unsigned)nsp, tz);
+    }
+}
diff --git a/fish-speech_amd/csrc/fm_kernels.h b/fish-speech_amd/csrc/fm_kernels.h
--- a/fish-speech_amd/csrc/fm_kernels.h
+++ b/fish-speech_amd/csrc/fm_kernels.h
@@ -417,6 +417,17 @@
 constexpr int FD_NSP = 16;
 inline bool attn_fd_ok(int hd, int g) { return (hd == 32 || hd == 64 || hd == 128) && g >= 1 && g <= 4; }
 template <typename T> void launch_attn_fd(hipStream_t s, const AttnDecArgs<T>& a, int R);
+struct SlowAttnWoArgs {
+    AttnDecArgs<bf16_t> at;
+    RowGemvArgs wo;
+    uint32_t* xt;
+    int gen;
+    int* err;
+    int rp;
+    int delay_pct, sleep, cheap;
+};
+bool slow_attn_wo_ok(int nh, int nkv, int hd, int N, int K);
+void launch_slow_attn_wo(hipStream_t s, const SlowAttnWoArgs& a);
 template <typename T> void launch_attn_decode3(hipStream_t s, const AttnDecArgs<T>& a, int R);
 template <typename T> void launch_fast_attn_fused(hipStream_t s, const FastFusedArgs<T>& a, int R);
 template <typename T> void launch_fast_attn2(hipStream_t s, const FastFusedArgs<T>& a, int R);
diff --git a/fish-speech_amd/csrc/fm_llm.cpp b/fish-speech_amd/csrc/fm_llm.cpp
--- a/fish-speech_amd/csrc/fm_llm.cpp
+++ b/fish-speech_amd/csrc/fm_llm.cpp
@@ -59,7 +59,7 @@
 
 static void chain_err_async(fm_llm* m) {
     if (fm_tuning().gemv_chain || fm_tuning().fin_split > 1 ||
-        (m->fxt && fm_tuning().fattn_wo))
+        (m->fxt && fm_tuning().fattn_wo) || (m->sxt && fm_tuning().slow_attn_wo))
         HIPCHK(hipMemcpyAsync(m->h_chain_err, m->chain_err, sizeof(int), hipMemcpyDeviceToHost, m->stream));
 }
 static void chain_err_check(fm_llm* m) {
@@ -69,7 +69,7 @@
     HIPCHK(hipMemset(m->chain_err, 0, 16 * sizeof(int)));
     if (m->fin_cnt) HIPCHK(hipMemset(m->fin_cnt, 0, (size_t)std::max(m->max_slots, 64) * 2 * sizeof(int)));
     throw FmError{FM_ERR_STATE,
-                  "in-launch hand-off wait timed out (gemv chain / split finalize / fused fast "
+                  "in-launch hand-off wait timed out (gemv chain / split finalize / fused fast or slow "
                   "attention + wo; counters reset)"};
 }
 
diff --git a/fish-speech_amd/csrc/fm_llm_frame.cpp b/fish-speech_amd/csrc/fm_llm_frame.cpp
--- a/fish-speech_amd/csrc/fm_llm_frame.cpp
+++ b/fish-speech_amd/csrc/fm_llm_frame.cpp
@@ -768,12 +768,22 @@
         bool tab;
         bool kv0;
         bool kv_only;
+        bool sw;
     };
+    bool slow_attn_wo_live(const Small& c, bool rf) const {
+        const StackDims& d = c.d;
+        if (!(sizeof(T) == 2 && !c.is_fast && c.n == 1 && rf && !m->quant && fm_tuning().slow_attn_wo && m->sxt &&
+              !fm_tuning().gemv_chain && d.n_layer >= 2 && d.n_layer <= 40 && !c.L.wo.rm_scale && !c.L.wo.rm_sz))
+            return false;
+        const AttnSlowPlan ap = attn_slow_plan(1, d.hd, d.nh / d.nkv, attn2_frame_cap(d.hd, d.nh / d.nkv, E, false));
+        return ap.kernel == 3 && ap.nwb == 8 && ap.hpb == 1 && slow_attn_wo_ok(d.nh, d.nkv, d.hd, d.dim, d.nq());
+    }
     SmallPath small_path(const Small& c, bool kv_only) const {
         const StackDims& d = c.d;
         SmallPath p{};
         p.kv_only = kv_only;
         p.rf = row_fin(c.n);
+        p.sw = !kv_only && slow_attn_wo_live(c, p.rf);
         const int fq = m->qmode();
         const bool fw_any = c.is_fast && p.rf && fm_tuning().fattn_wo && m->fxt && m->fdm.n_layer * m->C >= 2 &&
                             m->fdm.n_layer * m->C <= 40 && fattn_wo_ok(d.nh, d.nkv, d.hd, c.cpos, d.dim, d.nq(), fq);
@@ -825,20 +835,26 @@
             gemv(c.L.wqkv, a, PRO_PRENORM, EPI_STORE, 1, "linear", p.kv0 ? d.nq() / 16 : 0);
         }
     }
+    AttnDecArgs<T> small_slow_args(const Small& c) const {
+        const StackDims& d = c.d;
+        AttnDecArgs<T> aa{(const T*)m->qkv, d.nqkv(), m->frame_slot, m->frame_pos, d.nh, d.nkv, d.hd,
+                          d.qk_norm, m->c.norm_eps, (const T*)c.L.qn, (const T*)c.L.kn, m->rope, (T*)m->kc,
+                          (T*)m->vc, m->slot_stride, (size_t)c.layer * m->layer_stride, m->S,
+                          m->maxsplit, 1.0f / sqrtf((float)d.hd), m->part};
+        aa.cap = attn2_frame_cap(d.hd, d.nh / d.nkv, E, false);
+        aa.maxsplit = FM_CEIL(m->S, aa.cap);
+        aa.cnt = m->attn_cnt;
+        aa.dbg = fm_tuning().dbg;
+        aa.out = (T*)m->att;
+        return aa;
+    }
     void small_attn(const Small& c, const SmallPath& p) {
         const StackDims& d = c.d;
         const int n = c.n;
         hipStream_t st = s;
+        if (p.sw) return;
         if (!c.is_fast) {
-            AttnDecArgs<T> aa{(const T*)m->qkv, d.nqkv(), m->frame_slot, m->frame_pos, d.nh, d.nkv, d.hd,
-                              d.qk_norm, m->c.norm_eps, (const T*)c.L.qn, (const T*)c.L.kn, m->rope, (T*)m->kc,
-                              (T*)m->vc, m->slot_stride, (size_t)c.layer * m->layer_stride, m->S,
-                              m->maxsplit, 1.0f / sqrtf((float)d.hd), m->part};
-            aa.cap = attn2_frame_cap(d.hd, d.nh / d.nkv, E, false);
-            aa.maxsplit = FM_CEIL(m->S, aa.cap);
-            aa.cnt = m->attn_cnt;
-            aa.dbg = fm_tuning().dbg;
-            aa.out = (T*)m->att;
+            const AttnDecArgs<T> aa = small_slow_args(c);
             auto go = [st, aa, n] { attn_slow_on(st, aa, n); };
             m->prof.record("attn_slow", 0, go);
             launch("attn", 0, 0, go);
@@ -885,6 +901,25 @@
             }
             r.N = d.dim;
             r.K = d.nq();
+            if (p.sw) {
+                SlowAttnWoArgs W{};
+                if constexpr (sizeof(T) == 2) {
+                    W.at = small_slow_args(c);
+                    W.at.cap = attn_slow_plan(1, d.hd, d.nh / d.nkv, W.at.cap).cap;
+                }
+                W.wo = r;
+                W.xt = m->sxt;
+                W.gen = 1 + c.layer;
+                W.err = m->chain_err;
+                W.rp = fm_tuning().slow_attn_wo == 2 ? 4 : 2;
+                W.delay_pct = fm_tuning().slow_aw_delay;
+                W.sleep = fm_tuning().slow_aw_sleep;
+                W.cheap = fm_tuning().slow_aw_cheap;
+                hipStream_t st = s;
+                auto go = [st, W] { launch_slow_attn_wo(st, W); };
+                launch("slow_attn_wo", rowgemv_wbytes(r), 2.0 * r.N * r.K, go);
+                return;
+            }
             if (!p.fw) {
                 rowgemv(r, ROWGEMV_FIN);
                 return;
diff --git a/fish-speech_amd/csrc/fm_llm_model.h b/fish-speech_amd/csrc/fm_llm_model.h
--- a/fish-speech_amd/csrc/fm_llm_model.h
+++ b/fish-speech_amd/csrc/fm_llm_model.h
@@ -158,6 +158,7 @@
     bool row_qkv_ok = false;
     bool row_w13_ok = false;
     uint32_t* fxt = nullptr;
+    uint32_t* sxt = nullptr;
     int32_t* fiota = nullptr;
     void* qkv0 = nullptr;
     int32_t* qkv0_iota = nullptr;
diff --git a/fish-speech_amd/csrc/fm_llm_weights.cpp b/fish-speech_amd/csrc/fm_llm_weights.cpp
--- a/fish-speech_amd/csrc/fm_llm_weights.cpp
+++ b/fish-speech_amd/csrc/fm_llm_weights.cpp
@@ -406,6 +406,9 @@
     }
     if (m->prec == FM_PREC_BF16)
         m->fxt = (uint32_t*)m->dalloc(2 * (size_t)m->fdm.nh * m->fdm.hd * sizeof(uint32_t));
+    if (m->prec == FM_PREC_BF16 && !m->quant && m->sd.n_layer >= 2 && m->sd.n_layer <= 40 &&
+        slow_attn_wo_ok(m->sd.nh, m->sd.nkv, m->sd.hd, m->sd.dim, m->sd.nq()))
+        m->sxt = (uint32_t*)m->dalloc((size_t)m->sd.nq() * sizeof(uint32_t));
     m->emb = W(m, "embeddings.weight");
     m->cbemb = W(m, "codebook_embeddings.weight");
     m->norm = W(m, "norm.weight");
diff --git a/fish-speech_amd/csrc/fm_ops.cpp b/fish-speech_amd/csrc/fm_ops.cpp
--- a/fish-speech_amd/csrc/fm_ops.cpp
+++ b/fish-speech_amd/csrc/fm_ops.cpp
@@ -544,6 +544,105 @@
     HIPCHK(hipStreamSynchronize(s));
 }
 
+struct SlowAttnWoOp {
+    int fused, rp;
+    const float* qkv;
+    int nh, nkv, hd;
+    const float *qn, *kn;
+    int qk_norm;
+    float eps, base;
+    const int32_t *slots, *pos, *gens;
+    int nrun, restore, nslots, layers, layer;
+    const float *kc, *vc;
+    int S;
+    const float *w, *bias, *res;
+    int N;
+    const uint32_t* xt_init;
+    float *y, *krows, *vrows;
+    int* status;
+};
+void slow_attn_wo_op(hipStream_t s, const SlowAttnWoOp& o) {
+    DevBufs b(s);
+    const int nh = o.nh, nkv = o.nkv, hd = o.hd, S = o.S, N = o.N, K = nh * hd, ld = (nh + 2 * nkv) * hd, g = nh / nkv;
+    const AttnSlowPlan ap = attn_slow_plan(1, hd, g, attn2_frame_cap(hd, g, 2, false));
+    o.status[0] = ap.kernel == 3 && ap.nwb == 8 && ap.hpb == 1 && slow_attn_wo_ok(nh, nkv, hd, N, K) && !fm_tuning().gemv_chain;
+    o.status[1] = 0;
+    if (o.fused && !o.status[0]) return;
+    FMCHECK(ap.kernel == 3, "the unfused composition runs attn_fd");
+    RowGemvArgs r{};
+    r.W = b.upload<bf16_t>(o.w, (size_t)N * K);
+    if (o.bias) r.bias = b.upload<bf16_t>(o.bias, (size_t)N);
+    r.res = b.upload<bf16_t>(o.res, (size_t)N);
+    r.ldr = N;
+    r.N = N;
+    r.K = K;
+    const bf16_t* raw = b.upload<bf16_t>(o.qkv, (size_t)o.nrun * ld);
+    bf16_t* qnd = o.qk_norm ? b.upload<bf16_t>(o.qn, (size_t)hd) : (bf16_t*)b.alloc((size_t)hd * 2);
+    bf16_t* knd = o.qk_norm ? b.upload<bf16_t>(o.kn, (size_t)hd) : (bf16_t*)b.alloc((size_t)hd * 2);
+    float* rope = upload_rope(b, S, hd, o.base);
+    const size_t layer_stride = (size_t)nkv * S * hd, slot_stride = (size_t)o.layers * layer_stride;
+    const size_t cn = (size_t)o.nslots * slot_stride, layer_off = (size_t)o.layer * layer_stride;
+    const bf16_t *kc0 = b.upload<bf16_t>(o.kc, cn), *vc0 = b.upload<bf16_t>(o.vc, cn);
+    bf16_t *kc = (bf16_t*)b.alloc(cn * 2), *vc = (bf16_t*)b.alloc(cn * 2);
+    HIPCHK(hipMemcpyAsync(kc, kc0, cn * 2, hipMemcpyDeviceToDevice, s));
+    HIPCHK(hipMemcpyAsync(vc, vc0, cn * 2, hipMemcpyDeviceToDevice, s));
+    int* rows_d = (int*)b.alloc(8);
+    bf16_t* att = (bf16_t*)b.alloc((size_t)K * 2);
+    bf16_t* yd = (bf16_t*)b.alloc((size_t)o.nrun * N * 2);
+    bf16_t *kr = (bf16_t*)b.alloc((size_t)o.nrun * nkv * hd * 2), *vr = (bf16_t*)b.alloc((size_t)o.nrun * nkv * hd * 2);
+    uint32_t* xt = (uint32_t*)b.alloc((size_t)K * 4);
+    if (o.xt_init) b.put(xt, o.xt_init, (size_t)K * 4);
+    int* err = (int*)b.alloc(16);
+    AttnDecArgs<bf16_t> at{raw, ld, rows_d, rows_d + 1, nh, nkv, hd, o.qk_norm, o.eps, qnd, knd, rope, kc, vc, slot_stride,
+                           layer_off, S, 1, 1.0f / sqrtf((float)hd), nullptr};
+    at.cap = ap.cap;
+    at.nwb = ap.nwb;
+    at.hpb = ap.hpb;
+    at.maxsplit = std::min(FD_NSP, FM_CEIL(S, at.cap));
+    at.part = (float*)b.alloc((size_t)nh * at.maxsplit * (hd + 2) * 4);
+    at.cnt = (int*)b.alloc((size_t)nh * 4);
+    at.out = att;
+    for (int i = 0; i < o.nrun; ++i) {
+        if (o.restore && i) {
+            HIPCHK(hipMemcpyAsync(kc, kc0, cn * 2, hipMemcpyDeviceToDevice, s));
+            HIPCHK(hipMemcpyAsync(vc, vc0, cn * 2, hipMemcpyDeviceToDevice, s));
+        }
+        const int rs[2] = {o.slots[i], o.pos[i]};
+        b.put(rows_d, rs, 8);
+        at.qkv = raw + (size_t)i * ld;
+        r.res_out = yd + (size_t)i * N;
+        r.X = att;
+        if (o.fused) {
+            SlowAttnWoArgs A{};
+            A.at = at;
+            A.wo = r;
+            A.xt = xt;
+            A.gen = o.gens[i];
+            A.err = err;
+            A.rp = o.rp;
+            A.delay_pct = fm_tuning().slow_aw_delay;
+            A.sleep = fm_tuning().slow_aw_sleep;
+            A.cheap = fm_tuning().slow_aw_cheap;
+            launch_slow_attn_wo(s, A);
+        } else {
+            launch_attn_fd<bf16_t>(s, at, 1);
+            HIPCHK(hipGetLastError());
+            launch_rowgemv(s, r, ROWGEMV_FIN);
+        }
+        HIPCHK(hipGetLastError());
+        const size_t row0 = (size_t)o.slots[i] * slot_stride + layer_off + (size_t)o.pos[i] * hd;
+        HIPCHK(hipMemcpy2DAsync(kr + (size_t)i * nkv * hd, (size_t)hd * 2, kc + row0, (size_t)S * hd * 2, (size_t)hd * 2, nkv,
+                                hipMemcpyDeviceToDevice, s));
+        HIPCHK(hipMemcpy2DAsync(vr + (size_t)i * nkv * hd, (size_t)hd * 2, vc + row0, (size_t)S * hd * 2, (size_t)hd * 2, nkv,
+                                hipMemcpyDeviceToDevice, s));
+    }
+    download<bf16_t>(yd, (size_t)o.nrun * N, o.y, s);
+    download<bf16_t>(kr, (size_t)o.nrun * nkv * hd, o.krows, s);
+    download<bf16_t>(vr, (size_t)o.nrun * nkv * hd, o.vrows, s);
+    HIPCHK(hipMemcpyAsync(&o.status[1], err, 4, hipMemcpyDeviceToHost, s));
+    HIPCHK(hipStreamSynchronize(s));
+}
+
 template <typename T>
 void embed_t(hipStream_t s, const int32_t* tok, int R, const float* emb, int V, const float* cbemb, int d, int C,
              int cb, int sb, int se, int scale, float* x) {
@@ -1213,6 +1312,28 @@
     });
 }
 
+int fm_op_slow_attn_wo(int device, int fused, int rp, const float* qkv, int nh, int nkv, int hd, const float* qn,
+                       const float* kn, int qk_norm, float eps, float rope_base, const int32_t* slots, const int32_t* pos,
+                       const int32_t* gens, int nrun, int restore, int nslots, int layers, int layer, const float* kcache,
+                       const float* vcache, int S, const float* w, const float* bias, const float* res, int N,
+                       const uint32_t* xt_init, float* y, float* k_rows, float* v_rows, int* status) {
+    return fm_guard([&] {
+        FMCHECK(qkv && slots && pos && gens && kcache && vcache && w && res && y && k_rows && v_rows && status, "null argument");
+        FMCHECK(!qk_norm || (qn && kn), "qk_norm needs both norm weights");
+        FMCHECK(nh >= 1 && nkv >= 1 && nh % nkv == 0 && hd >= 8 && hd <= 128 && hd % 8 == 0, "bad heads / head_dim");
+        FMCHECK(S >= 16 && S % 16 == 0 && S <= 65536 && N >= 16 && N % 16 == 0 && nrun >= 1 && nrun <= 4096, "bad S / N / runs");
+        FMCHECK(rp == 2 || rp == 4, "rp must be 2 or 4");
+        for (int i = 0; i < nrun; ++i) {
+            FMCHECK(pos[i] >= 0 && pos[i] < S && gens[i] >= 1 && gens[i] <= 40, "bad position / gen");
+            check_slot_rows(1, &slots[i], nullptr, nslots, layers, layer, S);
+        }
+        StreamGuard g(device);
+        const SlowAttnWoOp o{fused, rp, qkv, nh, nkv, hd, qn, kn, qk_norm, eps, rope_base, slots, pos, gens, nrun, restore,
+                             nslots, layers, layer, kcache, vcache, S, w, bias, res, N, xt_init, y, k_rows, v_rows, status};
+        slow_attn_wo_op(g.s, o);
+    });
+}
+
 int fm_op_qk_rope(int device, int precision, int kernel, const float* qkv, int nh, int nkv, int hd, const float* qn,
                   const float* kn, int qk_norm, float eps, float rope_base, int pos, float* q_out, float* k_out) {
     return fm_guard([&] {
diff --git a/fish-speech_amd/csrc/fm_rowgemv.hip b/fish-speech_amd/csrc/fm_rowgemv.hip
--- a/fish-speech_amd/csrc/fm_rowgemv.hip
+++ b/fish-speech_amd/csrc/fm_rowgemv.hip
@@ -1,6 +1,7 @@
 #include "fm_common.h"
 #include "fm_kernels.h"
 #include "fm_runtime.h"
+#include "fm_attn_fd_dev.h"
 #include <type_traits>
 
 typedef __attribute__((ext_vector_type(2))) uint32_t u32x2_t;
@@ -41,9 +42,13 @@
     static constexpr int WPL = QM == 2 ? 1 : 2;
 };
 
-template <int U, int RP, bool PRENORM, int EPI, bool G, int QM, bool TX, int XR = 1>
+struct TxPoll {
+    unsigned delay = 0;
+    int sleep = 1, cheap = 0;
+};
+template <int U, int RP, bool PRENORM, int EPI, bool G, int QM, bool TX, int XR = 1, int NG = 1>
 __device__ __forceinline__ void rowgemv_body(const RowGemvArgs& a, const int blk, const uint32_t* xt, const uint32_t gen,
-                                             int* err) {
+                                             int* err, const TxPoll pw = TxPoll{}) {
     static_assert(!TX || (!PRENORM && EPI == 1), "tagged x: the residual form only");
     static_assert(XR == 1 || (XR == 2 && QM == 0 && EPI <= 1 && (!G || EPI == 1)), "two x rows: bf16 STORE / FIN");
     constexpr bool FIN = EPI == 1;
@@ -52,15 +57,18 @@
     constexpr int EPL = R::EPL, NW = EPL / 2;
     constexpr int SB = XR * 4 * RP;
     constexpr bool LATE = XR == 2 && !TX && !PRENORM && U >= 10;
-    __shared__ float red[XR * (4 * RP + 8)];
-    const int lane = threadIdx.x & 63, wave = threadIdx.x >> 6;
+    static_assert(NG == 1 || (NG == 2 && TX), "two row blocks per 512-thread block: the tagged-x form only");
+    __shared__ float red_s[NG][XR * (4 * RP + 8)];
+    const unsigned tid = NG == 1 ? threadIdx.x : threadIdx.x & 255u;
+    float(&red)[XR * (4 * RP + 8)] = red_s[NG == 1 ? 0 : threadIdx.x >> 8];
+    const int lane = tid & 63, wave = tid >> 6;
     const int n0 = blk * RP;
     const int nch = a.K / R::CE;
     const int wa = (wave * nch) >> 2, nmy = (((wave + 1) * nch) >> 2) - wa;
     const int last = nmy > 0 ? nmy - 1 : 0;
     const unsigned long long ts0 = a.dbg ? __builtin_amdgcn_s_memrealtime() : 0;
-    const int er = n0 + (int)(threadIdx.x % RP);
-    const int ex = XR == 2 ? (int)((threadIdx.x / RP) & 1) : 0;
+    const int er = n0 + (int)(tid % RP);
+    const int ex = XR == 2 ? (int)((tid / RP) & 1) : 0;
     int ri = 0, xi = 0;
     if constexpr (G && FIN) {
         const int32_t iv = a.residx[a.res_col];
@@ -126,11 +134,34 @@
     }
     asm volatile("" ::: "memory");
     unsigned long long tsw = 0, tsx = 0;
-    unsigned polls = 0;
+    unsigned polls = 0, cpolls = 0;
     if constexpr (TX) {
         if (a.dbg) tsw = __builtin_amdgcn_s_memrealtime();
         const __amdgpu_buffer_rsrc_t xr = __builtin_amdgcn_make_buffer_rsrc((void*)xt, (short)0, XR * a.K * 4, 0x00020000);
         u32x4_t xw[XR][U][EPL / 4];
+        auto nap = [&] {
+            if constexpr (NG == 2) {
+                if (pw.sleep >= 16) __builtin_amdgcn_s_sleep(16);
+                else if (pw.sleep >= 4) __builtin_amdgcn_s_sleep(4);
+                else __builtin_amdgcn_s_sleep(1);
+            } else {
+                __builtin_amdgcn_s_sleep(1);
+            }
+        };
+        if constexpr (NG == 2) {
+            const unsigned long long tw0 = __builtin_amdgcn_s_memrealtime();
+            while (pw.delay && (unsigned)(__builtin_amdgcn_s_memrealtime() - tw0) < pw.delay) __builtin_amdgcn_s_sleep(8);
+            if (pw.cheap) {
+                const int ng = nmy * (R::CE / 128);
+                const int wi = (wa * R::CE + 128 * (lane < ng ? lane : 0) + 127) * 4;
+                for (unsigned it = 0; it < (1u << 14); ++it) {
+                    cpolls = it + 1;
+                    const uint32_t w = __builtin_amdgcn_raw_buffer_load_b32(xr, wi, 0, 16);
+                    if (__all((w & 0xffffu) == gen)) break;
+                    nap();
+                }
+            }
+        }
         for (unsigned it = 0;; ++it) {
             polls = it + 1;
 #pragma unroll
@@ -157,7 +188,7 @@
                 if (lane == 0) __hip_atomic_store(err, 1, __ATOMIC_RELAXED, __HIP_MEMORY_SCOPE_AGENT);
                 break;
             }
-            __builtin_amdgcn_s_sleep(1);
+            nap();
         }
         if (a.dbg) tsx = __builtin_amdgcn_s_memrealtime();
 #pragma unroll
@@ -335,8 +366,8 @@
         if (lane == 0) red[4 * RP + 4 + wave] = v;
     }
     __syncthreads();
-    if ((int)threadIdx.x < XR * RP) {
-        const int t = XR == 2 ? (int)(threadIdx.x % RP) : (int)threadIdx.x;
+    if ((int)tid < XR * RP) {
+        const int t = XR == 2 ? (int)(tid % RP) : (int)tid;
         const float* rd = red + 4 * RP * ex;
         float v = ((rd[t] + rd[RP + t]) + rd[2 * RP + t]) + rd[3 * RP + t];
         if constexpr (QM == 1) {
@@ -360,12 +391,17 @@
             a.Y[er] = f2bf(v);
         }
     }
-    if (a.dbg && threadIdx.x == 0) {
+    if (a.dbg && tid == 0) {
 #pragma unroll
         for (int x = 0; x < XR; ++x) {
             if constexpr (TX) {
                 const unsigned long long t[7] = {ts0, tsw, tsx, ts1, __builtin_amdgcn_s_memrealtime(), 0, 0};
-                dbg_record(a.dbg, 0xFFF8u, polls, t);
+                dbg_record(a.dbg, 0xFFF8u, polls | (cpolls << 16), t);
+                if constexpr (NG == 2) {
+                    const unsigned long long tr[7] = {ts0, ts1, t[4], 0, 0, 0, 0};
+#pragma unroll
+                    for (int p = 0; p < RP / 2; ++p) dbg_record(a.dbg, 0xFFFAu, 0x80000000u | (unsigned)(blk * (RP / 2) + p), tr);
+                }
             } else {
                 const unsigned long long t[7] = {ts0, ts1, __builtin_amdgcn_s_memrealtime(), 0, 0, 0, 0};
                 dbg_record(a.dbg, 0xFFFAu, (unsigned)blk, t);
@@ -969,3 +1005,55 @@
     else if (qm == 1) go(std::integral_constant<int, 1>{});
     else go(std::integral_constant<int, 0>{});
 }
+
+template <int U, int HD, int RP>
+__global__ __launch_bounds__(512) __attribute__((amdgpu_waves_per_eu(4)))
+void slow_attn_wo_kernel(SlowAttnWoArgs A) {
+    const AttnDecArgs<bf16_t>& at = A.at;
+    const uint32_t gen = ((uint32_t)at.row_pos[0] * 41u + (uint32_t)A.gen) % 65535u + 1u;
+    const int natt = at.nh * at.maxsplit;
+    if ((int)blockIdx.x < natt) {
+        const int b = blockIdx.x;
+        attn_fd_body<bf16_t, HD, 8, 1, true>(at, 0, b % at.nkv, b / at.nkv, 1, A.xt, gen);
+        return;
+    }
+    TxPoll pw;
+    if (RP == 4 && A.delay_pct) {
+        const int npos = at.row_pos[0] + 1;
+        const int nsp = min(at.maxsplit, (npos + at.cap - 1) / at.cap);
+        const int chunk = ((npos + nsp - 1) / nsp + 15) & ~15;
+        pw.delay = (unsigned)(A.delay_pct * (300 + chunk * 12 / 10 + (nsp > 1 ? 180 : 0)) / 100);
+    }
+    pw.sleep = A.sleep;
+    pw.cheap = A.cheap;
+    rowgemv_body<U, RP, false, 1, false, 0, true, 1, 2>(A.wo, 2 * ((int)blockIdx.x - natt) + (int)(threadIdx.x >> 8), A.xt, gen,
+                                                        A.err, pw);
+}
+
+bool slow_attn_wo_ok(int nh, int nkv, int hd, int N, int K) {
+    const int U = rowgemv_u(K, 0);
+    return nkv > 0 && nh % nkv == 0 && attn_fd_ok(hd, nh / nkv) && hd == 128 && K == nh * hd && N > 0 && N % 8 == 0 &&
+           (U == 2 || U == 4);
+}
+
+void launch_slow_attn_wo(hipStream_t s, const SlowAttnWoArgs& A0) {
+    SlowAttnWoArgs A = A0;
+    AttnDecArgs<bf16_t>& at = A.at;
+    at.dbg = A.wo.dbg = fm_tuning().dbg;
+    if (A.sleep < 1) A.sleep = 1;
+    FMCHECK(A.delay_pct >= 0 && A.delay_pct <= 300, "fused slow attention + wo: first-read delay of 0 .. 300 per cent");
+    FMCHECK(slow_attn_wo_ok(at.nh, at.nkv, at.hd, A.wo.N, A.wo.K) && A.xt && A.err && A.gen > 0 && A.gen <= 40 && at.row_pos &&
+                at.row_slot && at.cap >= 16 && at.cnt && at.part && !at.qslab && (A.rp == 2 || A.rp == 4) && A.wo.W && A.wo.X &&
+                !A.wo.Wq && !A.wo.Wq4 && A.wo.res && A.wo.res_out && !A.wo.residx && A.wo.xr != 2,
+            "fused slow attention + wo: shapes, tag and buffers");
+    at.maxsplit = std::min(FD_NSP, FM_CEIL(at.S, at.cap));
+    at.nwb = 8;
+    at.hpb = 1;
+    const dim3 grid(at.nh * at.maxsplit + A.wo.N / (2 * A.rp)), block(512);
+    const int U = rowgemv_u(A.wo.K, 0);
+#define SW(u, hd)                                                                   \
+    (A.rp == 4 ? slow_attn_wo_kernel<u, hd, 4><<<grid, block, 0, s>>>(A) : slow_attn_wo_kernel<u, hd, 2><<<grid, block, 0, s>>>(A))
+    if (U == 2) SW(2, 128);
+    else SW(4, 128);
+#undef SW
+}
diff --git a/fish-speech_amd/csrc/fm_tune_table.h b/fish-speech_amd/csrc/fm_tune_table.h
--- a/fish-speech_amd/csrc/fm_tune_table.h
+++ b/fish-speech_amd/csrc/fm_tune_table.h
@@ -91,4 +91,8 @@
 FM_KNOB(prefix_vec, 1, FM_BOOL)
 FM_KNOB(fast_pair, 1, FM_BOOL)
 FM_KNOB(fast_dead_q, 1, FM_RANGE(0, 3))
+FM_KNOB(slow_attn_wo, 2, FM_RANGE(0, 2))
+FM_KNOB(slow_aw_delay, 40, FM_RANGE(0, 300))
+FM_KNOB(slow_aw_sleep, 1, FM_SET(1, 4, 16))
+FM_KNOB(slow_aw_cheap, 1, FM_BOOL)
 #endif
diff --git a/fish-speech_amd/fishmi/native.py b/fish-speech_amd/fishmi/native.py
--- a/fish-speech_amd/fishmi/native.py
+++ b/fish-speech_amd/fishmi/native.py
@@ -30,6 +30,7 @@
     "fm_op_codec_conv", "fm_op_codec_resunit", "fm_op_codec_window_attn", "fm_op_codec_rope_qk", "fm_op_codec_dwconv_ln",
     "fm_op_codec_rvq_decode", "fm_op_codec_snake", "fm_op_codec_silu_mul", "fm_op_codec_wn_fold", "fm_op_codec_vq_encode",
     "fm_op_decode_attn_ex", "fm_op_prompt_attn_ex", "fm_op_qk_rope_cache", "fm_op_fast_attn", "fm_op_fattn_wo",
+    "fm_op_slow_attn_wo",
 ]
 
 
@@ -160,6 +161,9 @@
     L.fm_op_fattn_wo.argtypes = [i32, i32, i32, i32, pf32, pf32, i32, pi32, i32, i32, i32, i32, i32, pf32, pf32, i32, f32, f32,
                                  i32, i32, i32, i32, i32, pf32, pf32, i32, pf32, pf32, pf32, i32, i32, pf32, i32, i32, i32,
                                  i32, i32, i32, ctypes.POINTER(ctypes.c_uint32), pf32, pi32]
+    L.fm_op_slow_attn_wo.argtypes = [i32, i32, i32, pf32, i32, i32, i32, pf32, pf32, i32, f32, f32, pi32, pi32, pi32, i32, i32,
+                                     i32, i32, i32, pf32, pf32, i32, pf32, pf32, pf32, i32, ctypes.POINTER(ctypes.c_uint32),
+                                     pf32, pf32, pf32, pi32]
     L.fm_op_embed.argtypes = [i32, i32, pi32, i32, pf32, i32, pf32, i32, i32, i32, i32, i32, i32, pf32]
     L.fm_op_quant4.argtypes = [i32, pf32, i32, i32, i32, ctypes.POINTER(ctypes.c_uint8), pf32, pf32, pf32, pf32, i32,
                                pf32, pf32]
diff --git a/fish-speech_amd/fishmi/ops.py b/fish-speech_amd/fishmi/ops.py
--- a/fish-speech_amd/fishmi/ops.py
+++ b/fish-speech_amd/fishmi/ops.py
@@ -219,6 +219,36 @@
     return y, kc, vc, bool(status[0]), int(status[1])
 
 
+def slow_attn_wo(qkv, nh, nkv, hd, slots, pos, kcache, vcache, rope_base, w, res, bias=None, qn=None, kn=None, eps=1e-6,
+                 layer=0, fused=True, rp=2, gens=None, restore=True, xt_init=None, device=0):
+    raw = np.ascontiguousarray(qkv, np.float32).reshape(-1, (nh + 2 * nkv) * hd)
+    n = raw.shape[0]
+    sl = np.ascontiguousarray(np.broadcast_to(np.asarray(slots, np.int32), (n,)))
+    ps = np.ascontiguousarray(np.broadcast_to(np.asarray(pos, np.int32), (n,)))
+    ge = np.ascontiguousarray(np.broadcast_to(np.asarray(1 if gens is None else gens, np.int32), (n,)))
+    kc, vc = _caches(kcache, vcache, nkv, hd)
+    nslots, layers, _, S, _ = kc.shape
+    ww = np.ascontiguousarray(w, np.float32)
+    N = ww.shape[0]
+    assert ww.shape == (N, nh * hd)
+    rr = np.ascontiguousarray(res, np.float32).reshape(N)
+    bi = None if bias is None else np.ascontiguousarray(bias, np.float32)
+    xt = None if xt_init is None else np.ascontiguousarray(xt_init, np.uint32)
+    assert xt is None or xt.shape == (nh * hd,)
+    qk, qn_, kn_ = _norm_w(qn, kn, hd)
+    y = np.zeros((n, N), np.float32)
+    kr = np.zeros((n, nkv, hd), np.float32)
+    vr = np.zeros((n, nkv, hd), np.float32)
+    status = np.zeros(2, np.int32)
+    native.check(native.lib().fm_op_slow_attn_wo(
+        device, int(fused), int(rp), native.f32p(raw), nh, nkv, hd, native.f32p(qn_), native.f32p(kn_), qk, float(eps),
+        float(rope_base), native.i32p(sl), native.i32p(ps), native.i32p(ge), n, int(restore), nslots, layers, int(layer),
+        native.f32p(kc), native.f32p(vc), S, native.f32p(ww), _opt(bi), native.f32p(rr), N,
+        None if xt is None else xt.ctypes.data_as(ctypes.POINTER(ctypes.c_uint32)), native.f32p(y), native.f32p(kr),
+        native.f32p(vr), native.i32p(status)))
+    return y, kr, vr, bool(status[0]), int(status[1])
+
+
 def embed(tok, emb, cbemb, num_codebooks, codebook_size, semantic_begin_id, semantic_end_id, scale,
           precision="bf16", device=0):
     t = np.ascontiguousarray(tok, np.int32)
diff --git a/include/fishmi.h b/include/fishmi.h
--- a/include/fishmi.h
+++ b/include/fishmi.h
@@ -132,6 +132,11 @@
                    float* kcache, float* vcache, int S, const float* w, const float* bias, const float* res,
                    int res_rows, int ldr, const float* res0, int N, int kv0, int pair, int ilp, int gen, int pos0,
                    const uint32_t* xt_init, float* y, int* status);
+int fm_op_slow_attn_wo(int device, int fused, int rp, const float* qkv, int nh, int nkv, int hd, const float* qn,
+                       const float* kn, int qk_norm, float eps, float rope_base, const int32_t* slots, const int32_t* pos,
+                       const int32_t* gens, int nrun, int restore, int nslots, int layers, int layer, const float* kcache,
+                       const float* vcache, int S, const float* w, const float* bias, const float* res, int N,
+                       const uint32_t* xt_init, float* y, float* k_rows, float* v_rows, int* status);
 int fm_op_embed(int device, int precision, const int32_t* tok, int R, const float* emb, int vocab,
                 const float* cbemb, int dim, int num_codebooks, int codebook_size, int semantic_begin_id,
                 int semantic_end_id, int scale_codebook_embeddings, float* x);
```

Result: faster. 12.67 audio-sec/wall-sec, median of 6 (+1.6%).
